# NikolaZubic/2dimageto3dmodel

Measured on NVIDIA H100. Metric: render+loss+GAN images/sec (cfg3: cfg2 render+loss at batch 32 + conv-GAN 256x256 G/D iteration, 1 G : 2 D, Adam), higher is better.
Workload: dtype tf32 (convs) / f32

## Files before the change

### 2dimageto3dmodel_b200/b3d/__init__.py

```python
import ctypes
import os

import torch

_HERE = os.path.dirname(os.path.abspath(__file__))
LIB_PATH = os.path.join(_HERE, "libb3d.so")

MODE_REFERENCE = 0
MODE_PAPER = 1
_MODES = {"R": MODE_REFERENCE, "reference": MODE_REFERENCE, "P": MODE_PAPER, "paper": MODE_PAPER,
          0: MODE_REFERENCE, 1: MODE_PAPER}


class B3DError(RuntimeError):
    pass


def _load():
    if not os.path.exists(LIB_PATH):
        raise B3DError(f"{LIB_PATH} is missing: build it with `make` (or __graft_entry__.build()). "
                       "There is no CPU fallback.")
    lib = ctypes.CDLL(LIB_PATH)
    lib.b3d_last_error.restype = ctypes.c_char_p
    lib.b3d_last_variant.restype = ctypes.c_char_p
    lib.b3d_launch_count.restype = ctypes.c_uint64
    lib.b3d_pc_silhouette_workspace_bytes.restype = ctypes.c_size_t
    return lib


lib = _load()

_vp = ctypes.c_void_p
_i = ctypes.c_int
_f = ctypes.c_float
_sz = ctypes.c_size_t
_ll = ctypes.c_longlong


_signed = []


def _sig(name, *argtypes):
    fn = getattr(lib, name)
    fn.argtypes = list(argtypes)
    fn.restype = ctypes.c_int
    _signed.append(name)
    return fn


_sig("b3d_pc_bin_count", _i)
_sig("b3d_inception_input", _vp, _i, _i, _i, _i, _i, _i, _i, _vp, _vp)
_sig("b3d_maxpool3x3s2_nhwc", _vp, _i, _i, _i, _i, _vp, _i, _vp)
_sig("b3d_mean_hw_nhwc", _vp, _i, _i, _i, _vp, _vp)
_sig("b3d_fid_accumulate", _vp, _i, _i, _vp, _vp, _vp)
_sig("b3d_pc_project", _vp, _vp, _i, _i, _i, _f, _f, _vp, _vp, _vp, _vp, _vp, _vp, _vp)
_sig("b3d_pc_silhouette_fwd_hosttaps", _vp, _vp, _vp, _i, _vp, _i, _i, _i, _i, _vp, _vp, _sz, _vp)
_sig("b3d_pc_silhouette_bwd_hosttaps", _vp, _vp, _vp, _i, _vp, _vp, _i, _i, _i, _i, _vp, _vp, _vp, _sz, _vp)
_sig("b3d_pc_project_bwd", _vp, _vp, _vp, _vp, _i, _i, _i, _f, _f, _vp, _vp, _vp)
_sig("b3d_pc_splat_grid", _vp, _i, _i, _i, _i, _vp, _vp)
_sig("b3d_mesh_face_setup", _vp, _vp, _vp, _i, _vp, _i, _i, _i, _i, _vp, _vp, _vp, _vp)
_sig("b3d_mesh_render_fwd", _vp, _vp, _vp, _vp, _i, _i, _i, _i, _i, _i, _vp, _vp, _vp, _vp, _vp)
_sig("b3d_conv2d_tf32", _vp, _vp, _vp, _vp, _i, _i, _i, _i, _i, _i, _i, _i, _vp, _vp, _i, _i, _i, _i, _i, _i, _i, _i, _i,
     _f, _vp, _i, _vp, _i, _i, _vp, _vp)
_sig("b3d_conv2d_wgrad_tf32", _vp, _vp, _vp, _i, _i, _i, _i, _i, _i, _i, _i, _i, _i, _i, _i, _i, _i, _i, _vp)
_sig("b3d_conv2d_thin_fwd", _vp, _vp, _vp, _vp, _i, _i, _i, _i, _i, _i, _i, _i, _i, _i, _i, _i, _i, _f, _vp)
_sig("b3d_conv2d_thin_wgrad", _vp, _vp, _vp, _i, _i, _i, _i, _i, _i, _i, _i, _i, _i, _i, _i, _vp)
_sig("b3d_vertex_pipeline_fwd", _vp, _ll, _ll, _ll, _ll, _i, _i, _vp, _vp, _i, _i, _vp, _vp, _vp, _vp, _vp, _vp, _vp)
_sig("b3d_vertex_pipeline_bwd", _vp, _vp, _vp, _vp, _vp, _i, _i, _i, _i, _vp, _vp, _vp, _vp, _vp, _vp, _vp, _vp, _vp)
_sig("b3d_bank_forward", _vp, _vp, _i, _vp, _i, _vp, _i, _vp, _sz, _vp, _i, _vp)
_sig("b3d_bank_backward", _vp, _vp, _i, _vp, _i, _vp, _vp, _vp, _vp)
_sig("b3d_pad_x_fwd", _vp, _vp, _ll, _i, _i, _i, _i, _vp)
_sig("b3d_pad_x_bwd", _vp, _vp, _ll, _i, _i, _i, _i, _vp)
_sig("b3d_stem_input_fwd", _vp, _vp, _vp, _i, _i, _i, _i, _i, _i, _i, _vp)
_sig("b3d_stem_input_bwd", _vp, _vp, _i, _i, _i, _i, _i, _i, _i, _vp)
_sig("b3d_leaky_bwd", _vp, _vp, _vp, _ll, _f, _vp)
_sig("b3d_fold_rows_fwd", _vp, _vp, _i, _i, _i, _i, _i, _i, _i, _vp)
_sig("b3d_fold_rows_bwd", _vp, _vp, _i, _i, _i, _i, _i, _i, _i, _vp)
_sig("b3d_wrap_x_inplace", _vp, _ll, _i, _i, _i, _i, _vp)
_sig("b3d_wrap_x_bwd_inplace", _vp, _ll, _i, _i, _i, _i, _vp)
_sig("b3d_pad_leaky_bias_bwd", _vp, _vp, _vp, _vp, _ll, _i, _i, _i, _i, _f, _vp)
_sig("b3d_vox_blur_axis", _vp, _vp, _vp, _i, _i, _i, _i, _i, _vp)
_sig("b3d_vox_scale_clamp", _vp, _vp, _vp, _i, _i, _vp)
_sig("b3d_vox_scale_clamp_bwd", _vp, _vp, _vp, _vp, _vp, _i, _i, _vp)
_sig("b3d_vox_termination", _vp, _i, _i, _i, _vp, _vp, _vp)
_sig("b3d_vox_termination_bwd", _vp, _vp, _i, _i, _i, _vp, _vp)
_sig("b3d_vox_splat_sorted", _vp, _vp, _i, _i, _i, _i, _vp, _vp)
_sig("b3d_vox_clamp01", _vp, ctypes.c_longlong, _vp)
_sig("b3d_vox_gather", _vp, _vp, _vp, _vp, _i, _i, _i, _i, _vp, _vp)
_sig("b3d_cbn_act_fwd", _vp, _vp, _vp, _vp, _i, _i, _vp, _i, _i, _i, _i, _i, _i, _i, _f, _i, _vp)
_sig("b3d_cbn_act_bwd1", _vp, _vp, _vp, _vp, _vp, _i, _i, _vp, _vp, _i, _vp, _vp, _i, _i, _vp, _vp, _i, _i, _i, _i, _i, _i, _i, _i,
     _f, _i, _vp)
_sig("b3d_cbn_act_bwd2", _vp, _vp, _vp, _vp, _vp, _i, _vp, _vp, _i, _f, _i, _i, _i, _i, _vp)
_sig("b3d_bn_sums", _vp, _ll, _i, _vp, _vp)
_sig("b3d_cbn_prepare", _vp, _i, _i, _i, _vp, ctypes.c_double, _f, _f, _i, _vp, _vp, _vp, _vp, _vp, _vp, _vp, _vp, _i, _i, _vp)
_sig("b3d_cbn_bwd_reduce", _vp, _vp, _i, _vp, _vp, _i, _i, _vp)
_sig("b3d_bn_sums_per_sample", _vp, _i, _ll, _i, _vp, _vp)
_sig("b3d_cbn_prepare_sync", _vp, _vp, _i, _i, _vp, _vp, _vp, _i, _i, _i, _vp, ctypes.c_double, _f, _f, _vp, _vp, _vp, _vp, _vp, _vp, _vp,
     _vp, _i, _i, _vp)
_sig("b3d_cbn_bwd_reduce_sync", _vp, _vp, _i, _i, _vp, _vp, _vp, _vp, _i, _vp, _vp, _i, _i, _vp)
_sig("b3d_chamfer_nn", _vp, _vp, _i, _i, _i, _vp, _vp, _vp)
_sig("b3d_chamfer_bwd", _vp, _vp, _vp, _vp, _i, _i, _i, _vp, _vp, _vp)
_sig("b3d_flat_loss_fwd", _vp, _vp, _i, _i, _i, _vp, _vp)
_sig("b3d_face_normals_fwd", _vp, _vp, _i, _i, _i, _vp, _vp)
_sig("b3d_face_normals_bwd", _vp, _vp, _vp, _i, _i, _i, _vp, _vp)
_sig("b3d_flat_loss_bwd", _vp, _vp, _i, _i, _i, _vp, _vp, _vp)
_sig("b3d_rgba_mse_iou_fwd", _vp, _vp, _vp, _i, _i, _i, _vp, _vp, _vp)
_sig("b3d_rgba_mse_bwd", _vp, _vp, _vp, _i, _i, _i, _vp, _vp, _vp, _vp)
_sig("b3d_rgba_l1_iou_fwd", _vp, _vp, _vp, _i, _i, _i, _vp, _vp, _vp)
_sig("b3d_rgba_l1_bwd", _vp, _vp, _vp, _i, _i, _i, _vp, _vp, _vp, _vp)
_sig("b3d_mesh_render_bwd", _vp, _vp, _vp, _i, _i, _i, _i, _i, _i, _i, _vp, _vp, _vp, _vp, _vp, _vp, _vp, _vp)
_sig("b3d_gather_fields", _vp, _i, _vp, _vp, _i, _vp)
_sig("b3d_image_batch", _vp, _vp, _vp, _vp, _i, _vp, _vp, _i, _i, _vp, _vp, _vp, _vp, _vp, _vp, _vp)
_sig("b3d_mesh_render_filtered_fwd", _vp, _vp, _vp, _vp, _i, _i, _i, _i, _i, _i, _i, _vp, _vp, _vp, _vp, _vp)
_sig("b3d_mesh_render_filtered_bwd", _vp, _vp, _vp, _i, _i, _i, _i, _i, _i, _i, _i, _vp, _vp, _vp, _vp, _vp, _vp, _vp, _vp)
_sig("b3d_mesh_face_pack", _vp, _vp, _vp, _f, _i, _i, _vp, _vp)
_sig("b3d_mesh_raster_attr_fwd", _vp, _vp, _i, _i, _i, _i, _i, _f, _i, _f, _f, _vp, _vp, _vp, _vp, _vp)
_sig("b3d_mesh_raster_attr_bwd", _vp, _vp, _i, _i, _i, _i, _i, _f, _i, _f, _f, _vp, _vp, _vp, _vp, _vp, _vp, _vp)
_sig("b3d_texel_visibility", _vp, _vp, _vp, _i, _i, _i, _i, _i, _i, _i, _vp, _vp, _vp)
_sig("b3d_pseudogt_pack", _vp, _i, _i, _vp, _vp, _i, _i, _i, _vp, _i, _i, _i, _vp, _vp, _vp, _vp)
_sig("b3d_sample_pack", _vp, _vp, _i, _i, _i, _vp, _i, _vp, _vp, _vp)


def mode_id(mode):
    try:
        return _MODES[mode]
    except KeyError:
        raise B3DError(f"unknown semantics mode {mode!r} (use 'R' or 'P')") from None


def check(rc):
    if rc != 0:
        raise B3DError(f"libb3d error {rc}: {lib.b3d_last_error().decode()}")


def last_variant():
    return lib.b3d_last_variant().decode()


def launch_count():
    return int(lib.b3d_launch_count())


def dev(t, name="tensor", dtype=torch.float32):
    if not isinstance(t, torch.Tensor):
        raise B3DError(f"{name}: expected a torch.Tensor")
    if not t.is_cuda:
        raise B3DError(f"{name}: libb3d runs on CUDA tensors only (got device {t.device}); "
                       "there is no CPU fallback")
    if t.dtype != dtype:
        raise B3DError(f"{name}: expected dtype {dtype}, got {t.dtype}")
    return t if t.is_contiguous() else t.contiguous()


# ... 60 lines not shown
```

### 2dimageto3dmodel_b200/b3d/bank.py

```python
import struct

import torch

from . import B3DError, check, lib, ptr, stream_ptr


def _r32(v):
    return (v + 31) // 32 * 32


def _r64(v):
    return (v + 63) // 64 * 64


class LayerWeights:
    __slots__ = ("wf", "wd", "df", "Cout", "Cin", "kh", "kw", "fold", "Cinp", "Coutp", "Tp", "bias")

    def __init__(self, spec):
        for k in ("Cout", "Cin", "kh", "kw", "fold", "Cinp", "Coutp", "Tp"):
            setattr(self, k, spec[k])
        self.wf = self.wd = self.df = self.bias = None


class WeightBank:
    def __init__(self, convs, fold=(), no_dgrad=(), round_tf32=True):
        self.names = list(convs)
        self.mods = [convs[n] for n in self.names]
        self.round_tf32 = bool(round_tf32)
        self.specs = []
        off_out = off_scr = off_w = 0
        for n, m in zip(self.names, self.mods):
            sn = hasattr(m, "weight_orig")
            w = m.weight_orig if sn else m.weight
            Cout, Cin, kh, kw = w.shape
            fd = n in fold
            Cinp = _r32(kh * Cin if fd else Cin)
            Tp = kw if fd else kh * kw
            sp = dict(name=n, sn=sn, Cout=Cout, Cin=Cin, kh=kh, kw=kw, fold=int(fd), Cinp=Cinp, Coutp=_r32(Cout), Tp=Tp,
                      K=Cin * kh * kw, need_d=n not in no_dgrad)
            sp["wf_off"] = off_out
            off_out += _r64(Tp * Cout * Cinp)
            self.specs.append(sp)
        self.f_total = off_out
        for sp in self.specs:
            sp["wd_off"] = -1
            if sp["need_d"]:
                sp["wd_off"] = off_out
                off_out += _r64(sp["Tp"] * sp["Cinp"] * sp["Coutp"])
        for sp in self.specs:
            sp["u_off"], sp["v_off"], sp["scal_off"] = off_out, off_out + _r64(sp["Cout"]), off_out + _r64(sp["Cout"]) + _r64(sp["K"])
            off_out = sp["scal_off"] + 64
            sp["t_off"], sp["s_off"] = off_scr, off_scr + _r64(2 * sp["K"])
            off_scr = sp["s_off"] + _r64(sp["Cout"])
            sp["dw_off"] = off_w
            off_w += _r64(sp["Cout"] * sp["K"])
        self.out_total, self.scr_total, self.w_total = off_out, off_scr, off_w
        self._ptrs = None
        self._dev = None

    def params(self):
        return [m.weight_orig if sp["sn"] else m.weight for m, sp in zip(self.mods, self.specs)]

    def _build(self, device):
        if lib.b3d_bank_layer_bytes() != 144:
            raise B3DError("bank: BankLayer record size mismatch between b3d/bank.py and csrc/sn_kernels.cu")
        rec, wtu, wv, emit, dot = [], [], [], [], []
        ptrs = []
        for i, (m, sp) in enumerate(zip(self.mods, self.specs)):
            w = m.weight_orig if sp["sn"] else m.weight
            u = m.weight_u if sp["sn"] else None
            v = m.weight_v if sp["sn"] else None
            for t in (w, u, v):
                if t is not None and (not t.is_cuda or t.dtype != torch.float32 or not t.is_contiguous()):
                    raise B3DError(f"bank: {sp['name']}: parameters must be contiguous CUDA fp32 tensors (no CPU fallback)")
            ptrs.append((w.data_ptr(), u.data_ptr() if u is not None else 0, v.data_ptr() if v is not None else 0))
            rec.append(struct.pack("<3Q9q12i", ptrs[-1][0], ptrs[-1][1], ptrs[-1][2], sp["t_off"], sp["s_off"], sp["wf_off"],
                                   sp["wd_off"], sp["u_off"], sp["v_off"], sp["scal_off"], sp["wf_off"], sp["dw_off"],
                                   sp["Cout"], sp["Cin"], sp["kh"], sp["kw"], sp["fold"], sp["Cinp"], sp["Coutp"], sp["Tp"],
                                   int(sp["sn"]), 0, 0, 0))
            if sp["sn"]:
                wtu += [(i, a, b, 0) for a in range(-(-sp["K"] // 256)) for b in range(-(-sp["Cout"] // 64))]
                wv += [(i, a, 0, 0) for a in range(-(-sp["Cout"] // 8))]
                dot += [(i, a, 0, 0) for a in range(-(-(sp["Tp"] * sp["Cout"] * sp["Cinp"]) // 4096))]
            emit += [(i, a, b, 0) for a in range(sp["Coutp"] // 32) for b in range(sp["Cinp"] // 32)]

        def dev_bytes(b):
            return torch.frombuffer(bytearray(b), dtype=torch.uint8).to(device)

        def items(lst):
            return torch.tensor(lst if lst else [(0, 0, 0, 0)], dtype=torch.int32).to(device), len(lst)

        self._table = dev_bytes(b"".join(rec))
        self._wtu, self._wv, self._emit, self._dot = items(wtu), items(wv), items(emit), items(dot)
        self._scratch = torch.zeros(max(self.scr_total, 64), device=device)
        self._ptrs, self._dev = ptrs, device

    def _check(self):
        ps = self.params()
        device = ps[0].device
        if self._ptrs is None or self._dev != device:
            self._build(device)
            return
        for (pw, pu, pv), m, sp in zip(self._ptrs, self.mods, self.specs):
            w = m.weight_orig if sp["sn"] else m.weight
            if w.data_ptr() != pw or (sp["sn"] and (m.weight_u.data_ptr() != pu or m.weight_v.data_ptr() != pv)):
                self._build(device)
                return

    def forward(self, training):
        self._check()
        ps = self.params()
        need_grad = torch.is_grad_enabled() and any(p.requires_grad for p in ps)
        outs = _BankFn.apply(self, bool(training), need_grad, *ps)
        n = len(self.specs)
        res = {}
        df_flat = outs[2 * n] if need_grad else None
        for i, sp in enumerate(self.specs):
            lw = LayerWeights(sp)
            lw.wf = outs[i]
            lw.wd = outs[n + i] if sp["need_d"] else None
            if need_grad:
                sz = sp["Tp"] * sp["Cout"] * sp["Cinp"]
                lw.df = df_flat[sp["wf_off"]: sp["wf_off"] + sz].view(sp["Tp"], sp["Cout"], sp["Cinp"])
            lw.bias = getattr(self.mods[i], "bias", None)
            res[sp["name"]] = lw
        return res


class _BankFn(torch.autograd.Function):
    @staticmethod
    def forward(ctx, bank, training, need_grad, *weights):
        device = weights[0].device
        out = torch.empty(bank.out_total, device=device, dtype=torch.float32)
        st = stream_ptr(weights[0])
        check(lib.b3d_bank_forward(ptr(bank._table), ptr(bank._wtu[0]), bank._wtu[1], ptr(bank._wv[0]), bank._wv[1],
                                   ptr(bank._emit[0]), bank._emit[1], ptr(bank._scratch), bank._scratch.numel() * 4,
                                   ptr(out), int(training) | (2 if bank.round_tf32 else 0), st))
        wfs, wds = [], []
        for sp in bank.specs:
            wfs.append(out[sp["wf_off"]: sp["wf_off"] + sp["Tp"] * sp["Cout"] * sp["Cinp"]].view(sp["Tp"], sp["Cout"], sp["Cinp"]))
            if sp["need_d"]:
                wds.append(out[sp["wd_off"]: sp["wd_off"] + sp["Tp"] * sp["Cinp"] * sp["Coutp"]].view(sp["Tp"], sp["Cinp"], sp["Coutp"]))
            else:
                wds.append(out.new_empty(0))
        df = torch.zeros(bank.f_total, device=device, dtype=torch.float32) if need_grad else out.new_empty(0)
        ctx.bank, ctx.out, ctx.df = bank, out, df
        ctx.mark_non_differentiable(*wds, df)
        return (*wfs, *wds, df)

    @staticmethod
    def backward(ctx, *grads):
        bank, out, df = ctx.bank, ctx.out, ctx.df
        n = len(bank.specs)
        if df.numel() == 0:
            return (None, None, None) + (None,) * n
        for sp, g in zip(bank.specs, grads[:n]):
            if g is None:
                continue
            sz = sp["Tp"] * sp["Cout"] * sp["Cinp"]
            if g.data_ptr() != df.data_ptr() + 4 * sp["wf_off"]:
                df[sp["wf_off"]: sp["wf_off"] + sz].copy_(g.reshape(-1))
        dw = torch.zeros(bank.w_total, device=df.device, dtype=torch.float32)
        bank.last_dw = dw
        check(lib.b3d_bank_backward(ptr(bank._table), ptr(bank._dot[0]), bank._dot[1], ptr(bank._emit[0]), bank._emit[1],
                                    ptr(out), ptr(df), ptr(dw), stream_ptr(df)))
        gws = []
        for sp, need in zip(bank.specs, ctx.needs_input_grad[3:]):
            gws.append(dw[sp["dw_off"]: sp["dw_off"] + sp["Cout"] * sp["K"]].view(sp["Cout"], sp["Cin"], sp["kh"], sp["kw"])
                       if need else None)
        return (None, None, None, *gws)
```

### 2dimageto3dmodel_b200/b3d/conv.py

```python
import ctypes

import torch

from . import B3DError, check, dev, last_variant, lib, ptr, stream_ptr
from .bank import LayerWeights

VARIANT_LOG = None


def _conv_call(fn, *args):
    rc = fn(*args)
    if VARIANT_LOG is not None and rc == 0:
        VARIANT_LOG.extend(v for v in last_variant().split(";") if v)
    return rc


def _ints(v):
    return (ctypes.c_int * len(v))(*v)


def _pad_last(t, mult):
    c = t.shape[-1]
    return t if c % mult == 0 else torch.nn.functional.pad(t, (0, mult - c % mult))

# ... 50 lines not shown
def stride2_classes(kh, kw, pad_y, H, W):
    out = []
    for cy in range(2):
        for cx in range(2):
            rs = [(r, s) for r in range(kh) for s in range(kw) if (cy + pad_y - r) % 2 == 0 and (cx - s) % 2 == 0]
            out.append((cy, cx, rs, [(cy + pad_y - r) // 2 for r, s in rs], [(cx - s) // 2 for r, s in rs],
                        (H - cy + 1) // 2, (W - cx + 1) // 2))
    return out


def _merge_parity_classes(classes):
    return len(classes) == 4 and all(c[2] for c in classes) and len({(len(c[2]), c[5], c[6]) for c in classes}) == 1


def _dgrad(gy, wd, in_hw, kh, kw, pad_y=0, stride=1, x_crop=0, g_pitch=0, mask=None, slope=1.0, sums=None):
    gy = _pad_last(gy, 32)
    N, Hout, Wout, Cop = gy.shape
    Cin = wd.shape[1]
    H, W = in_hw
    classes = stride2_classes(kh, kw, pad_y, H, W) if stride == 2 and not x_crop else []
    if stride != 1 and not classes:
        raise B3DError("conv2d_dgrad: stride must be 1 or 2 (x_crop: stride 1 only)")
    merged = _merge_parity_classes(classes)
    opts = None
    if g_pitch or mask is not None or merged:
        opts = _ConvOpts(None, 1.0, 0, g_pitch, 0)
        if mask is not None:
            opts.mask, opts.mask_slope, opts.stats_sum_only = mask.data_ptr(), slope, 1
        if merged:
            opts.nclass = 4
            for i, c in enumerate(classes):
                opts.class_ooy[i], opts.class_oox[i] = c[0], c[1]
    optr = ctypes.cast(ctypes.pointer(opts), ctypes.c_void_p) if opts is not None else None
    gx = torch.empty(N, H, W, Cin, device=gy.device, dtype=torch.float32)
    gptr, st = ctypes.c_void_p(gy.data_ptr()), stream_ptr(gy)

    def launch(Ha, Wa, dy, dx, osy, ooy, oox, taps):
        check(_conv_call(lib.b3d_conv2d_tf32, gptr, ptr(wd), None, ptr(gx), N, Hout, Wout, Cop, Ha, Wa, Cin, len(dy), _ints(dy),
                         _ints(dx), 1, 1, H, W, Cin, osy, osy, ooy, oox, 1.0, _ints(taps) if taps else None,
                         kh * kw if taps else 0, ptr(sums), 0, 0, optr, st))

    if stride == 1:
        launch(H, W, [pad_y - r for r in range(kh) for _ in range(kw)], [-s - x_crop for _ in range(kh) for s in range(kw)],
               1, 0, 0, None)
    elif merged:
        launch(classes[0][5], classes[0][6], [v for c in classes for v in c[3]], [v for c in classes for v in c[4]], 2, 0, 0,
               [r * kw + s for c in classes for r, s in c[2]])
    else:
        for cy, cx, rs, dy, dx, Ha, Wa in classes:
            if not rs:
                gx[:, cy::2, cx::2] = 0
                continue
            launch(Ha, Wa, dy, dx, 2, cy, cx, [r * kw + s for r, s in rs])
    return gx


def _wgrad(gy, x, kh, kw, pad_y=0, stride=1, x_crop=0, sink=None, g_pitch=0, fold_kh=0, fold_cin=0):
    N, Hout, Wout, Cout = gy.shape
    _, H, W, Cin = x.shape
    tap_major = int(sink is not None)
    st = stream_ptr(gy)
    if fold_kh:
        dw = sink if tap_major else torch.zeros(Cout, fold_cin, 1, kw, device=gy.device, dtype=torch.float32)
        check(_conv_call(lib.b3d_conv2d_wgrad_tf32, ctypes.c_void_p(gy.data_ptr()), ptr(x), ptr(dw), N, H, W, fold_cin, Hout,
                         Wout, Cout, 1, kw, pad_y, 1, 0, tap_major, fold_kh, g_pitch, st))
        return dw
    if _thin(Cout, Cin, kh, kw, stride):
        dw = sink if tap_major else torch.zeros(Cout, Cin, kh, kw, device=gy.device, dtype=torch.float32)
        check(_conv_call(lib.b3d_conv2d_thin_wgrad, ptr(gy), ptr(x), ptr(dw), N, H, W, Cin, Hout, Wout, Cout, kh, kw, pad_y,
                         x_crop, tap_major, st))
        return dw
    if tap_major:
        if Cout % 32:
            raise B3DError(f"conv2d: tap-major weight gradient needs Cout % 32 == 0 or a thin head (Cout={Cout})")
        dw = sink
    else:
        gy, x = _pad_last(gy, 32), _pad_last(x, 32)
        dw = torch.zeros(gy.shape[3], x.shape[3], kh, kw, device=gy.device, dtype=torch.float32)
    check(_conv_call(lib.b3d_conv2d_wgrad_tf32, ctypes.c_void_p(gy.data_ptr()), ptr(x), ptr(dw), N, H, W, x.shape[3], Hout, Wout,
                     gy.shape[3], kh, kw, pad_y, stride, x_crop, tap_major, 0, g_pitch, st))
    return dw if tap_major else dw[:Cout, :Cin]


def conv2d_nhwc(x, weight, bias=None, pad_y=0, stride=1, leaky=1.0, wt=None, pad_out=0, pad_mode=1, x_crop=0):
    x = dev(x, "x")
    Cout, Cin_w, kh, kw = weight.shape
    if Cin_w != x.shape[3]:
        raise B3DError(f"conv2d: input has {x.shape[3]} channels, weight expects {Cin_w}")
    wt = dev(wt if wt is not None else taps_layout(weight), "weight")
    return _fprop(x, wt, bias, kh, kw, pad_y, stride, leaky, pad_out, pad_mode, x_crop)


def conv2d_dgrad_nhwc(dy_, weight, in_hw, pad_y=0, stride=1, x_crop=0):
    Cout, Cin, kh, kw = weight.shape
    wd = _d_layout(weight.permute(2, 3, 0, 1).reshape(kh * kw, Cout, Cin))
    return _dgrad(dev(dy_, "grad_output"), wd, in_hw, kh, kw, pad_y, stride, x_crop)


def conv2d_wgrad_nhwc(dy_, x, kh, kw, pad_y=0, stride=1, x_crop=0):
    return _wgrad(dev(dy_, "grad_output"), dev(x, "input"), kh, kw, pad_y, stride, x_crop)


class ActLink:
    __slots__ = ("armed", "slope", "pad", "mode", "ptr", "shape", "want_gb", "gb", "done")

    def __init__(self):
        self.armed = self.done = False
        self.gb = None


class _Conv(torch.autograd.Function):
    @staticmethod
    def forward(ctx, x, w, bias, lw, pad_y, stride, leaky, pad_out, pad_mode, x_crop, stats=None, fold_raw=0, link_in=None,
                link_out=None, fold_fwd=False):
        x = dev(x.detach(), "x")
        Cx = x.shape[3]
        fold_pad = 0
        if fold_raw:
            if not lw.fold or Cx != 8 or lw.Cin != 8 or stride != 1 or x_crop:
                raise B3DError("conv2d: on-the-fly fold needs a folded 8-channel stride-1 stem")
            fold_pad = pad_y
        elif Cx != lw.Cinp:
            if lw.fold or Cx != lw.Cin:
                raise B3DError(f"conv2d: input has {Cx} channels, the layer expects {lw.Cinp if lw.fold else lw.Cin}")
            x = _pad_last(x, 32)
        kh, kw = (1, lw.kw) if lw.fold else (lw.kh, lw.kw)
        if lw.fold:
            pad_y = 0
        wf, b = dev(lw.wf.detach(), "weight"), bias.detach() if bias is not None else None
        if fold_raw and fold_fwd:
            from .ew import fold_rows
            out = _fprop(fold_rows(x, lw.kh, fold_pad, lw.Cinp), wf, b, kh, kw, 0, stride, leaky, pad_out, pad_mode, x_crop, stats)
        else:
            out = _fprop(x, wf, b, kh, kw, pad_y, stride, leaky, pad_out, pad_mode, x_crop, stats, fold_raw, fold_pad)
        ctx.save_for_backward(x, out if (leaky != 1.0 or pad_out) else None)
        ctx.lw = lw
        ctx.cfg = (pad_y, stride, Cx, bias is not None, leaky, pad_out, pad_mode, x_crop, kh, kw, fold_raw, fold_pad)
        thin = _thin(lw.Cout, lw.Cinp, kh, kw, stride)
        ctx.link_in = link_in if (link_in is not None and link_in.armed and link_in.ptr == x.data_ptr() and link_in.shape == tuple(x.shape)
                                  and Cx == lw.Cinp and lw.Cinp % 32 == 0 and not fold_raw and not thin) else None
        ctx.link_out = None
        if link_out is not None and pad_out and leaky != 1.0 and lw.Cout % 32 == 0 and not thin:
            link_out.armed, link_out.slope, link_out.pad, link_out.mode = True, float(leaky), int(pad_out), int(pad_mode)
            link_out.ptr, link_out.shape, link_out.done = out.data_ptr(), tuple(out.shape), False
            link_out.want_gb = bias is not None and bool(ctx.needs_input_grad[2])
            ctx.link_out = link_out
        return out

    @staticmethod
    def backward(ctx, gy):
        x, y = ctx.saved_tensors
        lw = ctx.lw
        pad_y, stride, Cx, has_bias, leaky, pad_out, pad_mode, x_crop, kh, kw, fold_raw, fold_pad = ctx.cfg
        Cout, Cin = lw.Cout, lw.Cinp
        N, H, W, _ = x.shape
        gy = dev(gy, "grad_output")
        st = stream_ptr(gy)
        gb = None
        want_gb = has_bias and ctx.needs_input_grad[2]
        g_pitch = 0
        link_out = ctx.link_out
        if link_out is not None and link_out.done:
            link_out.done = False
            if tuple(gy.shape) != tuple(y.shape):
                raise B3DError("conv2d: chained gradient has the wrong shape")
            g_pitch = y.shape[2]
            gb = link_out.gb if want_gb else None
            link_out.gb = None
            gy = gy[:, :, pad_out:y.shape[2] - pad_out]
        elif pad_out:
            _, Ho, OW, _ = y.shape
            masked = torch.empty(N, Ho, OW - 2 * pad_out, Cout, device=gy.device, dtype=torch.float32)
            gb = torch.zeros(Cout, device=gy.device, dtype=torch.float32) if want_gb else None
            check(lib.b3d_pad_leaky_bias_bwd(ptr(gy), ptr(y), ptr(masked), ptr(gb), N * Ho, OW - 2 * pad_out, Cout, pad_out,
                                             pad_mode, float(leaky), st))
            gy = masked
        elif leaky != 1.0:
            masked = torch.empty_like(gy)
            check(lib.b3d_leaky_bwd(ptr(gy), ptr(y), ptr(masked), gy.numel(), float(leaky), st))
            gy = masked
        if gb is None and want_gb:
            gb = gy.sum(dim=(0, 1, 2))
        gx = gw = None
        if ctx.needs_input_grad[0]:
            link_in = ctx.link_in
            sums = torch.zeros(2 * Cin, device=gy.device, dtype=torch.float64) if link_in is not None and link_in.want_gb else None
            gx = _dgrad(gy, lw.wd if lw.wd is not None else _d_layout(lw.wf.detach()), (gy.shape[1] if fold_raw else H, W), kh,
                        kw, pad_y, stride, x_crop, g_pitch, x if link_in is not None else None,
                        link_in.slope if link_in is not None else 1.0, sums)
            if link_in is not None:
                check(lib.b3d_wrap_x_bwd_inplace(ptr(gx), N * H, W - 2 * link_in.pad, Cin, link_in.pad, link_in.mode, st))
                link_in.gb = sums[:Cin].float() if sums is not None else None
                link_in.done = True
            if fold_raw:
                graw = torch.empty(N, H, W, Cx, device=gy.device, dtype=torch.float32)
                check(lib.b3d_fold_rows_bwd(ptr(gx), ptr(graw), N, H, W, Cx, lw.kh, fold_pad, Cin, st))
                gx = graw
            elif Cx != Cin:
# ... 50 lines not shown
```

### 2dimageto3dmodel_b200/b3d/ew.py

```python
import ctypes
import math
import struct

import torch

from . import B3DError, check, dev, lib, ptr, stream_ptr

REPLICATE, CIRCULAR = 0, 1


class _PadX(torch.autograd.Function):
    @staticmethod
    def forward(ctx, x_nhwc, amount, mode):
        x = dev(x_nhwc.detach(), "x")
        N, H, W, C = x.shape
        out = torch.empty(N, H, W + 2 * amount, C, device=x.device, dtype=torch.float32)
        check(lib.b3d_pad_x_fwd(ptr(x), ptr(out), N * H, W, C, amount, mode, stream_ptr(x)))
        ctx.cfg = (amount, mode, x.shape)
        return out

    @staticmethod
    def backward(ctx, g):
        amount, mode, shape = ctx.cfg
        N, H, W, C = shape
# ... 66 lines not shown


def identity_norm(x):
    return x


def norm_kind(norm):
    from torch.nn.modules.batchnorm import _BatchNorm
    if isinstance(norm, _BatchNorm):
        return 'batch'
    if isinstance(norm, torch.nn.InstanceNorm2d) and not norm.track_running_stats:
        return 'instance'
    if norm is identity_norm:
        return 'none'
    return None


def _check_glue(name, y, C_norm, up, pad, pad_mode):
    if y.dim() != 4:
        raise B3DError(f"{name}: expected a 4-D activation, got shape {tuple(y.shape)}")
    C, W = y.shape[1], y.shape[3]
    if C % 4 or 256 % (C // 4):
        raise B3DError(f"{name}: C={C} must be 4 * a divisor of 256")
    if C_norm is not None and C != C_norm:
        raise B3DError(f"{name}: {C} channels, but the norm layer has {C_norm}")
    if pad_mode not in (REPLICATE, CIRCULAR) or pad < 0 or (pad_mode == CIRCULAR and pad > up * W):
        raise B3DError(f"{name}: pad {pad} in mode {pad_mode} does not fit {up * W} columns")


def _f32(v):
    return struct.unpack("f", struct.pack("f", float(v)))[0]


def _dist_world():
    import torch.distributed as dist
    return dist.get_world_size() if dist.is_available() and dist.is_initialized() else 1


class CBNBatch:

    def __init__(self, cbns, z):
        self.offsets, off = {}, 0
        ws, bs = [], []
        for m in cbns:
            C = m.fc_gamma.out_features
            self.offsets[id(m)] = (off, off + C)
            off += 2 * C
            ws += [m.fc_gamma.weight, m.fc_beta.weight]
            bs += [m.fc_gamma.bias, m.fc_beta.bias]
        self.first = id(cbns[0])
        self.n_layers, self.done = len(cbns), 0
        self.gb = torch.nn.functional.linear(z, torch.cat(ws), torch.cat(bs))
        self.sink = None
        self.stats = torch.zeros(off, device=z.device, dtype=torch.float64) if z.is_cuda else None

    def stats_slot(self, cbn):
        if self.stats is None or norm_kind(cbn.norm) != 'batch' or not cbn.norm.training:
            return None
        goff, boff = self.offsets[id(cbn)]
        return self.stats[goff: goff + 2 * (boff - goff)]

    shared = False

    def grad_sink(self, N=None):
        if self.sink is None:
            self.sink = torch.empty_like(self.gb) if not self.shared else torch.empty(N, self.gb.shape[1], device=self.gb.device)
        return self.sink


class BNAffine(CBNBatch):
    shared = True

    def __init__(self, bn):
        C = bn.num_features
        self.offsets = {id(bn): (0, C)}
        self.first, self.n_layers, self.done = id(bn), 1, 0
        self.gb = torch.cat((bn.weight - 1, bn.bias)).view(1, 2 * C)
        self.sink, self.stats = None, None


class _CBNActPad(torch.autograd.Function):

    @staticmethod
    def forward(ctx, y, gb, cb, key, bn, skip, skip_off, up, pad, post_leaky, sums_in=None, slope=0.2, pad_mode=REPLICATE):
        y = dev(y.detach(), "y")
        N, H, W, C = y.shape
        gbd = dev(gb.detach(), "gamma/beta")
        P = gbd.shape[1]
        gp = 0 if cb.shared else P
        goff, boff = cb.offsets[key]
        st = stream_ptr(y)
        mode, sums, count, sync, peers = 0, None, 1.0, False, None
        kind = norm_kind(bn)
        if kind is None:
            raise B3DError(f"fused norm glue: unsupported norm layer {bn!r}")
        if kind == 'instance':
            sums = torch.empty(N, 2 * C, device=y.device, dtype=torch.float64)
            check(lib.b3d_bn_sums_per_sample(ptr(y), N, H * W, C, ptr(sums), st))
            mode, count = 3, float(H * W)
        elif kind == 'none':
            mode = 4
        elif bn.training or bn.running_mean is None:
            if sums_in is not None:
                sums = sums_in
            else:
                sums = torch.empty(2 * C, device=y.device, dtype=torch.float64)
                check(lib.b3d_bn_sums(ptr(y), N * H * W, C, ptr(sums), st))
            mode, count = 1, float(N * H * W)
            if bn.training and _dist_world() > 1 and bn.__class__.__name__.startswith("Synchronized"):
                import torch.distributed as dist
                from .sync import peer_sync
                mode, count, sync = 2, count * dist.get_world_size(), True
                peers = peer_sync(y.device) if C <= 512 else None
                if peers is None:
                    dist.all_reduce(sums)
        per_sample = mode >= 3
        mean = torch.empty((N, C) if per_sample else C, device=y.device, dtype=torch.float32)
        invstd = torch.empty_like(mean)
        scale = torch.empty(N, C, device=y.device, dtype=torch.float32)
        shift, gt = torch.empty_like(scale), torch.empty_like(scale)
        track = kind == 'batch' and bn.training and bn.track_running_stats
        momentum = -1.0 if kind != 'batch' or bn.momentum is None else float(bn.momentum)
        eps = float(bn.eps) if kind != 'none' else 0.0
        if peers is not None:
            check(lib.b3d_cbn_prepare_sync(peers.data, peers.flag, peers.rank, peers.world, ptr(peers.epoch), ptr(peers.err),
                                           ptr(gbd), gp, goff, boff, ptr(sums), count, float(bn.eps), momentum,
                                           ptr(bn.running_mean) if track else None, ptr(bn.running_var) if track else None,
                                           ptr(bn.num_batches_tracked) if track else None,
                                           ptr(mean), ptr(invstd), ptr(scale), ptr(shift), ptr(gt), N, C, st))
        else:
            check(lib.b3d_cbn_prepare(ptr(gbd), gp, goff, boff, ptr(sums), count, eps, momentum, mode,
                                      ptr(bn.running_mean) if (track or mode == 0) else None,
                                      ptr(bn.running_var) if (track or mode == 0) else None,
                                      ptr(bn.num_batches_tracked) if track else None,
                                      ptr(mean), ptr(invstd), ptr(scale), ptr(shift), ptr(gt), N, C, st))
        sk = dev(skip.detach(), "skip") if skip is not None else None
        pitch = sk.shape[2] if sk is not None else 0
        out = torch.empty(N, up * H, up * W + 2 * pad, C, device=y.device, dtype=torch.float32)
        check(lib.b3d_cbn_act_fwd(ptr(y), ptr(scale), ptr(shift), ptr(sk), pitch, skip_off, ptr(out), N, H, W, C, up, pad,
                                  int(pad_mode), float(slope), int(post_leaky), st))
        ctx.save_for_backward(y, gt, scale, shift, mean, invstd, sk if sk is not None else torch.empty(0))
        ctx.cb, ctx.key = cb, key
        ctx.cfg = (skip_off, up, pad, post_leaky, mode, sync, count, sk is not None, skip.shape if skip is not None else None,
                   P, goff, boff, float(slope), int(pad_mode))
        ctx.peers = peers
        ctx.clamp_lim = _f32(1.0 / math.sqrt(_f32(bn.eps))) if sync else None
        return out

    @staticmethod
    def backward(ctx, gout):
        y, gt, scale, shift, mean, invstd, sk = ctx.saved_tensors
        skip_off, up, pad, post_leaky, mode, sync, count, has_skip, skip_shape, P, goff, boff, slope, pad_mode = ctx.cfg
        cb = ctx.cb
        N, H, W, C = y.shape
        gout = dev(gout, "grad")
        st = stream_ptr(y)
        ga = torch.empty_like(y)
        gskip, gpitch = None, 0
        if has_skip and ctx.needs_input_grad[5]:
            gpitch = skip_shape[2]
            gskip = torch.zeros(skip_shape, device=y.device) if gpitch != W else torch.empty(skip_shape, device=y.device)
        want_gb = ctx.needs_input_grad[1]
        sink = cb.grad_sink(N) if want_gb else torch.empty(N, P, device=y.device)
        s1 = ctypes.c_void_p(sink.data_ptr() + 4 * boff)
        s2 = ctypes.c_void_p(sink.data_ptr() + 4 * goff)
        stat_pitch = C if mode >= 3 else 0
        check(lib.b3d_cbn_act_bwd1(ptr(gout), ptr(y), ptr(scale), ptr(shift), ptr(sk) if has_skip else None,
                                   sk.shape[2] if has_skip else 0, skip_off, ptr(mean), ptr(invstd), stat_pitch, ptr(ga), ptr(gskip),
                                   gpitch, skip_off, s1, s2, P, N, H, W, C, up, pad, pad_mode, slope, int(post_leaky), st))
        inv_m = 0.0
        if mode >= 3:
            inv_m = 1.0 / count if mode == 3 else 0.0
            check(lib.b3d_cbn_act_bwd2(ptr(ga), ptr(y), ptr(gt), ptr(mean), ptr(invstd), C, s1, s2, P, inv_m, N, H, W, C, st))
        elif mode != 0:
            red = torch.empty(2 * C, device=y.device, dtype=torch.float32)
            peers = ctx.peers
            if sync and peers is not None:
                check(lib.b3d_cbn_bwd_reduce_sync(peers.data, peers.flag, peers.rank, peers.world, ptr(peers.epoch), ptr(peers.err),
                                                  s1, s2, P, ptr(gt), ptr(red), N, C, st))
            else:
                check(lib.b3d_cbn_bwd_reduce(s1, s2, P, ptr(gt), ptr(red), N, C, st))
                if sync:
                    import torch.distributed as dist
                    dist.all_reduce(red)
            if sync:
                red[C:].mul_(invstd < ctx.clamp_lim)
            inv_m = 1.0 / count
        else:
            red = torch.zeros(2 * C, device=y.device, dtype=torch.float32)
        if mode < 3:
            check(lib.b3d_cbn_act_bwd2(ptr(ga), ptr(y), ptr(gt), ptr(mean), ptr(invstd), 0, ptr(red),
                                       ctypes.c_void_p(red.data_ptr() + 4 * C), 0, inv_m, N, H, W, C, st))
        ggb = None
        if want_gb:
            cb.done += 1
            if ctx.key == cb.first:
                if cb.done != cb.n_layers:
                    raise RuntimeError(f"CBNBatch: {cb.done} of {cb.n_layers} layers ran their backward before the first layer's")
                ggb = sink.sum(dim=0, keepdim=True) if cb.shared else sink
        return ga, ggb, None, None, None, gskip, None, None, None, None, None, None, None


def bn_act_pad(y_nchw, bn, skip_nchw=None, skip_off=0, up=1, pad=1, post_relu=False, slope=0.0):
    cb = BNAffine(bn)
    y = y_nchw.permute(0, 2, 3, 1)
    C = y.shape[3]
    if C % 4 or 256 % (C // 4):
        raise B3DError(f"bn_act_pad: C={C} must be 4 * a divisor of 256")
    skip = skip_nchw.permute(0, 2, 3, 1) if skip_nchw is not None else None
    out = _CBNActPad.apply(y, cb.gb, cb, id(bn), bn, skip, int(skip_off), int(up), int(pad), bool(post_relu), None, float(slope))
    return out.permute(0, 3, 1, 2)


def cbn_act_pad(y_nchw, cbn, z, skip_nchw=None, skip_off=0, up=1, pad=1, post_leaky=False, cb=None, sums=None,
                pad_mode=REPLICATE):
    if norm_kind(cbn.norm) is None:
        raise B3DError(f"cbn_act_pad: unsupported norm layer {cbn.norm!r}")
    _check_glue("cbn_act_pad", y_nchw, cbn.fc_gamma.out_features, int(up), int(pad), int(pad_mode))
    if cb is None:
        cb = CBNBatch([cbn], z)
    y = y_nchw.permute(0, 2, 3, 1)
    skip = skip_nchw.permute(0, 2, 3, 1) if skip_nchw is not None else None
    out = _CBNActPad.apply(y, cb.gb, cb, id(cbn), cbn.norm, skip, int(skip_off), int(up), int(pad), bool(post_leaky), sums, 0.2,
                           int(pad_mode))
    return out.permute(0, 3, 1, 2)


def in_act_pad(y_nchw, norm, pad=0, pad_mode=CIRCULAR, slope=0.2):
    if norm_kind(norm) != 'instance' or not norm.affine:
        raise B3DError(f"in_act_pad: expected an affine InstanceNorm2d without running buffers, got {norm!r}")
    _check_glue("in_act_pad", y_nchw, norm.num_features, 1, int(pad), int(pad_mode))
    cb = BNAffine(norm)
    out = _CBNActPad.apply(y_nchw.permute(0, 2, 3, 1), cb.gb, cb, id(norm), norm, None, 0, 1, int(pad), False, None,
                           float(slope), int(pad_mode))
    return out.permute(0, 3, 1, 2)
```

### 2dimageto3dmodel_b200/csrc/b3d_core.cu

```cuda
#include <atomic>
#include <stdarg.h>
#include <string.h>

#include "b3d_common.cuh"

namespace b3d {
static thread_local char g_err[512] = "";
static thread_local char g_variant[256] = "";
static std::atomic<uint64_t> g_launches{0};

void set_error(const char* fmt, ...) {
    va_list ap;
    va_start(ap, fmt);
    vsnprintf(g_err, sizeof(g_err), fmt, ap);
    va_end(ap);
}
void clear_variant() { g_variant[0] = 0; }
void add_variant(const char* fmt, ...) {
    size_t n = strlen(g_variant);
    if (n + 2 >= sizeof(g_variant)) return;
    if (n) g_variant[n++] = ';';
    va_list ap;
    va_start(ap, fmt);
    vsnprintf(g_variant + n, sizeof(g_variant) - n, fmt, ap);
    va_end(ap);
}
void count_launch(int n) { g_launches.fetch_add((uint64_t)n, std::memory_order_relaxed); }
}

extern "C" {
const char* b3d_last_error(void) { return b3d::g_err; }
const char* b3d_last_variant(void) { return b3d::g_variant; }
int b3d_version(void) { return 420; }
uint64_t b3d_launch_count(void) { return b3d::g_launches.load(std::memory_order_relaxed); }
}
```

### 2dimageto3dmodel_b200/csrc/ew_kernels.cu

```cuda
#include "b3d_common.cuh"

namespace {
constexpr int NT = 256;

__device__ __forceinline__ int src_col(int wo, int a, int W, int mode) {
    const int w = wo - a;
    if (mode == 0) return w < 0 ? 0 : (w >= W ? W - 1 : w);
    return w < 0 ? w + W : (w >= W ? w - W : w);
}

__global__ void __launch_bounds__(NT)
pad_x_fwd_kernel(const float4* __restrict__ x, float4* __restrict__ out, long long rows, int W, int C4, int a, int mode) {
    const int Wo = W + 2 * a;
    const long long total = rows * Wo * C4;
    for (long long i = (long long)blockIdx.x * NT + threadIdx.x; i < total; i += (long long)gridDim.x * NT) {
        const int c = (int)(i % C4);
        const long long t = i / C4;
        const int wo = (int)(t % Wo);
        const long long r = t / Wo;
        out[i] = __ldg(x + (r * W + src_col(wo, a, W, mode)) * C4 + c);
    }
}

__global__ void __launch_bounds__(NT)
// ... 542 lines not shown
        for (int r = 0; r < world; ++r) t += src[(size_t)r * SYNC_MAX + i];
        vec[i] = t;
    }
    __syncthreads();
}

__global__ void __launch_bounds__(512)
cbn_prepare_sync_kernel(SyncPeers P, int rank, int world, unsigned* epoch_ctr, int* err, const float* __restrict__ gb,
                        int gb_pitch, int gamma_off, int beta_off, const double* __restrict__ sums_local, double count, float eps,
                        float momentum, float* __restrict__ running_mean, float* __restrict__ running_var,
                        long long* __restrict__ nbt, float* __restrict__ mean_out, float* __restrict__ invstd_out,
                        float* __restrict__ scale, float* __restrict__ shift, float* __restrict__ gt, int N, int C) {
    __shared__ double tot[SYNC_MAX];
    __shared__ float mean_s[SYNC_MAX / 2], inv_s[SYNC_MAX / 2];
    const float f = cbn_momentum(momentum, nbt);
    for (int i = threadIdx.x; i < 2 * C; i += blockDim.x) tot[i] = sums_local[i];
    __syncthreads();
    peer_allreduce(P, rank, world, epoch_ctr, err, tot, 2 * C);
    for (int c = threadIdx.x; c < C; c += blockDim.x) {
        const double m = tot[c] / count;
        const double var_b = (tot[C + c] - tot[c] * m) / count;
        const float mean = (float)m, invstd = (float)(1.0 / sqrt(var_b > (double)eps ? var_b : (double)eps));
        mean_s[c] = mean;
        inv_s[c] = invstd;
        mean_out[c] = mean;
        invstd_out[c] = invstd;
        if (running_mean != nullptr) {
            running_mean[c] = (1.f - f) * running_mean[c] + f * mean;
            running_var[c] = (1.f - f) * running_var[c] + f * (float)(var_b * (count / (count > 1.0 ? count - 1.0 : 1.0)));
            if (c == 0 && nbt != nullptr) *nbt += 1;
        }
    }
    __syncthreads();
    for (int i = threadIdx.x; i < N * C; i += blockDim.x) {
        const int n = i / C, c = i - n * C;
        const float g1 = 1.f + gb[(long long)n * gb_pitch + gamma_off + c];
        const float sc = inv_s[c] * g1;
        scale[i] = sc;
        shift[i] = gb[(long long)n * gb_pitch + beta_off + c] - mean_s[c] * sc;
        gt[i] = g1;
    }
}

__global__ void __launch_bounds__(512)
cbn_bwd_reduce_sync_kernel(SyncPeers P, int rank, int world, unsigned* epoch_ctr, int* err, const float* __restrict__ S1,
                           const float* __restrict__ S2, int s_pitch, const float* __restrict__ gt, float* __restrict__ red, int N,
                           int C) {
    __shared__ double tot[SYNC_MAX];
    for (int c = threadIdx.x; c < C; c += blockDim.x) {
        float a = 0.f, b = 0.f;
        for (int n = 0; n < N; ++n) {
            const float g = gt[(long long)n * C + c];
            a = fmaf(g, S1[(long long)n * s_pitch + c], a);
            b = fmaf(g, S2[(long long)n * s_pitch + c], b);
        }
        tot[c] = (double)a;
        tot[C + c] = (double)b;
    }
    __syncthreads();
    peer_allreduce(P, rank, world, epoch_ctr, err, tot, 2 * C);
    for (int i = threadIdx.x; i < 2 * C; i += blockDim.x) red[i] = (float)tot[i];
}

__global__ void __launch_bounds__(NT)
cbn_bwd_reduce_kernel(const float* __restrict__ S1, const float* __restrict__ S2, int s_pitch, const float* __restrict__ gt,
                      float* __restrict__ red, int N, int C) {
    const int c = blockIdx.x * NT + threadIdx.x;
    if (c >= C) return;
    float a = 0.f, b = 0.f;
    for (int n = 0; n < N; ++n) {
        const float g = gt[(long long)n * C + c];
        a = fmaf(g, S1[(long long)n * s_pitch + c], a);
        b = fmaf(g, S2[(long long)n * s_pitch + c], b);
    }
    red[c] = a;
    red[C + c] = b;
}

namespace {
struct CbnGeom {
    int N, H, W, C4;
    int up, pad;
    int skip_pitch, skip_off;
    float slope;
    int post_leaky;
};

__device__ __forceinline__ float lk(float v, float s) { return v >= 0.f ? v : v * s; }

template <int PM>
__global__ void __launch_bounds__(NT)
cbn_act_fwd_kernel(const float4* __restrict__ y, const float4* __restrict__ scale, const float4* __restrict__ shift,
                   const float4* __restrict__ skip, float4* __restrict__ out, const CbnGeom g) {
    const int Wo = g.up * g.W + 2 * g.pad, Ho = g.up * g.H;
    const long long total = (long long)g.N * Ho * Wo * g.C4;
    for (long long i = (long long)blockIdx.x * NT + threadIdx.x; i < total; i += (long long)gridDim.x * NT) {
        const int c = (int)(i % g.C4);
        long long t = i / g.C4;
        const int xo = (int)(t % Wo);
        t /= Wo;
        const int yo = (int)(t % Ho);
        const int n = (int)(t / Ho);
        int xs = src_col(xo, g.pad, g.up * g.W, PM);
        const int ys = yo / g.up;
        xs /= g.up;
        const float4 v = __ldg(y + (((long long)n * g.H + ys) * g.W + xs) * g.C4 + c);
        const float4 sc = __ldg(scale + (long long)n * g.C4 + c), sh = __ldg(shift + (long long)n * g.C4 + c);
        float4 o = make_float4(lk(fmaf(v.x, sc.x, sh.x), g.slope), lk(fmaf(v.y, sc.y, sh.y), g.slope),
                               lk(fmaf(v.z, sc.z, sh.z), g.slope), lk(fmaf(v.w, sc.w, sh.w), g.slope));
        if (g.skip_pitch) {
            const float4 k = __ldg(skip + (((long long)n * g.H + ys) * g.skip_pitch + xs + g.skip_off) * g.C4 + c);
            o.x += k.x; o.y += k.y; o.z += k.z; o.w += k.w;
        }
        if (g.post_leaky) o = make_float4(lk(o.x, g.slope), lk(o.y, g.slope), lk(o.z, g.slope), lk(o.w, g.slope));
        out[i] = o;
    }
}

template <int PM>
__global__ void __launch_bounds__(NT)
cbn_act_fwd_rows_kernel(const float4* __restrict__ y, const float4* __restrict__ scale, const float4* __restrict__ shift,
                        const float4* __restrict__ skip, float4* __restrict__ out, const CbnGeom g) {
    const int Wo = g.up * g.W + 2 * g.pad, Ho = g.up * g.H, Wu = g.up * g.W;
    const int c = threadIdx.x % g.C4, px0 = threadIdx.x / g.C4, PPB = NT / g.C4;
    for (int row = blockIdx.x; row < g.N * Ho; row += gridDim.x) {
        const int n = row / Ho, yo = row - n * Ho;
        const int ys = yo / g.up;
        const float4 sc = __ldg(scale + (long long)n * g.C4 + c), sh = __ldg(shift + (long long)n * g.C4 + c);
        const float4* yrow = y + (((long long)n * g.H + ys) * g.W) * g.C4 + c;
        const float4* srow = g.skip_pitch ? skip + (((long long)n * g.H + ys) * g.skip_pitch + g.skip_off) * g.C4 + c : nullptr;
        float4* orow = out + (long long)row * Wo * g.C4 + c;
        constexpr int U = 4;
        for (int xb = px0; xb < Wo; xb += U * PPB) {
            float4 v[U], k[U];
#pragma unroll
            for (int u = 0; u < U; ++u) {
                const int xo = xb + u * PPB;
                if (xo >= Wo) continue;
                int xs = src_col(xo, g.pad, Wu, PM);
                xs = g.up == 2 ? xs >> 1 : xs;
                v[u] = __ldg(yrow + (long long)xs * g.C4);
                if (srow) k[u] = __ldg(srow + (long long)xs * g.C4);
            }
#pragma unroll
            for (int u = 0; u < U; ++u) {
                const int xo = xb + u * PPB;
                if (xo >= Wo) continue;
                float4 o = make_float4(lk(fmaf(v[u].x, sc.x, sh.x), g.slope), lk(fmaf(v[u].y, sc.y, sh.y), g.slope),
                                       lk(fmaf(v[u].z, sc.z, sh.z), g.slope), lk(fmaf(v[u].w, sc.w, sh.w), g.slope));
                if (srow) { o.x += k[u].x; o.y += k[u].y; o.z += k[u].z; o.w += k[u].w; }
                if (g.post_leaky) o = make_float4(lk(o.x, g.slope), lk(o.y, g.slope), lk(o.z, g.slope), lk(o.w, g.slope));
                orow[(long long)xo * g.C4] = o;
            }
        }
    }
}

template <int PM, bool PS>
__global__ void __launch_bounds__(NT)
cbn_act_bwd1_kernel(const float4* __restrict__ gout, const float4* __restrict__ y, const float4* __restrict__ scale,
                    const float4* __restrict__ shift, const float4* __restrict__ skip, const float4* __restrict__ mean,
                    const float4* __restrict__ invstd, float4* __restrict__ ga, float4* __restrict__ gskip, int gskip_pitch,
                    int gskip_off, float* __restrict__ S1, float* __restrict__ S2, int s_pitch, const CbnGeom g, int rows_per_cta) {
    const int n = blockIdx.y;
    const int y0 = blockIdx.x * rows_per_cta, y1 = min(y0 + rows_per_cta, g.H);
    const int Wu = g.up * g.W, Wo = Wu + 2 * g.pad;
    for (int c = threadIdx.x % g.C4, lane_px = threadIdx.x / g.C4, px_step = NT / g.C4; c < g.C4; c += g.C4) {
        const float4 sc = __ldg(scale + (long long)n * g.C4 + c), sh = __ldg(shift + (long long)n * g.C4 + c);
        const long long so = PS ? (long long)n * g.C4 + c : c;
        const float4 mu = __ldg(mean + so), is = __ldg(invstd + so);
        float4 a1 = make_float4(0.f, 0.f, 0.f, 0.f), a2 = a1;
        for (int p = y0 * g.W + lane_px; p < y1 * g.W; p += px_step) {
            const int ys = p / g.W, xs = p % g.W;
            float4 s = make_float4(0.f, 0.f, 0.f, 0.f);
            for (int i = 0; i < g.up; ++i) {
                const float4* row = gout + (((long long)n * g.up * g.H + g.up * ys + i) * Wo) * g.C4 + c;
                if (PM == 0) {
                    int lo = g.up * xs + g.pad, hi = lo + g.up;
                    if (xs == 0) lo = 0;
                    if (xs == g.W - 1) hi = Wo;
                    for (int xo = lo; xo < hi; ++xo) {
                        const float4 v = __ldg(row + (long long)xo * g.C4);
                        s.x += v.x; s.y += v.y; s.z += v.z; s.w += v.w;
                    }
                } else {
                    for (int u = g.up * xs; u < g.up * xs + g.up; ++u) {
                        float4 v = __ldg(row + (long long)(u + g.pad) * g.C4);
                        s.x += v.x; s.y += v.y; s.z += v.z; s.w += v.w;
                        if (u < g.pad) {
                            v = __ldg(row + (long long)(u + g.pad + Wu) * g.C4);
                            s.x += v.x; s.y += v.y; s.z += v.z; s.w += v.w;
                        }
                        if (u >= Wu - g.pad) {
                            v = __ldg(row + (long long)(u + g.pad - Wu) * g.C4);
                            s.x += v.x; s.y += v.y; s.z += v.z; s.w += v.w;
                        }
                    }
                }
            }
            const long long idx = (((long long)n * g.H + ys) * g.W + xs) * g.C4 + c;
            const float4 v = __ldg(y + idx);
            const float4 pre = make_float4(fmaf(v.x, sc.x, sh.x), fmaf(v.y, sc.y, sh.y), fmaf(v.z, sc.z, sh.z), fmaf(v.w, sc.w, sh.w));
            if (g.post_leaky) {
                float4 k = make_float4(0.f, 0.f, 0.f, 0.f);
                if (g.skip_pitch) k = __ldg(skip + (((long long)n * g.H + ys) * g.skip_pitch + xs + g.skip_off) * g.C4 + c);
                s.x = (lk(pre.x, g.slope) + k.x) >= 0.f ? s.x : s.x * g.slope;
                s.y = (lk(pre.y, g.slope) + k.y) >= 0.f ? s.y : s.y * g.slope;
                s.z = (lk(pre.z, g.slope) + k.z) >= 0.f ? s.z : s.z * g.slope;
                s.w = (lk(pre.w, g.slope) + k.w) >= 0.f ? s.w : s.w * g.slope;
            }
            if (gskip) gskip[(((long long)n * g.H + ys) * gskip_pitch + xs + gskip_off) * g.C4 + c] = s;
            const float4 a = make_float4(pre.x >= 0.f ? s.x : s.x * g.slope, pre.y >= 0.f ? s.y : s.y * g.slope,
                                         pre.z >= 0.f ? s.z : s.z * g.slope, pre.w >= 0.f ? s.w : s.w * g.slope);
            ga[idx] = a;
            a1.x += a.x; a1.y += a.y; a1.z += a.z; a1.w += a.w;
            a2.x = fmaf(a.x, (v.x - mu.x) * is.x, a2.x); a2.y = fmaf(a.y, (v.y - mu.y) * is.y, a2.y);
            a2.z = fmaf(a.z, (v.z - mu.z) * is.z, a2.z); a2.w = fmaf(a.w, (v.w - mu.w) * is.w, a2.w);
        }
        float* s1 = S1 + (long long)n * s_pitch + c * 4;
        float* s2 = S2 + (long long)n * s_pitch + c * 4;
        atomicAdd(s1 + 0, a1.x); atomicAdd(s1 + 1, a1.y); atomicAdd(s1 + 2, a1.z); atomicAdd(s1 + 3, a1.w);
        atomicAdd(s2 + 0, a2.x); atomicAdd(s2 + 1, a2.y); atomicAdd(s2 + 2, a2.z); atomicAdd(s2 + 3, a2.w);
    }
}

template <bool PS>
__global__ void __launch_bounds__(NT)
cbn_act_bwd2_kernel(float4* __restrict__ ga, const float4* __restrict__ y, const float4* __restrict__ gamma_t,
                    const float4* __restrict__ mean, const float4* __restrict__ invstd, const float4* __restrict__ m1,
                    const float4* __restrict__ m2, int m4, float inv_m, long long per_n, int C4, long long total) {
    for (long long i = (long long)blockIdx.x * NT + threadIdx.x; i < total; i += (long long)gridDim.x * NT) {
        const int c = (int)(i % C4);
        const long long n = i / per_n;
        const float4 a = ga[i], v = __ldg(y + i), gt = __ldg(gamma_t + n * C4 + c);
        const long long so = PS ? n * C4 + c : c;
        const float4 mu = __ldg(mean + so), is = __ldg(invstd + so);
        float4 q1 = __ldg(m1 + (PS ? n * m4 + c : c)), q2 = __ldg(m2 + (PS ? n * m4 + c : c));
        if (PS) {
            q1.x *= gt.x; q1.y *= gt.y; q1.z *= gt.z; q1.w *= gt.w;
            q2.x *= gt.x; q2.y *= gt.y; q2.z *= gt.z; q2.w *= gt.w;
        }
        q1.x *= inv_m; q1.y *= inv_m; q1.z *= inv_m; q1.w *= inv_m;
        q2.x *= inv_m; q2.y *= inv_m; q2.z *= inv_m; q2.w *= inv_m;
        ga[i] = make_float4(is.x * (a.x * gt.x - q1.x - (v.x - mu.x) * is.x * q2.x), is.y * (a.y * gt.y - q1.y - (v.y - mu.y) * is.y * q2.y),
                            is.z * (a.z * gt.z - q1.z - (v.z - mu.z) * is.z * q2.z), is.w * (a.w * gt.w - q1.w - (v.w - mu.w) * is.w * q2.w));
    }
}
}

extern "C" {
int b3d_cbn_act_fwd(const float* y, const float* scale, const float* shift, const float* skip, int skip_pitch, int skip_off,
                    float* out, int N, int H, int W, int C, int up, int pad, int pad_mode, float slope, int post_leaky,
                    void* stream) {
    B3D_REQUIRE(N >= 0 && H > 0 && W > 0 && C > 0 && C % 4 == 0 && (up == 1 || up == 2) && pad >= 0, B3D_EINVAL,
                "b3d_cbn_act_fwd: bad arguments");
    B3D_REQUIRE(pad_mode == 0 || (pad_mode == 1 && pad <= up * W), B3D_EINVAL, "b3d_cbn_act_fwd: pad mode %d with pad %d > %d columns",
                pad_mode, pad, up * W);
    if (N == 0) return B3D_OK;
    B3D_REQUIRE(y && scale && shift && out && (skip != nullptr) == (skip_pitch != 0), B3D_EINVAL, "b3d_cbn_act_fwd: null pointer");
    CbnGeom g{N, H, W, C / 4, up, pad, skip_pitch, skip_off, slope, post_leaky};
    const long long total = (long long)N * up * H * (up * W + 2 * pad) * (C / 4);
    cudaStream_t st = (cudaStream_t)stream;
    if (g.C4 <= NT && NT % g.C4 == 0 && (up == 1 || up == 2)) {
        const int rows = N * up * H, grid = rows < 132 * 16 ? rows : 132 * 16;
        if (pad_mode == 0)
            cbn_act_fwd_rows_kernel<0><<<grid, NT, 0, st>>>((const float4*)y, (const float4*)scale, (const float4*)shift,
                                                            (const float4*)skip, (float4*)out, g);
        else
            cbn_act_fwd_rows_kernel<1><<<grid, NT, 0, st>>>((const float4*)y, (const float4*)scale, (const float4*)shift,
                                                            (const float4*)skip, (float4*)out, g);
    } else if (pad_mode == 0) {
        cbn_act_fwd_kernel<0><<<grid_for(total), NT, 0, st>>>((const float4*)y, (const float4*)scale, (const float4*)shift,
                                                              (const float4*)skip, (float4*)out, g);
    } else {
        cbn_act_fwd_kernel<1><<<grid_for(total), NT, 0, st>>>((const float4*)y, (const float4*)scale, (const float4*)shift,
                                                              (const float4*)skip, (float4*)out, g);
    }
    B3D_LAUNCH_OK();
    return B3D_OK;
}

int b3d_cbn_act_bwd1(const float* gout, const float* y, const float* scale, const float* shift, const float* skip, int skip_pitch,
                     int skip_off, const float* mean, const float* invstd, int stat_pitch, float* ga, float* gskip, int gskip_pitch,
                     int gskip_off, float* S1, float* S2, int s_pitch, int N, int H, int W, int C, int up, int pad, int pad_mode,
                     float slope, int post_leaky, void* stream) {
    B3D_REQUIRE(N >= 0 && H > 0 && W > 0 && C > 0 && C % 4 == 0 && C / 4 <= NT && NT % (C / 4) == 0 && (up == 1 || up == 2), B3D_EINVAL,
                "b3d_cbn_act_bwd1: bad arguments (C/4 must divide %d)", NT);
    B3D_REQUIRE(stat_pitch == 0 || stat_pitch == C, B3D_EINVAL, "b3d_cbn_act_bwd1: statistics pitch %d must be 0 or C=%d", stat_pitch, C);
    B3D_REQUIRE(pad >= 0 && (pad_mode == 0 || (pad_mode == 1 && pad <= up * W)), B3D_EINVAL,
                "b3d_cbn_act_bwd1: pad mode %d with pad %d > %d columns", pad_mode, pad, up * W);
    if (N == 0) return B3D_OK;
    B3D_REQUIRE(gout && y && scale && shift && mean && invstd && ga && S1 && S2, B3D_EINVAL, "b3d_cbn_act_bwd1: null pointer");
    cudaStream_t st = (cudaStream_t)stream;
    B3D_REQUIRE(s_pitch >= C && s_pitch % 4 == 0, B3D_EINVAL, "b3d_cbn_act_bwd1: S pitch %d must be >= C and a multiple of 4", s_pitch);
    B3D_CUDA_OK(cudaMemset2DAsync(S1, sizeof(float) * (size_t)s_pitch, 0, sizeof(float) * (size_t)C, (size_t)N, st));
    B3D_CUDA_OK(cudaMemset2DAsync(S2, sizeof(float) * (size_t)s_pitch, 0, sizeof(float) * (size_t)C, (size_t)N, st));
    CbnGeom g{N, H, W, C / 4, up, pad, skip_pitch, skip_off, slope, post_leaky};
    int rows = (int)(((long long)N * H + 132 * 8 - 1) / (132 * 8));
    rows = rows < 1 ? 1 : rows;
    dim3 grid(b3d::ceil_div(H, rows), N);
    auto kernel = pad_mode == 0 ? (stat_pitch ? cbn_act_bwd1_kernel<0, true> : cbn_act_bwd1_kernel<0, false>)
                                : (stat_pitch ? cbn_act_bwd1_kernel<1, true> : cbn_act_bwd1_kernel<1, false>);
    kernel<<<grid, NT, 0, st>>>((const float4*)gout, (const float4*)y, (const float4*)scale, (const float4*)shift, (const float4*)skip,
                                (const float4*)mean, (const float4*)invstd, (float4*)ga, (float4*)gskip, gskip_pitch, gskip_off, S1, S2,
                                s_pitch, g, rows);
    B3D_LAUNCH_OK();
    return B3D_OK;
}

int b3d_cbn_act_bwd2(float* ga, const float* y, const float* gamma_t, const float* mean, const float* invstd, int stat_pitch,
                     const float* m1, const float* m2, int m_pitch, float inv_m, int N, int H, int W, int C, void* stream) {
    B3D_REQUIRE(N >= 0 && H > 0 && W > 0 && C > 0 && C % 4 == 0, B3D_EINVAL, "b3d_cbn_act_bwd2: bad arguments");
    B3D_REQUIRE(stat_pitch == 0 || (stat_pitch == C && m_pitch >= C && m_pitch % 4 == 0), B3D_EINVAL,
                "b3d_cbn_act_bwd2: statistics pitch %d must be 0 or C=%d (sums pitch %d >= C, a multiple of 4)", stat_pitch, C, m_pitch);
    if (N == 0) return B3D_OK;
    B3D_REQUIRE(ga && y && gamma_t && mean && invstd && m1 && m2, B3D_EINVAL, "b3d_cbn_act_bwd2: null pointer");
    const long long per_n = (long long)H * W * (C / 4), total = per_n * N;
    auto kernel = stat_pitch ? cbn_act_bwd2_kernel<true> : cbn_act_bwd2_kernel<false>;
    kernel<<<grid_for(total), NT, 0, (cudaStream_t)stream>>>((float4*)ga, (const float4*)y, (const float4*)gamma_t, (const float4*)mean,
                                                             (const float4*)invstd, (const float4*)m1, (const float4*)m2, m_pitch / 4,
                                                             inv_m, per_n, C / 4, total);
    B3D_LAUNCH_OK();
    return B3D_OK;
}

int b3d_bn_sums(const float* y, long long rows, int C, double* sums, void* stream) {
    B3D_REQUIRE(rows > 0 && C >= 4 && C % 4 == 0 && C / 4 <= NT && NT % (C / 4) == 0, B3D_EINVAL,
                "b3d_bn_sums: C=%d must be 4 * a divisor of %d", C, NT);
    B3D_REQUIRE(y && sums, B3D_EINVAL, "b3d_bn_sums: null pointer");
    B3D_CHECK_ALIGNED(y);
    cudaStream_t st = (cudaStream_t)stream;
    B3D_CUDA_OK(cudaMemsetAsync(sums, 0, sizeof(double) * 2 * (size_t)C, st));
    const int ppb = NT / (C / 4);
    long long blocks = (rows + ppb - 1) / ppb;
    if (blocks > 132 * 2) blocks = 132 * 2;
    bn_sums_kernel<false><<<(int)blocks, NT, 0, st>>>((const float4*)y, rows, C / 4, sums);
    B3D_LAUNCH_OK();
    return B3D_OK;
}

int b3d_bn_sums_per_sample(const float* y, int N, long long HW, int C, double* sums, void* stream) {
    B3D_REQUIRE(N > 0 && N <= 65535 && HW > 0 && C >= 4 && C % 4 == 0 && C / 4 <= NT && NT % (C / 4) == 0, B3D_EINVAL,
                "b3d_bn_sums_per_sample: N=%d (1..65535), C=%d must be 4 * a divisor of %d", N, C, NT);
    B3D_REQUIRE(y && sums, B3D_EINVAL, "b3d_bn_sums_per_sample: null pointer");
    B3D_CHECK_ALIGNED(y);
    cudaStream_t st = (cudaStream_t)stream;
    B3D_CUDA_OK(cudaMemsetAsync(sums, 0, sizeof(double) * 2 * (size_t)C * N, st));
    const int ppb = NT / (C / 4);
    long long blocks = (HW + ppb - 1) / ppb;
    const long long cap = (132 * 2 + N - 1) / N;
    if (blocks > cap) blocks = cap;
    bn_sums_kernel<true><<<dim3((unsigned)blocks, (unsigned)N), NT, 0, st>>>((const float4*)y, HW, C / 4, sums);
    B3D_LAUNCH_OK();
    return B3D_OK;
}

int b3d_cbn_prepare(const float* gb, int gb_pitch, int gamma_off, int beta_off, const double* sums, double count, float eps,
                    float momentum, int mode, float* running_mean, float* running_var, long long* num_batches_tracked,
                    float* mean, float* invstd, float* scale, float* shift, float* gt, int N, int C, void* stream) {
    B3D_REQUIRE(N > 0 && C > 0 && gb && mean && invstd && scale && shift && gt, B3D_EINVAL, "b3d_cbn_prepare: bad arguments");
    B3D_REQUIRE(mode >= 0 && mode <= 4, B3D_EINVAL, "b3d_cbn_prepare: unknown mode %d", mode);
    B3D_REQUIRE(mode == 0 ? (running_mean && running_var) : (mode == 4 || (sums != nullptr && count > 0)), B3D_EINVAL,
                "b3d_cbn_prepare: mode %d needs %s", mode, mode == 0 ? "running statistics" : "sums and a count");
    cbn_prepare_kernel<<<(N * C + NT - 1) / NT, NT, 0, (cudaStream_t)stream>>>(gb, gb_pitch, gamma_off, beta_off, sums, count, eps,
                                                                                momentum, mode, running_mean, running_var,
                                                                                num_batches_tracked, mean, invstd, scale, shift, gt, N, C);
    B3D_LAUNCH_OK();
    return B3D_OK;
}

int b3d_cbn_bwd_reduce(const float* S1, const float* S2, int s_pitch, const float* gt, float* red, int N, int C, void* stream) {
    B3D_REQUIRE(N > 0 && C > 0 && S1 && S2 && gt && red, B3D_EINVAL, "b3d_cbn_bwd_reduce: bad arguments");
    cbn_bwd_reduce_kernel<<<(C + NT - 1) / NT, NT, 0, (cudaStream_t)stream>>>(S1, S2, s_pitch, gt, red, N, C);
    B3D_LAUNCH_OK();
    return B3D_OK;
}

size_t b3d_sync_buffer_bytes(int world) { return (size_t)2 * world * SYNC_MAX * sizeof(double) + (size_t)2 * world * sizeof(unsigned) + 256; }
size_t b3d_sync_flag_offset(int world) { return (size_t)2 * world * SYNC_MAX * sizeof(double); }

static int fill_peers(SyncPeers& P, const void* const* peer_data, const void* const* peer_flag, int rank, int world, int C) {
    B3D_REQUIRE(world >= 2 && world <= SYNC_RANKS && rank >= 0 && rank < world, B3D_EINVAL, "sync: world=%d rank=%d (2..%d ranks)", world,
                rank, SYNC_RANKS);
    B3D_REQUIRE(C > 0 && 2 * C <= SYNC_MAX, B3D_EINVAL, "sync: C=%d exceeds %d", C, SYNC_MAX / 2);
    B3D_REQUIRE(peer_data && peer_flag, B3D_EINVAL, "sync: null peer tables");
// ... 34 lines not shown
```

### 2dimageto3dmodel_b200/csrc/sn_kernels.cu

```cuda
#include "b3d_common.cuh"

namespace {

constexpr int NT = 256;
constexpr float SN_EPS = 1e-12f;

struct alignas(16) BankLayer {
    const float* w;
    float* u;
    float* v;
    long long t_off;
    long long s_off;
    long long wf_off;
    long long wd_off;
    long long u_off;
    long long v_off;
    long long scal_off;
    long long df_off;
    long long dw_off;
    int Cout, Cin, kh, kw;
    int fold, Cinp, Coutp, Tp;
    int sn, pad0, pad1, pad2;
};

struct Item { int layer, a, b, c; };

constexpr double T_SCALE = 68719476736.0;
__device__ __forceinline__ float t_value(const float* scratch, long long t_off, int k) {
    return (float)((double)reinterpret_cast<const long long*>(scratch + t_off)[k] * (1.0 / T_SCALE));
}

__device__ __forceinline__ float block_reduce_sum(float v, float* red) {
    v = b3d::warp_sum(v);
    const int lane = threadIdx.x & 31, w = threadIdx.x >> 5;
    __syncthreads();
    if (lane == 0) red[w] = v;
    __syncthreads();
    float r = 0.f;
#pragma unroll
    for (int i = 0; i < NT / 32; ++i) r += red[i];
    return r;
}

__global__ void __launch_bounds__(NT)
bank_wtu_kernel(const BankLayer* __restrict__ layers, const Item* __restrict__ items, float* __restrict__ scratch) {
    const Item it = items[blockIdx.x];
    const BankLayer L = layers[it.layer];
    const int K = L.Cin * L.kh * L.kw;
    const int col = it.a * NT + threadIdx.x;
    const int r0 = it.b * 64, r1 = min(r0 + 64, L.Cout);
    if (col >= K) return;
    float acc = 0.f;
    const float* w = L.w + (size_t)r0 * K + col;
#pragma unroll 8
    for (int r = r0; r < r1; ++r, w += K) acc = fmaf(__ldg(w), __ldg(L.u + r), acc);
    atomicAdd(reinterpret_cast<unsigned long long*>(scratch + L.t_off) + col,
              (unsigned long long)__double2ll_rn((double)acc * T_SCALE));
}

__global__ void __launch_bounds__(NT)
bank_wv_kernel(const BankLayer* __restrict__ layers, const Item* __restrict__ items, float* __restrict__ scratch, int training) {
    __shared__ float red[NT / 32];
    const Item it = items[blockIdx.x];
    const BankLayer L = layers[it.layer];
    const int K = L.Cin * L.kh * L.kw;
    float inv = 1.f;
    if (training) {
        float p = 0.f;
        for (int k = threadIdx.x; k < K; k += NT) { const float x = t_value(scratch, L.t_off, k); p = fmaf(x, x, p); }
        inv = 1.f / fmaxf(sqrtf(block_reduce_sum(p, red)), SN_EPS);
    }
    const int warp = threadIdx.x >> 5, lane = threadIdx.x & 31;
    const int row = it.a * (NT / 32) + warp;
    if (row >= L.Cout) return;
    const float* w = L.w + (size_t)row * K;
    float acc = 0.f;
    for (int k = lane; k < K; k += 32) acc = fmaf(__ldg(w + k), training ? t_value(scratch, L.t_off, k) : L.v[k], acc);
    acc = b3d::warp_sum(acc);
    if (lane == 0) scratch[L.s_off + row] = acc * inv;
}

__device__ __forceinline__ float tf32_rna(float x, int on) {
    if (!on) return x;
    uint32_t r;
    asm("cvt.rna.tf32.f32 %0, %1;" : "=r"(r) : "f"(x));
    return __uint_as_float(r);
}

__device__ __forceinline__ float layer_sigma(const BankLayer& L, const float* sv, int training, float* red, float* inv_s) {
    float p = 0.f;
    for (int r = threadIdx.x; r < L.Cout; r += NT) {
        const float x = sv[r];
        p = fmaf(training ? x : L.u[r], x, p);
    }
    p = block_reduce_sum(p, red);
    if (!training) { *inv_s = 1.f; return p; }
    const float nrm = fmaxf(sqrtf(p), SN_EPS);
    *inv_s = 1.f / nrm;
    return p / nrm;
}

__global__ void __launch_bounds__(NT)
bank_emit_kernel(const BankLayer* __restrict__ layers, const Item* __restrict__ items, const float* __restrict__ scratch,
                 float* __restrict__ outb, int training, int round_tf32) {
    __shared__ float red[NT / 32];
    const Item it = items[blockIdx.x];
    const BankLayer L = layers[it.layer];
    const int K = L.Cin * L.kh * L.kw, taps = L.kh * L.kw;
    float sigma = 1.f, inv_s = 1.f;
    if (L.sn) {
        const float* sv = scratch + L.s_off;
        sigma = layer_sigma(L, sv, training, red, &inv_s);
        if (it.a == 0 && it.b == 0) {
            if (threadIdx.x == 0) { outb[L.scal_off] = sigma; outb[L.scal_off + 1] = 0.f; }
            float inv_t = 1.f;
            if (training) {
                float p = 0.f;
                for (int k = threadIdx.x; k < K; k += NT) { const float x = t_value(scratch, L.t_off, k); p = fmaf(x, x, p); }
                inv_t = 1.f / fmaxf(sqrtf(block_reduce_sum(p, red)), SN_EPS);
            }
            for (int k = threadIdx.x; k < K; k += NT) {
                const float x = training ? t_value(scratch, L.t_off, k) * inv_t : L.v[k];
                if (training) L.v[k] = x;
                outb[L.v_off + k] = x;
            }
            for (int r = threadIdx.x; r < L.Cout; r += NT) {
                const float x = training ? sv[r] * inv_s : L.u[r];
                if (training) L.u[r] = x;
                outb[L.u_off + r] = x;
            }
        }
    }
    const float rs = 1.f / sigma;
    const int co0 = it.a * 32, ci0 = it.b * 32;
    const int real_cin = L.fold ? L.kh * L.Cin : L.Cin;
    for (int e = threadIdx.x; e < 32 * 32; e += NT) {
        const int ci = ci0 + (e & 31), co = co0 + (e >> 5);
        if (co >= L.Cout || ci >= L.Cinp) continue;
        const bool real = ci < real_cin;
        int c = ci, r_fix = 0;
        if (L.fold) { c = ci % L.Cin; r_fix = ci / L.Cin; }
        for (int tp = 0; tp < L.Tp; ++tp) {
            float val = 0.f;
            if (real) {
                const int src = L.fold ? ((co * L.Cin + c) * L.kh + r_fix) * L.kw + tp : (co * L.Cin + c) * taps + tp;
                val = tf32_rna(__ldg(L.w + src) * rs, round_tf32);
            }
            outb[L.wf_off + ((size_t)tp * L.Cout + co) * L.Cinp + ci] = val;
        }
    }
    if (L.wd_off < 0) return;
    const int cop0 = it.a * 32;
    for (int e = threadIdx.x; e < 32 * 32; e += NT) {
        const int co = cop0 + (e & 31), ci = ci0 + (e >> 5);
        if (co >= L.Coutp || ci >= L.Cinp) continue;
        const bool real = ci < real_cin && co < L.Cout;
        int c = ci, r_fix = 0;
        if (L.fold) { c = ci % L.Cin; r_fix = ci / L.Cin; }
        for (int tp = 0; tp < L.Tp; ++tp) {
            float val = 0.f;
            if (real) {
                const int src = L.fold ? ((co * L.Cin + c) * L.kh + r_fix) * L.kw + tp : (co * L.Cin + c) * taps + tp;
                val = tf32_rna(__ldg(L.w + src) * rs, round_tf32);
            }
            outb[L.wd_off + ((size_t)tp * L.Cinp + ci) * L.Coutp + co] = val;
        }
    }
}

__global__ void __launch_bounds__(NT)
bank_bwd_dot_kernel(const BankLayer* __restrict__ layers, const Item* __restrict__ items, float* __restrict__ outb,
                    const float* __restrict__ dfb) {
    __shared__ float red[NT / 32];
    const Item it = items[blockIdx.x];
    const BankLayer L = layers[it.layer];
    if (!L.sn) return;
    const float* df = dfb + L.df_off;
    const float* wf = outb + L.wf_off;
    const size_t n = (size_t)L.Tp * L.Cout * L.Cinp;
    const size_t e0 = (size_t)it.a * 4096;
    float p = 0.f;
#pragma unroll 4
    for (int j = threadIdx.x; j < 4096; j += NT) {
        const size_t e = e0 + j;
        if (e < n) p = fmaf(__ldg(df + e), __ldg(wf + e), p);
    }
    p = block_reduce_sum(p, red);
    if (threadIdx.x == 0) atomicAdd(outb + L.scal_off + 1, p);
}

__global__ void __launch_bounds__(NT)
bank_bwd_emit_kernel(const BankLayer* __restrict__ layers, const Item* __restrict__ items, const float* __restrict__ outb,
                     const float* __restrict__ dfb, float* __restrict__ dwb) {
    const Item it = items[blockIdx.x];
    const BankLayer L = layers[it.layer];
    const int taps = L.kh * L.kw, K = L.Cin * taps;
    const float sigma = L.sn ? outb[L.scal_off] : 1.f, ip = L.sn ? outb[L.scal_off + 1] : 0.f;
    const float* df = dfb + L.df_off;
    float* dw = dwb + L.dw_off;
    const float* uu = outb + L.u_off;
    const float* vv = outb + L.v_off;
    const float rs = 1.f / sigma;
    const int co0 = it.a * 32, ci0 = it.b * 32;
    const int real_cin = L.fold ? L.kh * L.Cin : L.Cin;
    for (int e = threadIdx.x; e < 32 * 32; e += NT) {
        const int ci = ci0 + (e & 31), co = co0 + (e >> 5);
        if (co >= L.Cout || ci >= real_cin) continue;
        int c = ci, r_fix = 0;
        if (L.fold) { c = ci % L.Cin; r_fix = ci / L.Cin; }
        const float uc = L.sn ? uu[co] * ip : 0.f;
        for (int tp = 0; tp < L.Tp; ++tp) {
            const int src = L.fold ? ((co * L.Cin + c) * L.kh + r_fix) * L.kw + tp : (co * L.Cin + c) * taps + tp;
            const float g = __ldg(df + ((size_t)tp * L.Cout + co) * L.Cinp + ci);
            dw[src] = L.sn ? (g - uc * vv[src - co * K]) * rs : g;
        }
    }
}

}

extern "C" {

int b3d_bank_layer_bytes(void) { return (int)sizeof(BankLayer); }

int b3d_bank_forward(const void* layers, const void* items_wtu, int n_wtu, const void* items_wv, int n_wv,
                     const void* items_emit, int n_emit, float* scratch, size_t scratch_bytes, float* out, int training,
                     void* stream) {
    B3D_REQUIRE(layers && items_emit && scratch && out, B3D_EINVAL, "b3d_bank_forward: null pointer");
    B3D_REQUIRE(n_wv >= 0 && n_emit > 0 && n_wtu >= 0, B3D_EINVAL, "b3d_bank_forward: bad item counts");
    cudaStream_t st = (cudaStream_t)stream;
    B3D_CUDA_OK(cudaMemsetAsync(scratch, 0, scratch_bytes, st));
    const BankLayer* L = static_cast<const BankLayer*>(layers);
    const int flags = training;
    training &= 1;
    if (training && n_wtu > 0) {
        bank_wtu_kernel<<<n_wtu, NT, 0, st>>>(L, static_cast<const Item*>(items_wtu), scratch);
        B3D_LAUNCH_OK();
    }
    if (n_wv > 0) {
        bank_wv_kernel<<<n_wv, NT, 0, st>>>(L, static_cast<const Item*>(items_wv), scratch, training);
        B3D_LAUNCH_OK();
    }
    const int round_tf32 = (flags >> 1) & 1;
    bank_emit_kernel<<<n_emit, NT, 0, st>>>(L, static_cast<const Item*>(items_emit), scratch, out, training, round_tf32);
    B3D_LAUNCH_OK();
    return B3D_OK;
}

int b3d_bank_backward(const void* layers, const void* items_dot, int n_dot, const void* items_emit, int n_emit, float* out,
                      const float* df, float* dw, void* stream) {
    B3D_REQUIRE(layers && items_emit && n_emit > 0 && n_dot >= 0 && out && df && dw, B3D_EINVAL, "b3d_bank_backward: bad arguments");
    cudaStream_t st = (cudaStream_t)stream;
    const BankLayer* L = static_cast<const BankLayer*>(layers);
    if (n_dot > 0) {
        bank_bwd_dot_kernel<<<n_dot, NT, 0, st>>>(L, static_cast<const Item*>(items_dot), out, df);
        B3D_LAUNCH_OK();
    }
    bank_bwd_emit_kernel<<<n_emit, NT, 0, st>>>(L, static_cast<const Item*>(items_emit), out, df, dw);
    B3D_LAUNCH_OK();
    return B3D_OK;
}

}
```

### 2dimageto3dmodel_b200/csrc/tc_common.cuh

```cuda
#pragma once
#include <cuda.h>
#include <cuda_runtime.h>
#include <stdint.h>

#include "b3d_common.cuh"

namespace tc {

__device__ __forceinline__ uint32_t smem_u32(const void* p) { return (uint32_t)__cvta_generic_to_shared(p); }

__device__ __forceinline__ void mbar_init(uint64_t* bar, uint32_t count) {
    asm volatile("mbarrier.init.shared::cta.b64 [%0], %1;" ::"r"(smem_u32(bar)), "r"(count));
}
__device__ __forceinline__ void fence_barrier_init() { asm volatile("fence.mbarrier_init.release.cluster;" ::: "memory"); }
__device__ __forceinline__ void fence_proxy_async() { asm volatile("fence.proxy.async.shared::cta;" ::: "memory"); }

__device__ __forceinline__ void mbar_arrive_expect_tx(uint64_t* bar, uint32_t bytes) {
    asm volatile("mbarrier.arrive.expect_tx.shared::cta.b64 _, [%0], %1;" ::"r"(smem_u32(bar)), "r"(bytes) : "memory");
}
__device__ __forceinline__ void mbar_arrive(uint64_t* bar) {
    asm volatile("mbarrier.arrive.shared::cta.b64 _, [%0];" ::"r"(smem_u32(bar)) : "memory");
}
__device__ __forceinline__ void mbar_arrive(uint64_t* bar, uint32_t count) {
    asm volatile("mbarrier.arrive.shared::cta.b64 _, [%0], %1;" ::"r"(smem_u32(bar)), "r"(count) : "memory");
// ... 88 lines not shown
            "wgmma.mma_async.sync.aligned.m64n64k8.f32.tf32.tf32 "
            "{%0, %1, %2, %3, %4, %5, %6, %7, %8, %9, %10, %11, %12, %13, %14, %15, %16, %17, %18, %19, %20, %21, %22, %23, %24, %25, %26, %27, %28, %29, %30, %31}, "
            "{%32, %33, %34, %35}, %36, p, 1, 1;\n"
            "}\n"
            : "+f"(d[0]), "+f"(d[1]), "+f"(d[2]), "+f"(d[3]), "+f"(d[4]), "+f"(d[5]), "+f"(d[6]), "+f"(d[7]), "+f"(d[8]), "+f"(d[9]), "+f"(d[10]), "+f"(d[11]), "+f"(d[12]), "+f"(d[13]), "+f"(d[14]), "+f"(d[15]), "+f"(d[16]), "+f"(d[17]), "+f"(d[18]), "+f"(d[19]), "+f"(d[20]), "+f"(d[21]), "+f"(d[22]), "+f"(d[23]), "+f"(d[24]), "+f"(d[25]), "+f"(d[26]), "+f"(d[27]), "+f"(d[28]), "+f"(d[29]), "+f"(d[30]), "+f"(d[31])
            : "r"(a[0]), "r"(a[1]), "r"(a[2]), "r"(a[3]), "l"(db), "r"(accumulate));
    }
    __device__ __forceinline__ static void mma(float (&d)[32], uint64_t da, uint64_t db, uint32_t accumulate) {
        asm volatile(
            "{\n"
            ".reg .pred p;\n"
            "setp.ne.b32 p, %34, 0;\n"
            "wgmma.mma_async.sync.aligned.m64n64k8.f32.tf32.tf32 "
            "{%0, %1, %2, %3, %4, %5, %6, %7, %8, %9, %10, %11, %12, %13, %14, %15, %16, %17, %18, %19, %20, %21, %22, %23, %24, %25, %26, %27, %28, %29, %30, %31}, "
            "%32, %33, p, 1, 1;\n"
            "}\n"
            : "+f"(d[0]), "+f"(d[1]), "+f"(d[2]), "+f"(d[3]), "+f"(d[4]), "+f"(d[5]), "+f"(d[6]), "+f"(d[7]), "+f"(d[8]), "+f"(d[9]), "+f"(d[10]), "+f"(d[11]), "+f"(d[12]), "+f"(d[13]), "+f"(d[14]), "+f"(d[15]), "+f"(d[16]), "+f"(d[17]), "+f"(d[18]), "+f"(d[19]), "+f"(d[20]), "+f"(d[21]), "+f"(d[22]), "+f"(d[23]), "+f"(d[24]), "+f"(d[25]), "+f"(d[26]), "+f"(d[27]), "+f"(d[28]), "+f"(d[29]), "+f"(d[30]), "+f"(d[31])
            : "l"(da), "l"(db), "r"(accumulate));
    }
};
template <>
struct Wgmma<128> {
    __device__ __forceinline__ static void mma_rs(float (&d)[64], const uint32_t (&a)[4], uint64_t db, uint32_t accumulate) {
        asm volatile(
            "{\n"
            ".reg .pred p;\n"
            "setp.ne.b32 p, %69, 0;\n"
            "wgmma.mma_async.sync.aligned.m64n128k8.f32.tf32.tf32 "
            "{%0, %1, %2, %3, %4, %5, %6, %7, %8, %9, %10, %11, %12, %13, %14, %15, %16, %17, %18, %19, %20, %21, %22, %23, %24, %25, %26, %27, %28, %29, %30, %31, %32, %33, %34, %35, %36, %37, %38, %39, %40, %41, %42, %43, %44, %45, %46, %47, %48, %49, %50, %51, %52, %53, %54, %55, %56, %57, %58, %59, %60, %61, %62, %63}, "
            "{%64, %65, %66, %67}, %68, p, 1, 1;\n"
            "}\n"
            : "+f"(d[0]), "+f"(d[1]), "+f"(d[2]), "+f"(d[3]), "+f"(d[4]), "+f"(d[5]), "+f"(d[6]), "+f"(d[7]), "+f"(d[8]), "+f"(d[9]), "+f"(d[10]), "+f"(d[11]), "+f"(d[12]), "+f"(d[13]), "+f"(d[14]), "+f"(d[15]), "+f"(d[16]), "+f"(d[17]), "+f"(d[18]), "+f"(d[19]), "+f"(d[20]), "+f"(d[21]), "+f"(d[22]), "+f"(d[23]), "+f"(d[24]), "+f"(d[25]), "+f"(d[26]), "+f"(d[27]), "+f"(d[28]), "+f"(d[29]), "+f"(d[30]), "+f"(d[31]), "+f"(d[32]), "+f"(d[33]), "+f"(d[34]), "+f"(d[35]), "+f"(d[36]), "+f"(d[37]), "+f"(d[38]), "+f"(d[39]), "+f"(d[40]), "+f"(d[41]), "+f"(d[42]), "+f"(d[43]), "+f"(d[44]), "+f"(d[45]), "+f"(d[46]), "+f"(d[47]), "+f"(d[48]), "+f"(d[49]), "+f"(d[50]), "+f"(d[51]), "+f"(d[52]), "+f"(d[53]), "+f"(d[54]), "+f"(d[55]), "+f"(d[56]), "+f"(d[57]), "+f"(d[58]), "+f"(d[59]), "+f"(d[60]), "+f"(d[61]), "+f"(d[62]), "+f"(d[63])
            : "r"(a[0]), "r"(a[1]), "r"(a[2]), "r"(a[3]), "l"(db), "r"(accumulate));
    }
    __device__ __forceinline__ static void mma(float (&d)[64], uint64_t da, uint64_t db, uint32_t accumulate) {
        asm volatile(
            "{\n"
            ".reg .pred p;\n"
            "setp.ne.b32 p, %66, 0;\n"
            "wgmma.mma_async.sync.aligned.m64n128k8.f32.tf32.tf32 "
            "{%0, %1, %2, %3, %4, %5, %6, %7, %8, %9, %10, %11, %12, %13, %14, %15, %16, %17, %18, %19, %20, %21, %22, %23, %24, %25, %26, %27, %28, %29, %30, %31, %32, %33, %34, %35, %36, %37, %38, %39, %40, %41, %42, %43, %44, %45, %46, %47, %48, %49, %50, %51, %52, %53, %54, %55, %56, %57, %58, %59, %60, %61, %62, %63}, "
            "%64, %65, p, 1, 1;\n"
            "}\n"
            : "+f"(d[0]), "+f"(d[1]), "+f"(d[2]), "+f"(d[3]), "+f"(d[4]), "+f"(d[5]), "+f"(d[6]), "+f"(d[7]), "+f"(d[8]), "+f"(d[9]), "+f"(d[10]), "+f"(d[11]), "+f"(d[12]), "+f"(d[13]), "+f"(d[14]), "+f"(d[15]), "+f"(d[16]), "+f"(d[17]), "+f"(d[18]), "+f"(d[19]), "+f"(d[20]), "+f"(d[21]), "+f"(d[22]), "+f"(d[23]), "+f"(d[24]), "+f"(d[25]), "+f"(d[26]), "+f"(d[27]), "+f"(d[28]), "+f"(d[29]), "+f"(d[30]), "+f"(d[31]), "+f"(d[32]), "+f"(d[33]), "+f"(d[34]), "+f"(d[35]), "+f"(d[36]), "+f"(d[37]), "+f"(d[38]), "+f"(d[39]), "+f"(d[40]), "+f"(d[41]), "+f"(d[42]), "+f"(d[43]), "+f"(d[44]), "+f"(d[45]), "+f"(d[46]), "+f"(d[47]), "+f"(d[48]), "+f"(d[49]), "+f"(d[50]), "+f"(d[51]), "+f"(d[52]), "+f"(d[53]), "+f"(d[54]), "+f"(d[55]), "+f"(d[56]), "+f"(d[57]), "+f"(d[58]), "+f"(d[59]), "+f"(d[60]), "+f"(d[61]), "+f"(d[62]), "+f"(d[63])
            : "l"(da), "l"(db), "r"(accumulate));
    }
};
__device__ __forceinline__ uint64_t desc_k128(uint32_t smem_addr) {
    uint64_t d = 0;
    d |= (uint64_t)((smem_addr & 0x3FFFF) >> 4);
    d |= (uint64_t)1 << 16;
    d |= (uint64_t)(1024 >> 4) << 32;
    d |= (uint64_t)1 << 62;
    return d;
}
__device__ __forceinline__ uint64_t desc_k32(uint32_t smem_addr) {
    uint64_t d = 0;
    d |= (uint64_t)((smem_addr & 0x3FFFF) >> 4);
    d |= (uint64_t)1 << 16;
    d |= (uint64_t)(256 >> 4) << 32;
    d |= (uint64_t)3 << 62;
    return d;
}

typedef CUresult (*EncodeTiledFn)(CUtensorMap*, CUtensorMapDataType, cuuint32_t, void*, const cuuint64_t*,
                                  const cuuint64_t*, const cuuint32_t*, const cuuint32_t*, CUtensorMapInterleave,
                                  CUtensorMapSwizzle, CUtensorMapL2promotion, CUtensorMapFloatOOBfill);

inline EncodeTiledFn encode_fn() {
    static EncodeTiledFn fn = nullptr;
    if (!fn) {
        void* p = nullptr;
        cudaDriverEntryPointQueryResult q;
        if (cudaGetDriverEntryPoint("cuTensorMapEncodeTiled", &p, cudaEnableDefault, &q) == cudaSuccess &&
            q == cudaDriverEntryPointSuccess)
            fn = reinterpret_cast<EncodeTiledFn>(p);
    }
    return fn;
}

inline int make_tmap_f32(CUtensorMap* m, const void* base, int rank, const uint64_t* dims, const uint64_t* strides_b,
                         const uint32_t* box, const uint32_t* elem_strides = nullptr,
                         CUtensorMapSwizzle swz = CU_TENSOR_MAP_SWIZZLE_128B) {
    EncodeTiledFn fn = encode_fn();
    if (!fn) {
        b3d::set_error("cuTensorMapEncodeTiled is not available from the driver");
        return B3D_ECUDA;
    }
    cuuint64_t gd[5], gs[5];
    cuuint32_t bx[5], es[5];
    for (int i = 0; i < rank; ++i) {
        gd[i] = dims[i];
        bx[i] = box[i];
        es[i] = elem_strides ? elem_strides[i] : 1;
        if (i > 0) gs[i - 1] = strides_b[i - 1];
    }
    CUresult r = fn(m, CU_TENSOR_MAP_DATA_TYPE_FLOAT32, (cuuint32_t)rank, const_cast<void*>(base), gd, gs, bx, es,
                    CU_TENSOR_MAP_INTERLEAVE_NONE, swz, CU_TENSOR_MAP_L2_PROMOTION_L2_256B,
                    CU_TENSOR_MAP_FLOAT_OOB_FILL_NONE);
    if (r != CUDA_SUCCESS) {
        b3d::set_error("cuTensorMapEncodeTiled failed with CUresult %d (rank %d, inner box %u)", (int)r, rank, box[0]);
        return B3D_ECUDA;
    }
    return B3D_OK;
}

inline int num_sms() {
    int dev = 0, n = 0;
    if (cudaGetDevice(&dev) != cudaSuccess || cudaDeviceGetAttribute(&n, cudaDevAttrMultiProcessorCount, dev) != cudaSuccess || n < 1)
        return 132;
    return n;
}

}
```

### 2dimageto3dmodel_b200/csrc/tc_conv.cu

```cuda
#include "tc_common.cuh"

namespace {

constexpr int BM = 128;
constexpr int BK = 32;
constexpr int MMA_K = 8;
constexpr int MAX_TAPS = 25;
constexpr int NTHREADS = 384;

struct ConvParams {
    int N, Hout, Wout, Cout;
    int BW, BH, BI;
    int tiles_x, tiles_y;
    int xbase;
    int ntaps, kslices;
    int sy, sx;
    int dy[MAX_TAPS], dx[MAX_TAPS];
    int wtap[MAX_TAPS];
    int OH, OW, OC, osy, osx;
    float leaky;
    double* stats;
    int fold;
    int fold_y0;
    int mask;
// ... 640 lines not shown
}

int wgrad_splits(int base_ctas, long long ktotal) {
    constexpr long long FIXED = 16;
    const long long sms = tc::num_sms();
    long long smax = ktotal / 8;
    if (smax > 8 * sms) smax = 8 * sms;
    int best = 1;
    long long best_cost = -1;
    for (long long s = 1; s <= smax; ++s) {
        const long long cost = (base_ctas * s + sms - 1) / sms * ((ktotal + s - 1) / s + FIXED);
        if (best_cost < 0 || cost < best_cost) { best = (int)s; best_cost = cost; }
    }
    return best;
}

template <int BN, int STAGES, int KW = 1>
int launch_conv(const CUtensorMap& mx, const CUtensorMap& mw, const CUtensorMap& mm, const ConvParams& p, const float* bias, float* out,
                int tiles, cudaStream_t st) {
    using S = CSmem<BN, STAGES, KW>;
    static_assert(S::TOTAL <= 227 * 1024, "conv pipeline does not fit shared memory");
    B3D_CUDA_OK(cudaFuncSetAttribute(conv_wgmma_kernel<BN, STAGES, KW>, cudaFuncAttributeMaxDynamicSharedMemorySize, S::TOTAL));
    const int work = tiles * b3d::ceil_div(p.Cout, BN) * p.ncls;
    const int sms = tc::num_sms();
    conv_wgmma_kernel<BN, STAGES, KW><<<work < sms ? work : sms, NTHREADS, S::TOTAL, st>>>(mx, mw, mm, p, bias, out, tiles, work);
    B3D_LAUNCH_OK();
    if (KW > 1) b3d::add_variant("conv_wgmma_rowwin<%d,%d,%d>", BN, KW, STAGES);
    else b3d::add_variant("conv_wgmma<%d,%d>", BN, STAGES);
    return B3D_OK;
}

template <int BN>
int launch_rowwin(int kw, const CUtensorMap& mx, const CUtensorMap& mw, const CUtensorMap& mm, const ConvParams& p, const float* bias,
                  float* out, int tiles, cudaStream_t st) {
    if (kw == 2) return launch_conv<BN, BN == 64 ? 5 : 4, 2>(mx, mw, mm, p, bias, out, tiles, st);
    if (kw == 3) return launch_conv<BN, BN == 64 ? 4 : 3, 3>(mx, mw, mm, p, bias, out, tiles, st);
    return launch_conv<BN, BN == 64 ? 3 : 2, 5>(mx, mw, mm, p, bias, out, tiles, st);
}

int pow2_floor(int v) {
    int p = 1;
    while (p * 2 <= v) p *= 2;
    return p;
}

}

extern "C" {

int b3d_conv2d_tf32(const float* x, const float* wt, const float* bias, float* out, int N, int H, int W, int Cin,
                    int Hout, int Wout, int Cout, int ntaps, const int* dy, const int* dx, int sy, int sx, int OH,
                    int OW, int OC, int osy, int osx, int ooy, int oox, float leaky, const int* wtap,
                    int wtaps_total, double* stats, int fold_kh, int fold_pad, const b3d_conv_opts* opts, void* stream) {
    B3D_REQUIRE(N > 0 && H > 0 && W > 0 && Hout > 0 && Wout > 0 && Cout > 0, B3D_EINVAL, "b3d_conv2d_tf32: bad sizes");
    B3D_REQUIRE(Cin > 0 && Cin % BK == 0, B3D_EINVAL, "b3d_conv2d_tf32: Cin=%d must be a multiple of %d", Cin, BK);
    B3D_REQUIRE(ntaps >= 1 && ntaps <= MAX_TAPS && dy && dx, B3D_EINVAL, "b3d_conv2d_tf32: bad taps");
    B3D_REQUIRE(x && wt && out, B3D_EINVAL, "b3d_conv2d_tf32: null pointer");
    B3D_REQUIRE(sy >= 1 && sy <= 2 && sx >= 1 && sx <= 2, B3D_EINVAL, "b3d_conv2d_tf32: stride must be 1 or 2");
    if (!wtap) wtaps_total = ntaps;
    B3D_REQUIRE(wtaps_total >= ntaps || wtap, B3D_EINVAL, "b3d_conv2d_tf32: bad weight tap count");
    for (int t = 0; wtap && t < ntaps; ++t)
        B3D_REQUIRE(wtap[t] >= 0 && wtap[t] < wtaps_total, B3D_EINVAL, "b3d_conv2d_tf32: weight tap %d out of range", wtap[t]);
    B3D_CHECK_ALIGNED(x);
    B3D_CHECK_ALIGNED(wt);
    b3d::clear_variant();

    const float* mask = opts ? opts->mask : nullptr;
    const float mslope = opts ? opts->mask_slope : 1.f;
    B3D_REQUIRE(!mask || (reinterpret_cast<uintptr_t>(mask) % 16 == 0 && OC % 4 == 0), B3D_EINVAL,
                "b3d_conv2d_tf32: the mask needs a 16-byte aligned base and OC %% 4 == 0 (OC=%d)", OC);
    const int stats_sum = (opts && opts->stats_sum_only) ? 1 : 0;
    const int xpitch = (opts && opts->x_row_pitch) ? opts->x_row_pitch : W;
    const int ncls = (opts && opts->nclass > 1) ? opts->nclass : 1;
    B3D_REQUIRE(ncls <= 4 && ntaps % ncls == 0 && (ncls == 1 || (sy == 1 && sx == 1 && fold_kh == 0)), B3D_EINVAL,
                "b3d_conv2d_tf32: nclass=%d needs <= 4 equal tap groups of a stride-1 launch", ncls);
    const int tpc = ntaps / ncls;
    int cooy[4] = {ooy, ooy, ooy, ooy}, coox[4] = {oox, oox, oox, oox};
    for (int c = 0; c < ncls && ncls > 1; ++c) { cooy[c] = opts->class_ooy[c]; coox[c] = opts->class_oox[c]; }
    B3D_REQUIRE(xpitch >= W && (fold_kh == 0 || xpitch == W), B3D_EINVAL, "b3d_conv2d_tf32: x_row_pitch=%d must be >= W=%d (and absent with the on-the-fly fold)", xpitch, W);
    if (fold_kh > 0) {
        B3D_REQUIRE(fold_kh <= 8 && Cin == 32 * ((8 * fold_kh + 31) / 32) && sy == 1 && sx == 1 && !wtap && Wout % BM == 0,
                    B3D_EINVAL, "b3d_conv2d_tf32: on-the-fly fold needs 8 input channels, stride 1 and Wout %% 128 == 0 (Wout=%d)", Wout);
    }
    B3D_REQUIRE(!stats || mask || (osy == 1 && osx == 1), B3D_EINVAL, "b3d_conv2d_tf32: statistics need a dense output");
    const bool bn256 = Cout % 256 == 0 && (long long)N * Hout * Wout / BM * (Cout / 256) * ncls >= tc::num_sms();
    const int BN = bn256 ? 256 : Cout > 64 ? 128 : 64;
    cudaStream_t st = (cudaStream_t)stream;
    CUtensorMap mw;
    {
        const uint64_t dims[3] = {(uint64_t)Cin, (uint64_t)Cout, (uint64_t)wtaps_total};
        const uint64_t strides[2] = {(uint64_t)Cin * 4, (uint64_t)Cout * Cin * 4};
        const uint32_t box[3] = {(uint32_t)BK, (uint32_t)BN, 1};
        if (int rc = tc::make_tmap_f32(&mw, wt, 3, dims, strides, box)) return rc;
    }

    int g_kw = 0, g_step = 1, g_wstep = 1;
    if (sy == 1 && sx == 1 && fold_kh == 0) {
        int kw_ = 1;
        while (kw_ < tpc && dy[kw_] == dy[0]) ++kw_;
        const int step = kw_ > 1 ? dx[1] - dx[0] : 1;
        const int wstep = (wtap && kw_ > 1) ? wtap[1] - wtap[0] : 1;
        bool grid_ok = tpc % kw_ == 0 && (kw_ == 2 || kw_ == 3 || kw_ == 5) && (step == 1 || step == -1) && wstep >= 1 && wstep <= 2 &&
                       (ncls == 1 || wtap != nullptr);
        for (int t = 0; grid_ok && t < ntaps; ++t) {
            const int tc_ = t % tpc, t0 = t - tc_;
            grid_ok = dy[t] == dy[t0 + (tc_ / kw_) * kw_] && dx[t] == dx[0] + (tc_ % kw_) * step;
            if (wtap) grid_ok = grid_ok && wtap[t] == wtap[t0 + (tc_ / kw_) * kw_] + (tc_ % kw_) * wstep;
        }
        if (grid_ok && BN <= 128) { g_kw = kw_; g_step = step; g_wstep = wstep; }
    }

    auto run = [&](int xlo, int xhi) -> int {
        const int wspan = xhi - xlo;
        ConvParams p{};
        p.N = N; p.Hout = Hout; p.Wout = xhi; p.Cout = Cout; p.xbase = xlo;
        p.BW = pow2_floor(wspan < BM ? wspan : BM);
        p.BH = pow2_floor(Hout < BM / p.BW ? Hout : BM / p.BW);
        p.BI = BM / (p.BW * p.BH);
        p.tiles_x = b3d::ceil_div(wspan, p.BW);
        p.tiles_y = b3d::ceil_div(Hout, p.BH);
        const int tiles = p.tiles_x * p.tiles_y * b3d::ceil_div(N, p.BI);
        p.ntaps = tpc; p.kslices = Cin / BK; p.sy = sy; p.sx = sx; p.ncls = ncls;
        for (int t = 0; t < ntaps; ++t) { p.dy[t] = dy[t]; p.dx[t] = dx[t]; p.wtap[t] = wtap ? wtap[t] : t; }
        for (int c = 0; c < 4; ++c) { p.cooy[c] = cooy[c]; p.coox[c] = coox[c]; }
        p.OH = OH; p.OW = OW; p.OC = OC; p.osy = osy; p.osx = osx;
        p.leaky = leaky;
        p.stats = stats;
        p.mask = mask != nullptr; p.mslope = mslope; p.stats_sum = stats_sum;
        p.fold = fold_kh; p.fold_y0 = -fold_pad;
        {
            const unsigned long long esn = p.BI > 1 ? (unsigned long long)OH * OW * OC : 0, esy = p.BH > 1 ? (unsigned long long)osy * OW * OC : 0,
                                     esx = (unsigned long long)osx * OC;
            B3D_REQUIRE((p.BI - 1) * esn + (p.BH - 1) * esy + (p.BW - 1) * esx + OC < (1ull << 32), B3D_EINVAL,
                        "b3d_conv2d_tf32: a %d x %d x %d pixel tile spans more than 2^32 elements of the output", p.BI, p.BH, p.BW);
            p.esn = (uint32_t)esn; p.esy = (uint32_t)esy; p.esx = (uint32_t)esx;
        }
        CUtensorMap mm{};
        if (mask) {
            const uint64_t dims[4] = {(uint64_t)OC, (uint64_t)OW, (uint64_t)OH, (uint64_t)N};
            const uint64_t strides[3] = {(uint64_t)OC * 4, (uint64_t)OW * OC * 4, (uint64_t)OH * OW * OC * 4};
            const uint32_t box[4] = {(uint32_t)BK, (uint32_t)(osx * (p.BW - 1) + 1), (uint32_t)(osy * (p.BH - 1) + 1), (uint32_t)p.BI};
            const uint32_t es[4] = {1, (uint32_t)osx, (uint32_t)osy, 1};
            if (int rc = tc::make_tmap_f32(&mm, mask, 4, dims, strides, box, es)) return rc;
        }
        CUtensorMap mx;
        if (g_kw && wspan >= BM) {
            p.dx0 = g_step > 0 ? dx[0] : dx[g_kw - 1];
            for (int t = 0; t < g_kw; ++t) p.shift[t] = dx[t] - p.dx0;
            const uint64_t dims[4] = {(uint64_t)Cin, (uint64_t)W, (uint64_t)H, (uint64_t)N};
            const uint64_t strides[3] = {(uint64_t)Cin * 4, (uint64_t)xpitch * Cin * 4, (uint64_t)H * xpitch * Cin * 4};
            const uint32_t box[4] = {(uint32_t)BK, (uint32_t)(BM + g_kw - 1), 1, 1};
            if (int rc = tc::make_tmap_f32(&mx, x, 4, dims, strides, box)) return rc;
            CUtensorMap mwr;
            const uint64_t wdims[3] = {(uint64_t)Cin, (uint64_t)Cout, (uint64_t)wtaps_total};
            const uint64_t wstrides[2] = {(uint64_t)Cin * 4, (uint64_t)Cout * Cin * 4};
            const uint32_t wbox[3] = {(uint32_t)BK, (uint32_t)BN, (uint32_t)((g_kw - 1) * g_wstep + 1)};
            const uint32_t wes[3] = {1, 1, (uint32_t)g_wstep};
            if (int rc = tc::make_tmap_f32(&mwr, wt, 3, wdims, wstrides, wbox, wes)) return rc;
            return BN == 128 ? launch_rowwin<128>(g_kw, mx, mwr, mm, p, bias, out, tiles, st)
                             : launch_rowwin<64>(g_kw, mx, mwr, mm, p, bias, out, tiles, st);
        }
        if (fold_kh > 0) {
            B3D_REQUIRE(p.BH == 1 && p.BI == 1, B3D_EINVAL, "b3d_conv2d_tf32: on-the-fly fold needs one-row tiles");
            const uint64_t dims[4] = {8, (uint64_t)W, (uint64_t)H, (uint64_t)N};
            const uint64_t strides[3] = {32, (uint64_t)W * 32, (uint64_t)H * W * 32};
            const uint32_t box[4] = {8, (uint32_t)p.BW, 4, 1};
            if (int rc = tc::make_tmap_f32(&mx, x, 4, dims, strides, box, nullptr, CU_TENSOR_MAP_SWIZZLE_32B)) return rc;
        } else {
            const uint64_t dims[4] = {(uint64_t)Cin, (uint64_t)W, (uint64_t)H, (uint64_t)N};
            const uint64_t strides[3] = {(uint64_t)Cin * 4, (uint64_t)xpitch * Cin * 4, (uint64_t)H * xpitch * Cin * 4};
            const uint32_t box[4] = {(uint32_t)BK, (uint32_t)(sx * (p.BW - 1) + 1), (uint32_t)(sy * (p.BH - 1) + 1), (uint32_t)p.BI};
            const uint32_t es[4] = {1, (uint32_t)sx, (uint32_t)sy, 1};
            if (int rc = tc::make_tmap_f32(&mx, x, 4, dims, strides, box, es)) return rc;
        }
        if (BN == 256) return launch_conv<256, 4>(mx, mw, mm, p, bias, out, tiles, st);
        if (BN == 128) return launch_conv<128, 6>(mx, mw, mm, p, bias, out, tiles, st);
        return launch_conv<64, 8>(mx, mw, mm, p, bias, out, tiles, st);
    };
    const int bw_full = pow2_floor(Wout < BM ? Wout : BM);
    const int rem = Wout % bw_full;
    if (rem != 0 && rem * 8 <= bw_full && Wout > bw_full) {
        const int rc = run(0, Wout - rem);
        return rc ? rc : run(Wout - rem, Wout);
    }
    return run(0, Wout);
}

int b3d_conv2d_wgrad_tf32(const float* dy, const float* x, float* dw, int N, int H, int W, int Cin, int Hout, int Wout,
                          int Cout, int kh, int kw, int pad_y, int stride, int x_off, int tap_major, int fold_kh, int dy_row_pitch,
                          void* stream) {
    B3D_REQUIRE(N > 0 && Cin > 0 && Cout > 0 && H > 0 && W > 0 && Hout > 0 && Wout > 0, B3D_EINVAL,
                "b3d_conv2d_wgrad_tf32: bad sizes");
    B3D_REQUIRE(kh * kw <= MAX_TAPS && (stride == 1 || stride == 2) && x_off >= 0, B3D_EINVAL, "b3d_conv2d_wgrad_tf32: bad kernel/stride");
    B3D_REQUIRE(dy && x && dw, B3D_EINVAL, "b3d_conv2d_wgrad_tf32: null pointer");
    B3D_REQUIRE(Cin % 32 == 0 && Cout % 32 == 0, B3D_EINVAL,
                "b3d_conv2d_wgrad_tf32: Cin=%d and Cout=%d must be multiples of 32 (pad the channels with zeros)", Cin, Cout);
    B3D_CHECK_ALIGNED(dy);
    B3D_CHECK_ALIGNED(x);
    b3d::clear_variant();
    if (tap_major) B3D_CHECK_ALIGNED(dw);
    WgradParams p{};
    p.N = N; p.Hout = Hout; p.Wout = Wout; p.Cout = Cout; p.Cin = Cin;
    const uint64_t dpitch = dy_row_pitch > 0 ? dy_row_pitch : Wout;
    B3D_REQUIRE(dpitch >= (uint64_t)Wout, B3D_EINVAL, "b3d_conv2d_wgrad_tf32: dy_row_pitch=%d must be >= Wout=%d", dy_row_pitch, Wout);
    cudaStream_t st = (cudaStream_t)stream;
    if (fold_kh > 0) {
        B3D_REQUIRE(fold_kh > 4 && fold_kh <= 8 && Cin == 64 && kh == 1 && kw == STEM_KW && stride == 1 && x_off == 0 &&
                        Cout % 64 == 0 && W == Wout + STEM_KW - 1 && Hout == H + 2 * pad_y - fold_kh + 1,
                    B3D_EINVAL, "b3d_conv2d_wgrad_tf32: the raw-input stem weight gradient needs 4 < fold_kh <= 8 rows folded into "
                    "64 channels, a 1x5 stride-1 filter, Cout %% 64 == 0 and the x padding in the input");
        p.BWk = BK; p.BHk = 1;
        p.kx = b3d::ceil_div(Wout, BK);
        p.ky = Hout;
        p.kh = 1; p.kw = kw; p.pad_y = pad_y; p.st = 1; p.tapmajor = tap_major ? 1 : 0;
        p.splits = wgrad_splits(Cout / 64, (long long)N * p.kx * p.ky);
        CUtensorMap mdy, mx;
        {
            const uint64_t dims[5] = {32, (uint64_t)Wout, (uint64_t)Hout, (uint64_t)N, (uint64_t)Cout / 32};
            const uint64_t strides[4] = {(uint64_t)Cout * 4, dpitch * Cout * 4, (uint64_t)Hout * dpitch * Cout * 4, 128};
            const uint32_t box[5] = {32, (uint32_t)BK, 1, 1, 2};
            if (int rc = tc::make_tmap_f32(&mdy, dy, 5, dims, strides, box)) return rc;
        }
        {
            const uint64_t dims[4] = {8, (uint64_t)W, (uint64_t)H, (uint64_t)N};
            const uint64_t strides[3] = {32, (uint64_t)W * 32, (uint64_t)H * W * 32};
            const uint32_t box[4] = {8, (uint32_t)StemSmem::WPX, (uint32_t)fold_kh, 1};
            if (int rc = tc::make_tmap_f32(&mx, x, 4, dims, strides, box, nullptr, CU_TENSOR_MAP_SWIZZLE_NONE)) return rc;
        }
        B3D_CUDA_OK(cudaFuncSetAttribute(wgrad_stem_kernel, cudaFuncAttributeMaxDynamicSharedMemorySize, StemSmem::TOTAL));
        wgrad_stem_kernel<<<dim3(Cout / 64, p.splits), NTHREADS, StemSmem::TOTAL, st>>>(mdy, mx, p, fold_kh, dw);
        B3D_LAUNCH_OK();
        b3d::add_variant("wgrad_stem<%d,%d,%d>", STEM_KW, STEM_STAGES, STEM_NRAW);
        return B3D_OK;
    }
    p.BWk = pow2_floor(Wout < BK ? Wout : BK);
    p.BHk = BK / p.BWk;
    p.kx = b3d::ceil_div(Wout, p.BWk);
    p.ky = b3d::ceil_div(Hout, p.BHk);
    p.kh = kh; p.kw = kw; p.pad_y = pad_y; p.st = stride; p.xoff = x_off; p.tapmajor = tap_major ? 1 : 0;
    const int BN = Cin > 64 ? 128 : 64;
    int T = 1;
    p.tstep = 1;
    if (Wout >= BK) {
        if (stride == 1 && kw == 3 && BN == 64) T = 3;
        if (stride == 2 && kw == 4) { T = 2; p.tstep = 2; }
    }
    const int base_ctas = b3d::ceil_div(Cout, BM) * b3d::ceil_div(Cin, BN) * kh * (kw / T);
    const long long ktotal = (long long)N * p.kx * p.ky;
    const int splits = wgrad_splits(base_ctas, ktotal);
    p.splits = splits;

    CUtensorMap mdy, mx;
    {
        const uint64_t dims[5] = {32, (uint64_t)Wout, (uint64_t)Hout, (uint64_t)N, (uint64_t)Cout / 32};
        const uint64_t strides[4] = {(uint64_t)Cout * 4, dpitch * Cout * 4, (uint64_t)Hout * dpitch * Cout * 4, 128};
        const uint32_t box[5] = {32, (uint32_t)p.BWk, (uint32_t)p.BHk, 1, (uint32_t)(BM / 32)};
        if (int rc = tc::make_tmap_f32(&mdy, dy, 5, dims, strides, box)) return rc;
    }
    {
        const uint64_t dims[5] = {32, (uint64_t)W, (uint64_t)H, (uint64_t)N, (uint64_t)Cin / 32};
        const uint64_t strides[4] = {(uint64_t)Cin * 4, (uint64_t)W * Cin * 4, (uint64_t)H * W * Cin * 4, 128};
        const int wpx = T == 1 ? p.BWk : 36;
        const uint32_t box[5] = {32, (uint32_t)(stride * (wpx - 1) + 1), (uint32_t)(stride * (p.BHk - 1) + 1), 1, (uint32_t)(BN / 32)};
        const uint32_t es[5] = {1, (uint32_t)stride, (uint32_t)stride, 1, 1};
        if (int rc = tc::make_tmap_f32(&mx, x, 5, dims, strides, box, es, CU_TENSOR_MAP_SWIZZLE_NONE)) return rc;
    }
    dim3 grid(b3d::ceil_div(Cout, BM), b3d::ceil_div(Cin, BN), kh * (kw / T) * splits);
    if (T == 3) return launch_wgrad<64, 3, 3, 3>(mdy, mx, p, dw, grid, st);
    if (T == 2) return BN == 128 ? launch_wgrad<128, 2, 3, 2>(mdy, mx, p, dw, grid, st) : launch_wgrad<64, 3, 3, 2>(mdy, mx, p, dw, grid, st);
    if (BN == 128) return launch_wgrad<128, 3, 3, 1>(mdy, mx, p, dw, grid, st);
    return launch_wgrad<64, 4, 4, 1>(mdy, mx, p, dw, grid, st);
}

}
```

### 2dimageto3dmodel_b200/models/gan.py

```python
import math

import torch
import torch.nn as nn
import torch.nn.functional as F

from b3d import B3DError
from b3d.bank import WeightBank
from b3d.conv import conv2d as _tc_conv2d
from b3d.conv import ActLink, conv2d_banked
from b3d.ew import CIRCULAR, REPLICATE, CBNBatch, cbn_act_pad, identity_norm, in_act_pad, norm_kind, pad_x, stem_input
from rendering.utils import adjust_poles, symmetrize_texture


class TCConv2d(nn.Conv2d):

    def forward(self, x, leaky=1.0, pad_out=0, pad_mode=CIRCULAR, x_crop=0):
        if not x.is_cuda:
            raise B3DError("models.gan convolutions run on CUDA only (libb3d wgmma kernels); there is no CPU fallback")
        if self.stride[0] != self.stride[1] or self.dilation != (1, 1) or self.groups != 1 or self.padding_mode != 'zeros':
            raise B3DError("TCConv2d supports zero padding, square strides, no dilation / groups")
        if self.padding[1] != 0:
            x = F.pad(x, (self.padding[1], self.padding[1], 0, 0))
        return _tc_conv2d(x, self.weight, self.bias, pad_y=self.padding[0], stride=self.stride[0], leaky=leaky,
                          pad_out=pad_out, pad_mode=pad_mode, x_crop=x_crop)


def positional_encoding(Ny, Nx):
    half = (Nx == Ny // 2)
    lat = torch.arange(Ny, dtype=torch.float64) * (math.pi / Ny)
    lon = -math.pi + torch.arange(Ny, dtype=torch.float64) * (2 * math.pi / Ny)
    rows, cols = lat.view(Ny, 1).expand(Ny, Ny), lon.view(1, Ny).expand(Ny, Ny)
    enc = torch.stack((rows.cos(), rows.sin(), cols.cos(), cols.sin()))
    if half:
        enc = enc[:, :, Ny // 4: Ny - Ny // 4]
    return enc.numpy()


def _norm_and_bias(args):
    if args.norm_d == 'instance':
        return (lambda ch: nn.InstanceNorm2d(ch, affine=True)), False
    if args.norm_d == 'none':
        return (lambda ch: None), True
    raise ValueError(f"norm_d={args.norm_d!r}")


def _conv_norm_act(conv, norm, x, pad_next=0, lw=None, link_in=None, link_out=None):
    if lw is not None:
        run = lambda **kw: conv2d_banked(x, lw, pad_y=conv.padding[0], stride=conv.stride[0], link_in=link_in,
                                         link_out=link_out, **kw)
    else:
        run = lambda **kw: conv(x, **kw)
    if norm is None and conv.out_channels in (16, 32, 64, 128, 256, 512, 1024):
        return run(leaky=0.2, pad_out=pad_next, pad_mode=CIRCULAR)
    if norm_kind(norm) == 'instance' and norm.affine and conv.out_channels in (16, 32, 64, 128, 256, 512, 1024):
        return in_act_pad(run(), norm, pad_next, CIRCULAR, 0.2)
    y = run(leaky=0.2) if norm is None else F.leaky_relu(norm(run()), 0.2)
    return pad_x(y, pad_next, CIRCULAR) if pad_next else y


def _head(conv, x, lw):
    return conv(x) if lw is None else conv2d_banked(x, lw, pad_y=conv.padding[0], stride=conv.stride[0])


def _bankable(m):
    return isinstance(m, TCConv2d) and m.padding[1] == 0 and m.dilation == (1, 1) and m.groups == 1 and m.stride[0] == m.stride[1]


class _DiscriminatorBase(nn.Module):

    def _setup(self, args, circular, positional_embeddings):
        self.args = args
        self.circular = circular
        self.positional_embeddings = positional_embeddings
        if circular:
            self.pad = lambda x: pad_x(x, 2, CIRCULAR)
            self.pad2 = lambda x: pad_x(x, 1, CIRCULAR)
        else:
            self.pad = lambda x: x
        if positional_embeddings:
            self.pos_emb = None

    def _positions(self, x):
        if self.pos_emb is None:
            self.pos_emb = torch.FloatTensor(positional_encoding(x.shape[2], x.shape[3])).unsqueeze(0)
        dev_copy = getattr(self, '_pos_emb_dev', None)
        if dev_copy is None or dev_copy.device != x.device:
            dev_copy = self._pos_emb_dev = self.pos_emb.to(x.device)
        return dev_copy

    def _with_positions(self, x, extra=()):
        parts = [x, *extra]
        if self.positional_embeddings:
# ... 153 lines not shown
                        fold.append(f"{dn}.{cn}")
            bank = self.__dict__['_bank'] = WeightBank(convs, fold=fold)
        return bank.forward(self.training) if bank else None

    def forward(self, x, mesh_map=None, c=None, caption=None):
        W = self._weights() if x.is_cuda else None
        d1, m1 = self.d1(x, c, caption, W=W, prefix="d1.")
        if self.args.texture_only:
            d2, m2 = self.d2(x, c, caption, W=W, prefix="d2.")
        else:
            d2, m2 = self.d2(x, mesh_map, c, caption, W=W, prefix="d2.")
        if self.args.num_discriminators == 3:
            d3, m3 = self.d3(x, c, caption, W=W, prefix="d3.")
            return [d1, d2, d3], [m1, m2, m3]
        return [d1, d2], [m1, m2]


class ConditionalBatchNorm2d(nn.Module):
    def __init__(self, args, ch, emb_dim):
        super().__init__()
        kind = args.norm_g
        if kind == 'syncbatch':
            from sync_batchnorm import SynchronizedBatchNorm2d
            self.norm = SynchronizedBatchNorm2d(ch, affine=False)
        elif kind == 'batch':
            self.norm = nn.BatchNorm2d(ch, affine=False)
        elif kind == 'instance':
            self.norm = nn.InstanceNorm2d(ch, affine=False)
        elif kind == 'none':
            self.norm = identity_norm
        else:
            raise ValueError(f"norm_g={kind!r}")
        self.fc_gamma = nn.Linear(emb_dim, ch)
        self.fc_beta = nn.Linear(emb_dim, ch)

    def forward(self, x, z):
        g = self.fc_gamma(z)[:, :, None, None]
        b = self.fc_beta(z)[:, :, None, None]
        return self.norm(x) * (1 + g) + b


class ResBlockUp(nn.Module):
    def __init__(self, args, ch_in, ch_out, emb_dim, pad_fn):
        super().__init__()
        mid = min(ch_in, ch_out)
        self.ch_out = ch_out
        sn = nn.utils.spectral_norm
        self.conv1 = sn(TCConv2d(ch_in, mid, 3, padding=(1, 0), bias=False))
        self.conv2 = sn(TCConv2d(mid, ch_out, 3, padding=(1, 0), bias=False))
        self.norm1 = ConditionalBatchNorm2d(args, mid, emb_dim)
        self.norm2 = ConditionalBatchNorm2d(args, ch_out, emb_dim)
        self.relu = nn.LeakyReLU(0.2, inplace=True)
        self.pad = pad_fn
        self.shortcut = sn(TCConv2d(ch_in, ch_out, 1, bias=False)) if ch_in != ch_out else (lambda x: x)

    def forward(self, x, z):
        skip = self.shortcut(x)
        h = self.relu(self.norm1(self.conv1(self.pad(x, 1)), z))
        h = self.relu(self.norm2(self.conv2(self.pad(h, 1)), z))
        return h + skip

    def fusable(self):
        return norm_kind(self.norm1.norm) is not None and norm_kind(self.norm2.norm) is not None

    def forward_fused(self, xp, z, up, pad_next, post_leaky=False, W=None, prefix="", cb=None, pad_mode=REPLICATE):
        s1 = s2 = None
        if W is not None:
            if cb is not None:
                s1, s2 = cb.stats_slot(self.norm1), cb.stats_slot(self.norm2)
            c1 = lambda t: conv2d_banked(t, W[prefix + ".conv1"], pad_y=1, stats=s1)
            c2 = lambda t: conv2d_banked(t, W[prefix + ".conv2"], pad_y=1, stats=s2)
            sc = lambda t: conv2d_banked(t, W[prefix + ".shortcut"], x_crop=1)
        else:
            c1, c2, sc = self.conv1, self.conv2, (lambda t: self.shortcut(t, x_crop=1))
        y1 = c1(xp)
        a = cbn_act_pad(y1, self.norm1, z, up=1, pad=1, cb=cb, sums=s1, pad_mode=pad_mode)
        y2 = c2(a)
        if isinstance(self.shortcut, nn.Module):
            skip, off = sc(xp), 0
        else:
            skip, off = xp, 1
        return cbn_act_pad(y2, self.norm2, z, skip_nchw=skip, skip_off=off, up=up, pad=pad_next, post_leaky=post_leaky, cb=cb,
                           sums=s2, pad_mode=pad_mode)


class Generator(nn.Module):
    def __init__(self, args, emb_dim, symmetric=True, mesh_head=True):
        super().__init__()
        self.relu = nn.LeakyReLU(0.2, inplace=True)
        self.up = lambda x: F.interpolate(x, scale_factor=2, mode='nearest')
        self.args, self.symmetric, self.mesh_head = args, symmetric, mesh_head
        self.height, self.width = 8, (4 if symmetric else 8)
        if symmetric:
            self.pad = lambda x, amount: pad_x(x, amount, REPLICATE)
        else:
            self.pad = lambda x, amount: pad_x(x, amount, CIRCULAR)

        if args.conditional_class and args.conditional_color:
            self.emb_class = nn.Embedding(args.n_classes[0], emb_dim // 2)
            self.emb_color = nn.Embedding(args.n_classes[1], emb_dim // 2)
            emb_dim += emb_dim
        elif args.conditional_class:
            self.emb_class = nn.Embedding(args.n_classes[0], emb_dim)
            emb_dim += emb_dim

        self.fc = nn.Linear(emb_dim, self.height * self.width * 512)
        block = lambda cin, cout: ResBlockUp(args, cin, cout, emb_dim, self.pad)
        self.blk1 = block(512, 512)
        self.blk2 = block(512, 256)
        res = args.texture_resolution
        if res >= 256:
            self.blk3a = block(256, 256)
        if res >= 512:
            self.blk3b = block(256, 256)
        if res >= 1024:
            self.blk3c = block(256, 256)
        if args.conditional_text:
            self.att = SpatialAttention(256, args.text_embedding_dim)
        self.blk4 = block(256, 128)
        self.blk5 = block(128, 128)
        self.blk6 = block(128, 64)
        self.conv_final = TCConv2d(64, 3, 5, padding=(2, 0))
        if mesh_head:
            self.blk3_mesh = block(256, 64)
            self.conv_mesh = TCConv2d(64, 3, 5, padding=(2, 0))
            with torch.no_grad():
                self.conv_mesh.weight.zero_()
                self.conv_mesh.bias.zero_()

    def forward(self, z, c=None, caption=None, return_attention=False):
        a = self.args
        if a.conditional_class:
            if c is None:
                raise AssertionError("class-conditional generator needs c")
            cond = [z, self.emb_class(c[:, 0])]
            if a.conditional_color:
                cond.append(self.emb_color(c[:, 1]))
            z = torch.cat(cond, dim=1)

        x = self.fc(z).view(z.shape[0], -1, self.height, self.width)
        x = x.contiguous(memory_format=torch.channels_last)
        if not a.conditional_text and self.blk1.fusable() and not getattr(self, 'disable_fusion', False):
            return self._forward_fused(x, z, return_attention)
        x = self.up(self.blk1(x, z))
        x = self.blk2(x, z)
        attention_map = None
        if a.conditional_text:
            att, attention_map = self.att(x, *caption)
            x = x + att
        x = self.up(x)

        t = x
        for name in ('blk3a', 'blk3b', 'blk3c'):
            if hasattr(self, name):
                t = self.up(getattr(self, name)(t, z))
        t = self.up(self.blk4(t, z))
        t = self.up(self.blk5(t, z))
        t = self.relu(self.blk6(t, z))
        x_tex = torch.tanh(self.conv_final(self.pad(t, 2)))

        x_mesh = None
        if self.mesh_head:
            m = self.relu(self.blk3_mesh(x, z))
            x_mesh = adjust_poles(self.conv_mesh(self.pad(m, 2)))

        if self.symmetric:
            x_tex = symmetrize_texture(x_tex)
            if x_mesh is not None:
                x_mesh = symmetrize_texture(x_mesh)
            if attention_map is not None:
                attention_map = symmetrize_texture(attention_map)
        return (x_tex, x_mesh, attention_map) if return_attention else (x_tex, x_mesh)

    def _weights(self):
        if getattr(self, 'disable_bank', False):
            return None
        bank = self.__dict__.get('_bank')
        if bank is None:
            convs = {}
            for bn in ('blk1', 'blk2', 'blk3a', 'blk3b', 'blk3c', 'blk4', 'blk5', 'blk6', 'blk3_mesh'):
                blk = getattr(self, bn, None)
                if blk is None:
                    continue
                convs[bn + ".conv1"], convs[bn + ".conv2"] = blk.conv1, blk.conv2
                if isinstance(blk.shortcut, nn.Module):
                    convs[bn + ".shortcut"] = blk.shortcut
            convs["conv_final"] = self.conv_final
            if self.mesh_head:
                convs["conv_mesh"] = self.conv_mesh
            bank = self.__dict__['_bank'] = WeightBank(convs)
        return bank.forward(self.training)

    def _forward_fused(self, x, z, return_attention):
        W = self._weights()
        pm = REPLICATE if self.symmetric else CIRCULAR
        names = [n for n in ('blk1', 'blk2', 'blk3a', 'blk3b', 'blk3c', 'blk4', 'blk5', 'blk6') if hasattr(self, n)]
        if self.mesh_head:
            names.append('blk3_mesh')
        cb = CBNBatch([m for n in names for m in (getattr(self, n).norm1, getattr(self, n).norm2)], z)
        blk = lambda name, inp, **kw: getattr(self, name).forward_fused(inp, z, W=W, prefix=name, cb=cb, pad_mode=pm, **kw)
        head = (lambda conv, name, inp: conv(inp)) if W is None else (lambda conv, name, inp: conv2d_banked(inp, W[name], pad_y=2))
        sym = symmetrize_texture if self.symmetric else (lambda t: t)
        p = pad_x(x, 1, pm)
        p = blk('blk1', p, up=2, pad_next=1)
        p = blk('blk2', p, up=2, pad_next=1)
        t = p
        for name in ('blk3a', 'blk3b', 'blk3c'):
            if hasattr(self, name):
                t = blk(name, t, up=2, pad_next=1)
        t = blk('blk4', t, up=2, pad_next=1)
        t = blk('blk5', t, up=2, pad_next=1)
        t = blk('blk6', t, up=1, pad_next=2, post_leaky=True)
        x_tex = sym(torch.tanh(head(self.conv_final, "conv_final", t)))
        x_mesh = None
        if self.mesh_head:
            m = blk('blk3_mesh', p, up=1, pad_next=2, post_leaky=True)
            x_mesh = sym(adjust_poles(head(self.conv_mesh, "conv_mesh", m)))
        return (x_tex, x_mesh, None) if return_attention else (x_tex, x_mesh)


class SpatialAttention(nn.Module):

    def __init__(self, input_dim, context_dim):
        super().__init__()
        self.conv_context = nn.Conv2d(context_dim, input_dim, 1, stride=1, padding=0, bias=False)
        self.sm = nn.Softmax(dim=1)

    def forward(self, input, context, mask):
        B, _, ih, iw = input.shape
        L = context.size(2)
        q = input.reshape(B, -1, ih * iw).transpose(1, 2)
        src = self.conv_context(context.unsqueeze(3)).squeeze(3)
        att = torch.bmm(q, src).view(B * ih * iw, L)
        if mask is not None:
            att = att + mask.unsqueeze(1).expand(-1, ih * iw, -1).reshape(B * ih * iw, L).float() * -10000
        att = self.sm(att).view(B, ih * iw, L).transpose(1, 2)
        out = torch.bmm(src, att).view(B, -1, ih, iw)
        return out, att.reshape(B, -1, ih, iw)
```

### include/b3d.h

```cpp
#ifndef B3D_H_
#define B3D_H_

#include <stddef.h>
#include <stdint.h>

#ifdef __cplusplus
extern "C" {
#endif

#if defined(__GNUC__)
#define B3D_API __attribute__((visibility("default")))
#else
#define B3D_API
#endif

#define B3D_OK 0
#define B3D_EINVAL (-1)
#define B3D_EALIGN (-2)
#define B3D_ECUDA (-3)

#define B3D_MODE_REFERENCE 0
#define B3D_MODE_PAPER 1

B3D_API const char* b3d_last_error(void);
// ... 60 lines not shown
                                         int F, int H, int W, int Th, int Tw, int filter, int32_t* imidx, float* imwei,
                                         float* imout, float* improb, void* stream);
B3D_API int b3d_mesh_render_filtered_bwd(const float* fgeo, const float* fuv, const float* tex, int has_bg, int B, int F,
                                         int H, int W, int Th, int Tw, int filter, const int32_t* imidx,
                                         const float* imwei, const float* d_imout, const float* d_improb, float* dfp2d,
                                         float* dfuv, float* dtex, void* stream);

B3D_API int b3d_mesh_face_pack(const float* points3d, const float* points2d, const float* normalz, float multiplier,
                               int B, int F, float* fgeo, void* stream);
B3D_API int b3d_mesh_raster_attr_fwd(const float* fgeo, const float* attr, int d, int B, int F, int H, int W,
                                     float expand, int knum, float multiplier, float delta, int32_t* imidx,
                                     float* imwei, float* imfeat, float* improb, void* stream);
B3D_API int b3d_mesh_raster_attr_bwd(const float* fgeo, const float* attr, int d, int B, int F, int H, int W,
                                     float expand, int knum, float multiplier, float delta, const int32_t* imidx,
                                     const float* imwei, const float* d_imfeat, const float* d_improb, float* dp2d,
                                     float* dattr, void* stream);

B3D_API int b3d_texel_visibility(const int32_t* imidx, const float* imwei, const float* fuv, int B, int F, int H, int W,
                                 int Th, int Tw, int symmetric, uint32_t* words, uint8_t* vis, void* stream);

B3D_API int b3d_face_normals_fwd(const float* verts, const int32_t* faces, int B, int V, int F, float* normals, void* stream);
B3D_API int b3d_face_normals_bwd(const float* verts, const int32_t* faces, const float* gnormals, int B, int V, int F,
                                 float* dverts, void* stream);

B3D_API int b3d_flat_loss_fwd(const float* norms, const int32_t* ff, int B, int F, int K, float* loss,
                              void* stream);
B3D_API int b3d_flat_loss_bwd(const float* norms, const int32_t* ff, int B, int F, int K,
                              const float* gloss, float* dnorms, void* stream);

B3D_API int b3d_rgba_mse_iou_fwd(const float* image, const float* alpha, const float* target, int B, int H,
                                 int W, float* loss, int32_t* counts, void* stream);
B3D_API int b3d_rgba_mse_bwd(const float* image, const float* alpha, const float* target, int B, int H,
                             int W, const float* gloss, float* d_image, float* d_alpha, void* stream);

B3D_API int b3d_rgba_l1_iou_fwd(const float* image, const float* alpha, const float* target, int B, int H,
                                int W, float* loss, int32_t* counts, void* stream);
B3D_API int b3d_rgba_l1_bwd(const float* image, const float* alpha, const float* target, int B, int H,
                            int W, const float* gloss, float* d_image, float* d_alpha, void* stream);

B3D_API int b3d_chamfer_nn(const float* query, const float* cand, int B, int N, int M, float* dist,
                           int32_t* idx, void* stream);
B3D_API int b3d_chamfer_bwd(const float* query, const float* cand, const int32_t* idx, const float* gdist,
                            int B, int N, int M, float* dquery, float* dcand, void* stream);

typedef struct b3d_conv_opts {
    const float* mask;
    float mask_slope;
    int stats_sum_only;
    int x_row_pitch;
    int nclass;
    int class_ooy[4];
    int class_oox[4];
} b3d_conv_opts;
B3D_API int b3d_conv2d_tf32(const float* x, const float* wt, const float* bias, float* out, int N, int H, int W,
                            int Cin, int Hout, int Wout, int Cout, int ntaps, const int* dy, const int* dx,
                            int sy, int sx, int OH, int OW, int OC, int osy, int osx, int ooy, int oox,
                            float leaky, const int* wtap, int wtaps_total, double* stats, int fold_kh,
                            int fold_pad, const b3d_conv_opts* opts, void* stream);

B3D_API int b3d_conv2d_wgrad_tf32(const float* dy, const float* x, float* dw, int N, int H, int W, int Cin,
                                  int Hout, int Wout, int Cout, int kh, int kw, int pad_y, int stride,
                                  int x_off, int tap_major, int fold_kh, int dy_row_pitch, void* stream);

B3D_API int b3d_conv2d_thin_fwd(const float* x, const float* wt, const float* bias, float* out, int N, int H, int W, int Cin,
                                int Hout, int Wout, int Cout, int kh, int kw, int pad_y, int x_off, int OW, int OC,
                                float leaky, void* stream);
B3D_API int b3d_conv2d_thin_wgrad(const float* dy, const float* x, float* dw, int N, int H, int W, int Cin, int Hout,
                                  int Wout, int Cout, int kh, int kw, int pad_y, int x_off, int tap_major, void* stream);

B3D_API int b3d_vertex_record_bytes(void);
B3D_API int b3d_vertex_pipeline_fwd(const float* dmap, long long sn, long long sc, long long sy, long long sx, int h, int w,
                                    const void* rec, const void* sgn, int B, int V, const float* scale, const float* trans,
                                    const float* rot, const float* z0, float* raw, float* vtx, void* stream);
B3D_API int b3d_vertex_pipeline_bwd(const float* g_raw, const float* g_vtx, const float* raw, const void* rec, const void* sgn,
                                    int B, int V, int h, int w, const float* scale, const float* trans, const float* rot,
                                    const float* z0, float* d_dmap, float* d_scale, float* d_trans, float* d_z0, void* stream);

B3D_API int b3d_bank_layer_bytes(void);
B3D_API int b3d_bank_forward(const void* layers, const void* items_wtu, int n_wtu, const void* items_wv, int n_wv,
                             const void* items_emit, int n_emit, float* scratch, size_t scratch_bytes, float* out,
                             int training, void* stream);
B3D_API int b3d_bank_backward(const void* layers, const void* items_dot, int n_dot, const void* items_emit, int n_emit,
                              float* out, const float* df, float* dw, void* stream);

B3D_API int b3d_pad_x_fwd(const float* x, float* out, long long rows, int W, int C, int amount, int mode, void* stream);
B3D_API int b3d_pad_x_bwd(const float* gout, float* gx, long long rows, int W, int C, int amount, int mode, void* stream);
B3D_API int b3d_stem_input_fwd(const float* x, const float* pos, float* out, int N, int C1, int C2, int H, int W, int amount,
                               int mode, void* stream);
B3D_API int b3d_stem_input_bwd(const float* gout, float* gx, int N, int C1, int C2, int H, int W, int amount, int mode,
                               void* stream);
B3D_API int b3d_fold_rows_fwd(const float* x, float* out, int N, int H, int W, int C, int kh, int pad_y, int Cp, void* stream);
B3D_API int b3d_fold_rows_bwd(const float* gout, float* gx, int N, int H, int W, int C, int kh, int pad_y, int Cp, void* stream);
B3D_API int b3d_wrap_x_inplace(float* buf, long long rows, int W, int C, int amount, int mode, void* stream);
B3D_API int b3d_wrap_x_bwd_inplace(float* g, long long rows, int W, int C, int amount, int mode, void* stream);
B3D_API int b3d_pad_leaky_bias_bwd(const float* gout_pad, const float* y_pad, float* gy, float* gbias, long long rows, int W,
                                   int C, int amount, int mode, float slope, void* stream);
B3D_API int b3d_leaky_bwd(const float* gy, const float* y, float* out, long long n, float slope, void* stream);

B3D_API int b3d_cbn_act_fwd(const float* y, const float* scale, const float* shift, const float* skip, int skip_pitch,
                            int skip_off, float* out, int N, int H, int W, int C, int up, int pad, int pad_mode, float slope,
                            int post_leaky, void* stream);
B3D_API int b3d_cbn_act_bwd1(const float* gout, const float* y, const float* scale, const float* shift, const float* skip,
                             int skip_pitch, int skip_off, const float* mean, const float* invstd, int stat_pitch, float* ga,
                             float* gskip, int gskip_pitch, int gskip_off, float* S1, float* S2, int s_pitch, int N, int H,
                             int W, int C, int up, int pad, int pad_mode, float slope, int post_leaky, void* stream);
B3D_API int b3d_cbn_act_bwd2(float* ga, const float* y, const float* gamma_t, const float* mean, const float* invstd,
                             int stat_pitch, const float* m1, const float* m2, int m_pitch, float inv_m, int N, int H, int W,
                             int C, void* stream);
B3D_API int b3d_bn_sums(const float* y, long long rows, int C, double* sums, void* stream);
B3D_API int b3d_cbn_prepare(const float* gb, int gb_pitch, int gamma_off, int beta_off, const double* sums, double count,
                            float eps, float momentum, int mode, float* running_mean, float* running_var,
                            long long* num_batches_tracked, float* mean, float* invstd, float* scale, float* shift, float* gt,
                            int N, int C, void* stream);
B3D_API int b3d_cbn_bwd_reduce(const float* S1, const float* S2, int s_pitch, const float* gt, float* red, int N, int C,
                               void* stream);
B3D_API int b3d_bn_sums_per_sample(const float* y, int N, long long HW, int C, double* sums, void* stream);
B3D_API size_t b3d_sync_buffer_bytes(int world);
B3D_API size_t b3d_sync_flag_offset(int world);
B3D_API int b3d_cbn_prepare_sync(const void* const* peer_data, const void* const* peer_flag, int rank, int world,
                                 unsigned* epoch, int* err, const float* gb, int gb_pitch, int gamma_off, int beta_off,
                                 const double* sums_local, double count, float eps, float momentum, float* running_mean,
                                 float* running_var, long long* num_batches_tracked, float* mean, float* invstd, float* scale,
                                 float* shift, float* gt, int N, int C, void* stream);
B3D_API int b3d_cbn_bwd_reduce_sync(const void* const* peer_data, const void* const* peer_flag, int rank, int world,
                                    unsigned* epoch, int* err, const float* S1, const float* S2, int s_pitch, const float* gt,
                                    float* red, int N, int C, void* stream);

B3D_API int b3d_inception_input(const float* img, int B, int H, int W, int OH, int OW, int OC, int normalize, float* out,
                                void* stream);
B3D_API int b3d_maxpool3x3s2_nhwc(const float* x, int N, int H, int W, int C, float* out, int OC, void* stream);
B3D_API int b3d_mean_hw_nhwc(const float* x, int N, int HW, int C, float* out, void* stream);
B3D_API int b3d_fid_accumulate(const float* feat, int n, int D, double* sum, double* outer, void* stream);

#define B3D_GATHER_F32 0
#define B3D_GATHER_F16 1
#define B3D_GATHER_I64 2
#define B3D_GATHER_MAX_FIELDS 8
typedef struct {
    const void* src;
    int src_type;
    int n;
    int C_src, C, H, W;
    int mirror;
    float scale, bias;
    void* dst;
} b3d_gather_field;
B3D_API int b3d_gather_fields(const b3d_gather_field* fields, int nfields, const int32_t* idx, const uint8_t* flip, int B,
                              void* stream);

#define B3D_IMAGE_MAX_RES 4
#define B3D_IMAGE_MAX_SIDE 2048
B3D_API int b3d_image_batch(const uint32_t* pixels, const int64_t* offsets, const int32_t* geometry, const float* poses,
                            int n, const int32_t* idx, const uint8_t* flip, int B, int nres, const int32_t* res,
                            float* const* images, float* scale, float* translation, float* rot, int64_t* ind,
                            void* stream);

B3D_API int b3d_pseudogt_pack(const uint8_t* vis, int Th, int Tw, const float* tex, const float* alpha, int B, int R, int C,
                              const float* image, int Ci, int h, int w, uint16_t* tex_out, uint16_t* alpha_out,
                              uint16_t* image_out, void* stream);

B3D_API int b3d_sample_pack(const float* image, const int32_t* imidx, int B, int H, int W, const float* tex, int T,
                            uint8_t* tiles, uint8_t* tex8, void* stream);

#ifdef __cplusplus
}
#endif
// ... 2 lines not shown
```

Before: 1441.

## Fold nearest-upsample into 3x3 conv via sub-pixel 2x2 parity-class weights

Generator up-blocks previously upsampled the activation 2x in the norm/activation kernel and then ran a 3x3 conv on the large map. Now the conv runs directly on the low-resolution input. The 3x3 weights are pre-combined into four 2x2 parity-class kernels (16 taps), and dgrad and wgrad use matching 4x4 transposed kernels plus a fold kernel. This removes the upsampled intermediate and cuts conv FLOPs by about 9/4 relative to 16/4 tap work. The skip path is also read at half resolution. In exchange it adds new kernels, extra weight-bank storage and a zeroed per-step wgrad scratch buffer.

```diff
diff --git a/2dimageto3dmodel_b200/b3d/__init__.py b/2dimageto3dmodel_b200/b3d/__init__.py
--- a/2dimageto3dmodel_b200/b3d/__init__.py
+++ b/2dimageto3dmodel_b200/b3d/__init__.py
@@ -69,6 +69,7 @@
 _sig("b3d_vertex_pipeline_bwd", _vp, _vp, _vp, _vp, _vp, _i, _i, _i, _i, _vp, _vp, _vp, _vp, _vp, _vp, _vp, _vp, _vp)
 _sig("b3d_bank_forward", _vp, _vp, _i, _vp, _i, _vp, _i, _vp, _sz, _vp, _i, _vp)
 _sig("b3d_bank_backward", _vp, _vp, _i, _vp, _i, _vp, _vp, _vp, _vp)
+_sig("b3d_up2_fold", _vp, _vp, _i, _i, _vp)
 _sig("b3d_pad_x_fwd", _vp, _vp, _ll, _i, _i, _i, _i, _vp)
 _sig("b3d_pad_x_bwd", _vp, _vp, _ll, _i, _i, _i, _i, _vp)
 _sig("b3d_stem_input_fwd", _vp, _vp, _vp, _i, _i, _i, _i, _i, _i, _i, _vp)
diff --git a/2dimageto3dmodel_b200/b3d/bank.py b/2dimageto3dmodel_b200/b3d/bank.py
--- a/2dimageto3dmodel_b200/b3d/bank.py
+++ b/2dimageto3dmodel_b200/b3d/bank.py
@@ -14,16 +14,16 @@
 
 
 class LayerWeights:
-    __slots__ = ("wf", "wd", "df", "Cout", "Cin", "kh", "kw", "fold", "Cinp", "Coutp", "Tp", "bias")
+    __slots__ = ("wf", "wd", "wp", "df", "Cout", "Cin", "kh", "kw", "fold", "Cinp", "Coutp", "Tp", "bias")
 
     def __init__(self, spec):
         for k in ("Cout", "Cin", "kh", "kw", "fold", "Cinp", "Coutp", "Tp"):
             setattr(self, k, spec[k])
-        self.wf = self.wd = self.df = self.bias = None
+        self.wf = self.wd = self.wp = self.df = self.bias = None
 
 
 class WeightBank:
-    def __init__(self, convs, fold=(), no_dgrad=(), round_tf32=True):
+    def __init__(self, convs, fold=(), no_dgrad=(), round_tf32=True, up2=()):
         self.names = list(convs)
         self.mods = [convs[n] for n in self.names]
         self.round_tf32 = bool(round_tf32)
@@ -36,8 +36,11 @@
             fd = n in fold
             Cinp = _r32(kh * Cin if fd else Cin)
             Tp = kw if fd else kh * kw
+            u2 = n in up2
+            if u2 and (fd or (kh, kw) != (3, 3) or Cin % 32 or Cout % 32):
+                raise B3DError(f"bank: {n}: up2 needs an unfolded 3x3 layer with Cin, Cout multiples of 32")
             sp = dict(name=n, sn=sn, Cout=Cout, Cin=Cin, kh=kh, kw=kw, fold=int(fd), Cinp=Cinp, Coutp=_r32(Cout), Tp=Tp,
-                      K=Cin * kh * kw, need_d=n not in no_dgrad)
+                      K=Cin * kh * kw, need_d=n not in no_dgrad or u2, up2=int(u2))
             sp["wf_off"] = off_out
             off_out += _r64(Tp * Cout * Cinp)
             self.specs.append(sp)
@@ -46,7 +49,7 @@
             sp["wd_off"] = -1
             if sp["need_d"]:
                 sp["wd_off"] = off_out
-                off_out += _r64(sp["Tp"] * sp["Cinp"] * sp["Coutp"])
+                off_out += _r64((32 if sp["up2"] else sp["Tp"]) * sp["Cinp"] * sp["Coutp"])
         for sp in self.specs:
             sp["u_off"], sp["v_off"], sp["scal_off"] = off_out, off_out + _r64(sp["Cout"]), off_out + _r64(sp["Cout"]) + _r64(sp["K"])
             off_out = sp["scal_off"] + 64
@@ -77,7 +80,7 @@
             rec.append(struct.pack("<3Q9q12i", ptrs[-1][0], ptrs[-1][1], ptrs[-1][2], sp["t_off"], sp["s_off"], sp["wf_off"],
                                    sp["wd_off"], sp["u_off"], sp["v_off"], sp["scal_off"], sp["wf_off"], sp["dw_off"],
                                    sp["Cout"], sp["Cin"], sp["kh"], sp["kw"], sp["fold"], sp["Cinp"], sp["Coutp"], sp["Tp"],
-                                   int(sp["sn"]), 0, 0, 0))
+                                   int(sp["sn"]), sp["up2"], 0, 0))
             if sp["sn"]:
                 wtu += [(i, a, b, 0) for a in range(-(-sp["K"] // 256)) for b in range(-(-sp["Cout"] // 64))]
                 wv += [(i, a, 0, 0) for a in range(-(-sp["Cout"] // 8))]
@@ -119,6 +122,8 @@
             lw = LayerWeights(sp)
             lw.wf = outs[i]
             lw.wd = outs[n + i] if sp["need_d"] else None
+            if sp["up2"]:
+                lw.wp, lw.wd = lw.wd[:16], lw.wd[16:].reshape(16, sp["Cin"], sp["Cout"])
             if need_grad:
                 sz = sp["Tp"] * sp["Cout"] * sp["Cinp"]
                 lw.df = df_flat[sp["wf_off"]: sp["wf_off"] + sz].view(sp["Tp"], sp["Cout"], sp["Cinp"])
@@ -139,7 +144,9 @@
         wfs, wds = [], []
         for sp in bank.specs:
             wfs.append(out[sp["wf_off"]: sp["wf_off"] + sp["Tp"] * sp["Cout"] * sp["Cinp"]].view(sp["Tp"], sp["Cout"], sp["Cinp"]))
-            if sp["need_d"]:
+            if sp["up2"]:
+                wds.append(out[sp["wd_off"]: sp["wd_off"] + 32 * sp["Cin"] * sp["Cout"]].view(32, sp["Cout"], sp["Cin"]))
+            elif sp["need_d"]:
                 wds.append(out[sp["wd_off"]: sp["wd_off"] + sp["Tp"] * sp["Cinp"] * sp["Coutp"]].view(sp["Tp"], sp["Cinp"], sp["Coutp"]))
             else:
                 wds.append(out.new_empty(0))
diff --git a/2dimageto3dmodel_b200/b3d/conv.py b/2dimageto3dmodel_b200/b3d/conv.py
--- a/2dimageto3dmodel_b200/b3d/conv.py
+++ b/2dimageto3dmodel_b200/b3d/conv.py
@@ -156,6 +156,105 @@
     return dw if tap_major else dw[:Cout, :Cin]
 
 
+def up2_fprop_taps():
+    cls = [(py, px) for py in range(2) for px in range(2)]
+    q = [(py, px, a, b) for py, px in cls for a in range(2) for b in range(2)]
+    return ([py + a - 1 for py, px, a, b in q], [px + b for py, px, a, b in q], [((py * 2 + px) * 2 + a) * 2 + b for py, px, a, b in q],
+            cls)
+
+
+def up2_dgrad_taps():
+    return [r - 1 for r in range(4) for _ in range(4)], [s - 3 for _ in range(4) for s in range(4)]
+
+
+def up2_wgrad_columns(W):
+    return [(1, W, -1), (0, 1, -3), (W + 1, 1, 2 * W - 1)]
+
+
+def _up_fprop(xp, wp, wsc=None, stats=None):
+    N, H, Wp, Cin = xp.shape
+    W, Cout = Wp - 2, wp.shape[1]
+    st = stream_ptr(xp)
+    y = torch.empty(N, 2 * H, 2 * W, Cout, device=xp.device, dtype=torch.float32)
+    dy, dx, wtap, cls = up2_fprop_taps()
+    opts = _ConvOpts(None, 1.0, 0, 0, 4)
+    for i, (py, px) in enumerate(cls):
+        opts.class_ooy[i], opts.class_oox[i] = py, px
+    check(_conv_call(lib.b3d_conv2d_tf32, ptr(xp), ptr(wp), None, ptr(y), N, H, Wp, Cin, H, W, Cout, 16, _ints(dy), _ints(dx), 1, 1,
+                     2 * H, 2 * W, Cout, 2, 2, 0, 0, 1.0, _ints(wtap), 16, ptr(stats), 0, 0,
+                     ctypes.cast(ctypes.pointer(opts), ctypes.c_void_p), st))
+    sc = None
+    if wsc is not None:
+        Csc = wsc.shape[1]
+        sc = torch.empty(N, H, W, Csc, device=xp.device, dtype=torch.float32)
+        check(_conv_call(lib.b3d_conv2d_tf32, ptr(xp), ptr(wsc), None, ptr(sc), N, H, Wp, Cin, H, W, Csc, 1, _ints([0]), _ints([1]), 1,
+                         1, H, W, Csc, 1, 1, 0, 0, 1.0, None, 0, None, 0, 0, None, st))
+    return y, sc
+
+
+def _up_dgrad(gy, wd4, gsc=None, wdsc=None):
+    N, H2, W2, Cout = gy.shape
+    H, Wp, Cin = H2 // 2, W2 // 2 + 2, wd4.shape[1]
+    st = stream_ptr(gy)
+    gx = torch.empty(N, H, Wp, Cin, device=gy.device, dtype=torch.float32)
+    dy, dx = up2_dgrad_taps()
+    check(_conv_call(lib.b3d_conv2d_tf32, ptr(gy), ptr(wd4), None, ptr(gx), N, H2, W2, Cout, H, Wp, Cin, 16, _ints(dy), _ints(dx), 2, 2,
+                     H, Wp, Cin, 1, 1, 0, 0, 1.0, None, 0, None, 0, 0, None, st))
+    if gsc is not None:
+        gs = torch.empty_like(gx)
+        check(_conv_call(lib.b3d_conv2d_tf32, ptr(gsc), ptr(wdsc), None, ptr(gs), N, H, Wp - 2, gsc.shape[3], H, Wp, Cin, 1, _ints([0]),
+                         _ints([-1]), 1, 1, H, Wp, Cin, 1, 1, 0, 0, 1.0, None, 0, None, 0, 0, None, st))
+        gx += gs
+    return gx
+
+
+def _up_wgrad(gy, xp, df, gsc=None, dfsc=None):
+    N, H, Wp, Cin = xp.shape
+    _, H2, W2, Cout = gy.shape
+    st = stream_ptr(gy)
+    dpt = torch.zeros(16, Cin, Cout, device=gy.device, dtype=torch.float32)
+    for j0, w, x_off in up2_wgrad_columns(Wp - 2):
+        check(_conv_call(lib.b3d_conv2d_wgrad_tf32, ctypes.c_void_p(xp.data_ptr() + 4 * Cin * j0), ptr(gy), ptr(dpt), N, H2, W2, Cout,
+                         H, w, Cin, 4, 4, 1, 2, x_off, 1, 0, Wp, st))
+    check(lib.b3d_up2_fold(ptr(dpt), ptr(df), Cout, Cin, st))
+    if gsc is not None:
+        check(_conv_call(lib.b3d_conv2d_wgrad_tf32, ptr(gsc), ptr(xp), ptr(dfsc), N, H, Wp, Cin, H, Wp - 2, gsc.shape[3], 1, 1, 0, 1,
+                         1, 1, 0, 0, st))
+
+
+class _UpConv(torch.autograd.Function):
+
+    @staticmethod
+    def forward(ctx, xp, wf, wfsc, lw, lwsc, stats):
+        xp = dev(xp.detach(), "x")
+        if xp.shape[3] != lw.Cin or lw.wp is None:
+            raise B3DError(f"conv2d_up2: input has {xp.shape[3]} channels (layer: {lw.Cin}), or the layer is not an up2 layer")
+        y, sc = _up_fprop(xp, dev(lw.wp.detach(), "weight"), dev(lwsc.wf.detach(), "weight") if lwsc is not None else None, stats)
+        ctx.save_for_backward(xp)
+        ctx.lw, ctx.lwsc = lw, lwsc
+        return (y, sc) if sc is not None else y
+
+    @staticmethod
+    def backward(ctx, gy, gsc=None):
+        xp, = ctx.saved_tensors
+        lw, lwsc = ctx.lw, ctx.lwsc
+        gy = dev(gy, "grad_output")
+        gsc = dev(gsc, "grad_output") if gsc is not None else None
+        gx = _up_dgrad(gy, lw.wd, gsc, lwsc.wd if gsc is not None else None) if ctx.needs_input_grad[0] else None
+        if ctx.needs_input_grad[1] or ctx.needs_input_grad[2]:
+            if lw.df is None or (gsc is not None and lwsc.df is None):
+                raise B3DError("conv2d_up2: weight gradients need the bank's gradient sinks")
+            _up_wgrad(gy, xp, lw.df, gsc, lwsc.df if gsc is not None else None)
+        return (gx, lw.df if ctx.needs_input_grad[1] else None, lwsc.df if ctx.needs_input_grad[2] else None, None, None, None)
+
+
+def conv2d_up2_banked(xp_nchw, lw, lw_sc=None, stats=None):
+    x = xp_nchw.permute(0, 2, 3, 1)
+    out = _UpConv.apply(x, lw.wf, lw_sc.wf if lw_sc is not None else None, lw, lw_sc, stats)
+    y, sc = out if lw_sc is not None else (out, None)
+    return y.permute(0, 3, 1, 2), sc.permute(0, 3, 1, 2) if sc is not None else None
+
+
 def conv2d_nhwc(x, weight, bias=None, pad_y=0, stride=1, leaky=1.0, wt=None, pad_out=0, pad_mode=1, x_crop=0):
     x = dev(x, "x")
     Cout, Cin_w, kh, kw = weight.shape
@@ -188,6 +287,8 @@
     def forward(ctx, x, w, bias, lw, pad_y, stride, leaky, pad_out, pad_mode, x_crop, stats=None, fold_raw=0, link_in=None,
                 link_out=None, fold_fwd=False):
         x = dev(x.detach(), "x")
+        if lw.wp is not None:
+            raise B3DError("conv2d: a layer registered with up2 runs through conv2d_up2_banked")
         Cx = x.shape[3]
         fold_pad = 0
         if fold_raw:
diff --git a/2dimageto3dmodel_b200/b3d/ew.py b/2dimageto3dmodel_b200/b3d/ew.py
--- a/2dimageto3dmodel_b200/b3d/ew.py
+++ b/2dimageto3dmodel_b200/b3d/ew.py
@@ -172,7 +172,8 @@
 class _CBNActPad(torch.autograd.Function):
 
     @staticmethod
-    def forward(ctx, y, gb, cb, key, bn, skip, skip_off, up, pad, post_leaky, sums_in=None, slope=0.2, pad_mode=REPLICATE):
+    def forward(ctx, y, gb, cb, key, bn, skip, skip_off, up, pad, post_leaky, sums_in=None, slope=0.2, pad_mode=REPLICATE,
+                skip_half=False):
         y = dev(y.detach(), "y")
         N, H, W, C = y.shape
         gbd = dev(gb.detach(), "gamma/beta")
@@ -225,14 +226,14 @@
                                       ptr(bn.num_batches_tracked) if track else None,
                                       ptr(mean), ptr(invstd), ptr(scale), ptr(shift), ptr(gt), N, C, st))
         sk = dev(skip.detach(), "skip") if skip is not None else None
-        pitch = sk.shape[2] if sk is not None else 0
+        pitch = (-sk.shape[2] if skip_half else sk.shape[2]) if sk is not None else 0
         out = torch.empty(N, up * H, up * W + 2 * pad, C, device=y.device, dtype=torch.float32)
         check(lib.b3d_cbn_act_fwd(ptr(y), ptr(scale), ptr(shift), ptr(sk), pitch, skip_off, ptr(out), N, H, W, C, up, pad,
                                   int(pad_mode), float(slope), int(post_leaky), st))
         ctx.save_for_backward(y, gt, scale, shift, mean, invstd, sk if sk is not None else torch.empty(0))
         ctx.cb, ctx.key = cb, key
         ctx.cfg = (skip_off, up, pad, post_leaky, mode, sync, count, sk is not None, skip.shape if skip is not None else None,
-                   P, goff, boff, float(slope), int(pad_mode))
+                   P, goff, boff, float(slope), int(pad_mode), pitch)
         ctx.peers = peers
         ctx.clamp_lim = _f32(1.0 / math.sqrt(_f32(bn.eps))) if sync else None
         return out
@@ -240,7 +241,7 @@
     @staticmethod
     def backward(ctx, gout):
         y, gt, scale, shift, mean, invstd, sk = ctx.saved_tensors
-        skip_off, up, pad, post_leaky, mode, sync, count, has_skip, skip_shape, P, goff, boff, slope, pad_mode = ctx.cfg
+        skip_off, up, pad, post_leaky, mode, sync, count, has_skip, skip_shape, P, goff, boff, slope, pad_mode, pitch = ctx.cfg
         cb = ctx.cb
         N, H, W, C = y.shape
         gout = dev(gout, "grad")
@@ -248,16 +249,17 @@
         ga = torch.empty_like(y)
         gskip, gpitch = None, 0
         if has_skip and ctx.needs_input_grad[5]:
-            gpitch = skip_shape[2]
-            gskip = torch.zeros(skip_shape, device=y.device) if gpitch != W else torch.empty(skip_shape, device=y.device)
+            gpitch = pitch
+            covered = abs(gpitch) == (W // 2 if gpitch < 0 else W)
+            gskip = torch.empty(skip_shape, device=y.device) if covered else torch.zeros(skip_shape, device=y.device)
         want_gb = ctx.needs_input_grad[1]
         sink = cb.grad_sink(N) if want_gb else torch.empty(N, P, device=y.device)
         s1 = ctypes.c_void_p(sink.data_ptr() + 4 * boff)
         s2 = ctypes.c_void_p(sink.data_ptr() + 4 * goff)
         stat_pitch = C if mode >= 3 else 0
-        check(lib.b3d_cbn_act_bwd1(ptr(gout), ptr(y), ptr(scale), ptr(shift), ptr(sk) if has_skip else None,
-                                   sk.shape[2] if has_skip else 0, skip_off, ptr(mean), ptr(invstd), stat_pitch, ptr(ga), ptr(gskip),
-                                   gpitch, skip_off, s1, s2, P, N, H, W, C, up, pad, pad_mode, slope, int(post_leaky), st))
+        check(lib.b3d_cbn_act_bwd1(ptr(gout), ptr(y), ptr(scale), ptr(shift), ptr(sk) if has_skip else None, pitch, skip_off,
+                                   ptr(mean), ptr(invstd), stat_pitch, ptr(ga), ptr(gskip), gpitch, skip_off, s1, s2, P, N, H, W, C,
+                                   up, pad, pad_mode, slope, int(post_leaky), st))
         inv_m = 0.0
         if mode >= 3:
             inv_m = 1.0 / count if mode == 3 else 0.0
@@ -288,7 +290,7 @@
                 if cb.done != cb.n_layers:
                     raise RuntimeError(f"CBNBatch: {cb.done} of {cb.n_layers} layers ran their backward before the first layer's")
                 ggb = sink.sum(dim=0, keepdim=True) if cb.shared else sink
-        return ga, ggb, None, None, None, gskip, None, None, None, None, None, None, None
+        return ga, ggb, None, None, None, gskip, None, None, None, None, None, None, None, None
 
 
 def bn_act_pad(y_nchw, bn, skip_nchw=None, skip_off=0, up=1, pad=1, post_relu=False, slope=0.0):
@@ -303,7 +305,7 @@
 
 
 def cbn_act_pad(y_nchw, cbn, z, skip_nchw=None, skip_off=0, up=1, pad=1, post_leaky=False, cb=None, sums=None,
-                pad_mode=REPLICATE):
+                pad_mode=REPLICATE, skip_half=False):
     if norm_kind(cbn.norm) is None:
         raise B3DError(f"cbn_act_pad: unsupported norm layer {cbn.norm!r}")
     _check_glue("cbn_act_pad", y_nchw, cbn.fc_gamma.out_features, int(up), int(pad), int(pad_mode))
@@ -312,7 +314,7 @@
     y = y_nchw.permute(0, 2, 3, 1)
     skip = skip_nchw.permute(0, 2, 3, 1) if skip_nchw is not None else None
     out = _CBNActPad.apply(y, cb.gb, cb, id(cbn), cbn.norm, skip, int(skip_off), int(up), int(pad), bool(post_leaky), sums, 0.2,
-                           int(pad_mode))
+                           int(pad_mode), bool(skip_half))
     return out.permute(0, 3, 1, 2)
 
 
diff --git a/2dimageto3dmodel_b200/csrc/b3d_core.cu b/2dimageto3dmodel_b200/csrc/b3d_core.cu
--- a/2dimageto3dmodel_b200/csrc/b3d_core.cu
+++ b/2dimageto3dmodel_b200/csrc/b3d_core.cu
@@ -31,6 +31,6 @@
 extern "C" {
 const char* b3d_last_error(void) { return b3d::g_err; }
 const char* b3d_last_variant(void) { return b3d::g_variant; }
-int b3d_version(void) { return 420; }
+int b3d_version(void) { return 430; }
 uint64_t b3d_launch_count(void) { return b3d::g_launches.load(std::memory_order_relaxed); }
 }
diff --git a/2dimageto3dmodel_b200/csrc/ew_kernels.cu b/2dimageto3dmodel_b200/csrc/ew_kernels.cu
--- a/2dimageto3dmodel_b200/csrc/ew_kernels.cu
+++ b/2dimageto3dmodel_b200/csrc/ew_kernels.cu
@@ -648,6 +648,7 @@
     int N, H, W, C4;
     int up, pad;
     int skip_pitch, skip_off;
+    int skip_sh;
     float slope;
     int post_leaky;
 };
@@ -675,7 +676,8 @@
         float4 o = make_float4(lk(fmaf(v.x, sc.x, sh.x), g.slope), lk(fmaf(v.y, sc.y, sh.y), g.slope),
                                lk(fmaf(v.z, sc.z, sh.z), g.slope), lk(fmaf(v.w, sc.w, sh.w), g.slope));
         if (g.skip_pitch) {
-            const float4 k = __ldg(skip + (((long long)n * g.H + ys) * g.skip_pitch + xs + g.skip_off) * g.C4 + c);
+            const float4 k = __ldg(skip + (((long long)n * (g.H >> g.skip_sh) + (ys >> g.skip_sh)) * g.skip_pitch + (xs >> g.skip_sh) +
+                                           g.skip_off) * g.C4 + c);
             o.x += k.x; o.y += k.y; o.z += k.z; o.w += k.w;
         }
         if (g.post_leaky) o = make_float4(lk(o.x, g.slope), lk(o.y, g.slope), lk(o.z, g.slope), lk(o.w, g.slope));
@@ -694,7 +696,8 @@
         const int ys = yo / g.up;
         const float4 sc = __ldg(scale + (long long)n * g.C4 + c), sh = __ldg(shift + (long long)n * g.C4 + c);
         const float4* yrow = y + (((long long)n * g.H + ys) * g.W) * g.C4 + c;
-        const float4* srow = g.skip_pitch ? skip + (((long long)n * g.H + ys) * g.skip_pitch + g.skip_off) * g.C4 + c : nullptr;
+        const float4* srow = g.skip_pitch ? skip + (((long long)n * (g.H >> g.skip_sh) + (ys >> g.skip_sh)) * g.skip_pitch + g.skip_off) * g.C4 + c
+                                          : nullptr;
         float4* orow = out + (long long)row * Wo * g.C4 + c;
         constexpr int U = 4;
         for (int xb = px0; xb < Wo; xb += U * PPB) {
@@ -706,7 +709,7 @@
                 int xs = src_col(xo, g.pad, Wu, PM);
                 xs = g.up == 2 ? xs >> 1 : xs;
                 v[u] = __ldg(yrow + (long long)xs * g.C4);
-                if (srow) k[u] = __ldg(srow + (long long)xs * g.C4);
+                if (srow) k[u] = __ldg(srow + (long long)(xs >> g.skip_sh) * g.C4);
             }
 #pragma unroll
             for (int u = 0; u < U; ++u) {
@@ -722,7 +725,7 @@
     }
 }
 
-template <int PM, bool PS>
+template <int PM, bool PS, int HS>
 __global__ void __launch_bounds__(NT)
 cbn_act_bwd1_kernel(const float4* __restrict__ gout, const float4* __restrict__ y, const float4* __restrict__ scale,
                     const float4* __restrict__ shift, const float4* __restrict__ skip, const float4* __restrict__ mean,
@@ -736,52 +739,59 @@
         const long long so = PS ? (long long)n * g.C4 + c : c;
         const float4 mu = __ldg(mean + so), is = __ldg(invstd + so);
         float4 a1 = make_float4(0.f, 0.f, 0.f, 0.f), a2 = a1;
-        for (int p = y0 * g.W + lane_px; p < y1 * g.W; p += px_step) {
-            const int ys = p / g.W, xs = p % g.W;
-            float4 s = make_float4(0.f, 0.f, 0.f, 0.f);
-            for (int i = 0; i < g.up; ++i) {
-                const float4* row = gout + (((long long)n * g.up * g.H + g.up * ys + i) * Wo) * g.C4 + c;
-                if (PM == 0) {
-                    int lo = g.up * xs + g.pad, hi = lo + g.up;
-                    if (xs == 0) lo = 0;
-                    if (xs == g.W - 1) hi = Wo;
-                    for (int xo = lo; xo < hi; ++xo) {
-                        const float4 v = __ldg(row + (long long)xo * g.C4);
-                        s.x += v.x; s.y += v.y; s.z += v.z; s.w += v.w;
-                    }
-                } else {
-                    for (int u = g.up * xs; u < g.up * xs + g.up; ++u) {
-                        float4 v = __ldg(row + (long long)(u + g.pad) * g.C4);
-                        s.x += v.x; s.y += v.y; s.z += v.z; s.w += v.w;
-                        if (u < g.pad) {
-                            v = __ldg(row + (long long)(u + g.pad + Wu) * g.C4);
+        const int Wq = g.W >> HS;
+        for (int p = (y0 >> HS) * Wq + lane_px; p < (y1 >> HS) * Wq; p += px_step) {
+            float4 t = make_float4(0.f, 0.f, 0.f, 0.f);
+#pragma unroll
+            for (int e = 0; e < (1 << (2 * HS)); ++e) {
+                const int ys = ((p / Wq) << HS) + (e >> 1), xs = ((p % Wq) << HS) + (e & 1);
+                float4 s = make_float4(0.f, 0.f, 0.f, 0.f);
+                for (int i = 0; i < g.up; ++i) {
+                    const float4* row = gout + (((long long)n * g.up * g.H + g.up * ys + i) * Wo) * g.C4 + c;
+                    if (PM == 0) {
+                        int lo = g.up * xs + g.pad, hi = lo + g.up;
+                        if (xs == 0) lo = 0;
+                        if (xs == g.W - 1) hi = Wo;
+                        for (int xo = lo; xo < hi; ++xo) {
+                            const float4 v = __ldg(row + (long long)xo * g.C4);
                             s.x += v.x; s.y += v.y; s.z += v.z; s.w += v.w;
                         }
-                        if (u >= Wu - g.pad) {
-                            v = __ldg(row + (long long)(u + g.pad - Wu) * g.C4);
+                    } else {
+                        for (int u = g.up * xs; u < g.up * xs + g.up; ++u) {
+                            float4 v = __ldg(row + (long long)(u + g.pad) * g.C4);
                             s.x += v.x; s.y += v.y; s.z += v.z; s.w += v.w;
+                            if (u < g.pad) {
+                                v = __ldg(row + (long long)(u + g.pad + Wu) * g.C4);
+                                s.x += v.x; s.y += v.y; s.z += v.z; s.w += v.w;
+                            }
+                            if (u >= Wu - g.pad) {
+                                v = __ldg(row + (long long)(u + g.pad - Wu) * g.C4);
+                                s.x += v.x; s.y += v.y; s.z += v.z; s.w += v.w;
+                            }
                         }
                     }
                 }
+                const long long idx = (((long long)n * g.H + ys) * g.W + xs) * g.C4 + c;
+                const float4 v = __ldg(y + idx);
+                const float4 pre = make_float4(fmaf(v.x, sc.x, sh.x), fmaf(v.y, sc.y, sh.y), fmaf(v.z, sc.z, sh.z), fmaf(v.w, sc.w, sh.w));
+                if (g.post_leaky) {
+                    float4 k = make_float4(0.f, 0.f, 0.f, 0.f);
+                    if (g.skip_pitch)
+                        k = __ldg(skip + (((long long)n * (g.H >> HS) + (ys >> HS)) * g.skip_pitch + (xs >> HS) + g.skip_off) * g.C4 + c);
+                    s.x = (lk(pre.x, g.slope) + k.x) >= 0.f ? s.x : s.x * g.slope;
+                    s.y = (lk(pre.y, g.slope) + k.y) >= 0.f ? s.y : s.y * g.slope;
+                    s.z = (lk(pre.z, g.slope) + k.z) >= 0.f ? s.z : s.z * g.slope;
+                    s.w = (lk(pre.w, g.slope) + k.w) >= 0.f ? s.w : s.w * g.slope;
+                }
+                t.x += s.x; t.y += s.y; t.z += s.z; t.w += s.w;
+                const float4 a = make_float4(pre.x >= 0.f ? s.x : s.x * g.slope, pre.y >= 0.f ? s.y : s.y * g.slope,
+                                             pre.z >= 0.f ? s.z : s.z * g.slope, pre.w >= 0.f ? s.w : s.w * g.slope);
+                ga[idx] = a;
+                a1.x += a.x; a1.y += a.y; a1.z += a.z; a1.w += a.w;
+                a2.x = fmaf(a.x, (v.x - mu.x) * is.x, a2.x); a2.y = fmaf(a.y, (v.y - mu.y) * is.y, a2.y);
+                a2.z = fmaf(a.z, (v.z - mu.z) * is.z, a2.z); a2.w = fmaf(a.w, (v.w - mu.w) * is.w, a2.w);
             }
-            const long long idx = (((long long)n * g.H + ys) * g.W + xs) * g.C4 + c;
-            const float4 v = __ldg(y + idx);
-            const float4 pre = make_float4(fmaf(v.x, sc.x, sh.x), fmaf(v.y, sc.y, sh.y), fmaf(v.z, sc.z, sh.z), fmaf(v.w, sc.w, sh.w));
-            if (g.post_leaky) {
-                float4 k = make_float4(0.f, 0.f, 0.f, 0.f);
-                if (g.skip_pitch) k = __ldg(skip + (((long long)n * g.H + ys) * g.skip_pitch + xs + g.skip_off) * g.C4 + c);
-                s.x = (lk(pre.x, g.slope) + k.x) >= 0.f ? s.x : s.x * g.slope;
-                s.y = (lk(pre.y, g.slope) + k.y) >= 0.f ? s.y : s.y * g.slope;
-                s.z = (lk(pre.z, g.slope) + k.z) >= 0.f ? s.z : s.z * g.slope;
-                s.w = (lk(pre.w, g.slope) + k.w) >= 0.f ? s.w : s.w * g.slope;
-            }
-            if (gskip) gskip[(((long long)n * g.H + ys) * gskip_pitch + xs + gskip_off) * g.C4 + c] = s;
-            const float4 a = make_float4(pre.x >= 0.f ? s.x : s.x * g.slope, pre.y >= 0.f ? s.y : s.y * g.slope,
-                                         pre.z >= 0.f ? s.z : s.z * g.slope, pre.w >= 0.f ? s.w : s.w * g.slope);
-            ga[idx] = a;
-            a1.x += a.x; a1.y += a.y; a1.z += a.z; a1.w += a.w;
-            a2.x = fmaf(a.x, (v.x - mu.x) * is.x, a2.x); a2.y = fmaf(a.y, (v.y - mu.y) * is.y, a2.y);
-            a2.z = fmaf(a.z, (v.z - mu.z) * is.z, a2.z); a2.w = fmaf(a.w, (v.w - mu.w) * is.w, a2.w);
+            if (gskip) gskip[(((long long)n * (g.H >> HS) + p / Wq) * gskip_pitch + p % Wq + gskip_off) * g.C4 + c] = t;
         }
         float* s1 = S1 + (long long)n * s_pitch + c * 4;
         float* s2 = S2 + (long long)n * s_pitch + c * 4;
@@ -822,9 +832,12 @@
                 "b3d_cbn_act_fwd: bad arguments");
     B3D_REQUIRE(pad_mode == 0 || (pad_mode == 1 && pad <= up * W), B3D_EINVAL, "b3d_cbn_act_fwd: pad mode %d with pad %d > %d columns",
                 pad_mode, pad, up * W);
+    const int skip_sh = skip_pitch < 0;
+    skip_pitch = skip_sh ? -skip_pitch : skip_pitch;
+    B3D_REQUIRE(!skip_sh || (H % 2 == 0 && W % 2 == 0), B3D_EINVAL, "b3d_cbn_act_fwd: a half-resolution skip needs even H, W");
     if (N == 0) return B3D_OK;
     B3D_REQUIRE(y && scale && shift && out && (skip != nullptr) == (skip_pitch != 0), B3D_EINVAL, "b3d_cbn_act_fwd: null pointer");
-    CbnGeom g{N, H, W, C / 4, up, pad, skip_pitch, skip_off, slope, post_leaky};
+    CbnGeom g{N, H, W, C / 4, up, pad, skip_pitch, skip_off, skip_sh, slope, post_leaky};
     const long long total = (long long)N * up * H * (up * W + 2 * pad) * (C / 4);
     cudaStream_t st = (cudaStream_t)stream;
     if (g.C4 <= NT && NT % g.C4 == 0 && (up == 1 || up == 2)) {
@@ -855,18 +868,26 @@
     B3D_REQUIRE(stat_pitch == 0 || stat_pitch == C, B3D_EINVAL, "b3d_cbn_act_bwd1: statistics pitch %d must be 0 or C=%d", stat_pitch, C);
     B3D_REQUIRE(pad >= 0 && (pad_mode == 0 || (pad_mode == 1 && pad <= up * W)), B3D_EINVAL,
                 "b3d_cbn_act_bwd1: pad mode %d with pad %d > %d columns", pad_mode, pad, up * W);
+    const int skip_sh = skip_pitch < 0;
+    skip_pitch = skip_sh ? -skip_pitch : skip_pitch;
+    B3D_REQUIRE(skip_sh == (gskip_pitch < 0) || !gskip, B3D_EINVAL, "b3d_cbn_act_bwd1: skip and its gradient differ in resolution");
+    gskip_pitch = gskip_pitch < 0 ? -gskip_pitch : gskip_pitch;
+    B3D_REQUIRE(!skip_sh || (H % 2 == 0 && W % 2 == 0), B3D_EINVAL, "b3d_cbn_act_bwd1: a half-resolution skip needs even H, W");
     if (N == 0) return B3D_OK;
     B3D_REQUIRE(gout && y && scale && shift && mean && invstd && ga && S1 && S2, B3D_EINVAL, "b3d_cbn_act_bwd1: null pointer");
     cudaStream_t st = (cudaStream_t)stream;
     B3D_REQUIRE(s_pitch >= C && s_pitch % 4 == 0, B3D_EINVAL, "b3d_cbn_act_bwd1: S pitch %d must be >= C and a multiple of 4", s_pitch);
     B3D_CUDA_OK(cudaMemset2DAsync(S1, sizeof(float) * (size_t)s_pitch, 0, sizeof(float) * (size_t)C, (size_t)N, st));
     B3D_CUDA_OK(cudaMemset2DAsync(S2, sizeof(float) * (size_t)s_pitch, 0, sizeof(float) * (size_t)C, (size_t)N, st));
-    CbnGeom g{N, H, W, C / 4, up, pad, skip_pitch, skip_off, slope, post_leaky};
+    CbnGeom g{N, H, W, C / 4, up, pad, skip_pitch, skip_off, skip_sh, slope, post_leaky};
     int rows = (int)(((long long)N * H + 132 * 8 - 1) / (132 * 8));
     rows = rows < 1 ? 1 : rows;
+    rows += skip_sh && rows % 2;
     dim3 grid(b3d::ceil_div(H, rows), N);
-    auto kernel = pad_mode == 0 ? (stat_pitch ? cbn_act_bwd1_kernel<0, true> : cbn_act_bwd1_kernel<0, false>)
-                                : (stat_pitch ? cbn_act_bwd1_kernel<1, true> : cbn_act_bwd1_kernel<1, false>);
+    auto kernel = skip_sh ? (pad_mode == 0 ? (stat_pitch ? cbn_act_bwd1_kernel<0, true, 1> : cbn_act_bwd1_kernel<0, false, 1>)
+                                           : (stat_pitch ? cbn_act_bwd1_kernel<1, true, 1> : cbn_act_bwd1_kernel<1, false, 1>))
+                          : (pad_mode == 0 ? (stat_pitch ? cbn_act_bwd1_kernel<0, true, 0> : cbn_act_bwd1_kernel<0, false, 0>)
+                                           : (stat_pitch ? cbn_act_bwd1_kernel<1, true, 0> : cbn_act_bwd1_kernel<1, false, 0>));
     kernel<<<grid, NT, 0, st>>>((const float4*)gout, (const float4*)y, (const float4*)scale, (const float4*)shift, (const float4*)skip,
                                 (const float4*)mean, (const float4*)invstd, (float4*)ga, (float4*)gskip, gskip_pitch, gskip_off, S1, S2,
                                 s_pitch, g, rows);
diff --git a/2dimageto3dmodel_b200/csrc/sn_kernels.cu b/2dimageto3dmodel_b200/csrc/sn_kernels.cu
--- a/2dimageto3dmodel_b200/csrc/sn_kernels.cu
+++ b/2dimageto3dmodel_b200/csrc/sn_kernels.cu
@@ -20,7 +20,7 @@
     long long dw_off;
     int Cout, Cin, kh, kw;
     int fold, Cinp, Coutp, Tp;
-    int sn, pad0, pad1, pad2;
+    int sn, up2, pad1, pad2;
 };
 
 struct Item { int layer, a, b, c; };
@@ -98,6 +98,17 @@
     const float nrm = fmaxf(sqrtf(p), SN_EPS);
     *inv_s = 1.f / nrm;
     return p / nrm;
+}
+
+__device__ __forceinline__ int up2_lo(int p, int a) { return p ? 2 * a : a; }
+__device__ __forceinline__ int up2_hi(int p, int a) { return p ? 1 + a : 2 * a; }
+
+__device__ __forceinline__ float up2_phase(const float (&w)[9], int q) {
+    const int py = q >> 3, px = (q >> 2) & 1, a = (q >> 1) & 1, b = q & 1;
+    float v = 0.f;
+    for (int k = up2_lo(py, a); k <= up2_hi(py, a); ++k)
+        for (int l = up2_lo(px, b); l <= up2_hi(px, b); ++l) v += w[k * 3 + l];
+    return v;
 }
 
 __global__ void __launch_bounds__(NT)
@@ -150,6 +161,26 @@
         }
     }
     if (L.wd_off < 0) return;
+    if (L.up2) {
+        float* P = outb + L.wd_off;
+        float* D4 = P + (size_t)16 * L.Cout * L.Cin;
+        for (int pass = 0; pass < 2; ++pass)
+            for (int e = threadIdx.x; e < 32 * 32; e += NT) {
+                const int ci = ci0 + (pass ? e >> 5 : e & 31), co = co0 + (pass ? e & 31 : e >> 5);
+                if (co >= L.Cout || ci >= L.Cin) continue;
+                float w[9];
+#pragma unroll
+                for (int t = 0; t < 9; ++t) w[t] = __ldg(L.w + (co * L.Cin + ci) * 9 + t) * rs;
+                for (int q = 0; q < 16; ++q) {
+                    const float val = tf32_rna(up2_phase(w, q), round_tf32);
+                    const int py = q >> 3, px = (q >> 2) & 1, a = (q >> 1) & 1, b = q & 1;
+                    const int t4 = (3 - py - 2 * a) * 4 + 3 - px - 2 * b;
+                    if (pass) D4[((size_t)t4 * L.Cin + ci) * L.Cout + co] = val;
+                    else P[((size_t)q * L.Cout + co) * L.Cin + ci] = val;
+                }
+            }
+        return;
+    }
     const int cop0 = it.a * 32;
     for (int e = threadIdx.x; e < 32 * 32; e += NT) {
         const int co = cop0 + (e & 31), ci = ci0 + (e >> 5);
@@ -217,9 +248,42 @@
     }
 }
 
+__global__ void __launch_bounds__(NT)
+up2_fold_kernel(const float* __restrict__ dpt, float* __restrict__ df, int Cout, int Cin) {
+    __shared__ float tile[9][32][33];
+    const int co0 = blockIdx.x * 32, ci0 = blockIdx.y * 32;
+    for (int e = threadIdx.x; e < 32 * 32; e += NT) {
+        const int co = e & 31, ci = e >> 5;
+        float acc[9] = {};
+        for (int q = 0; q < 16; ++q) {
+            const int py = q >> 3, px = (q >> 2) & 1, a = (q >> 1) & 1, b = q & 1;
+            const int t4 = (3 - py - 2 * a) * 4 + 3 - px - 2 * b;
+            const float g = __ldg(dpt + ((size_t)t4 * Cin + ci0 + ci) * Cout + co0 + co);
+            for (int k = up2_lo(py, a); k <= up2_hi(py, a); ++k)
+                for (int l = up2_lo(px, b); l <= up2_hi(px, b); ++l) acc[k * 3 + l] += g;
+        }
+#pragma unroll
+        for (int t = 0; t < 9; ++t) tile[t][co][ci] = acc[t];
+    }
+    __syncthreads();
+    for (int e = threadIdx.x; e < 32 * 32; e += NT) {
+        const int ci = e & 31, co = e >> 5;
+#pragma unroll
+        for (int t = 0; t < 9; ++t) df[((size_t)t * Cout + co0 + co) * Cin + ci0 + ci] += tile[t][co][ci];
+    }
+}
+
 }
 
 extern "C" {
+
+int b3d_up2_fold(const float* dpt, float* df, int Cout, int Cin, void* stream) {
+    B3D_REQUIRE(dpt && df && Cout > 0 && Cin > 0 && Cout % 32 == 0 && Cin % 32 == 0, B3D_EINVAL,
+                "b3d_up2_fold: bad arguments (Cout=%d, Cin=%d must be multiples of 32)", Cout, Cin);
+    up2_fold_kernel<<<dim3(Cout / 32, Cin / 32), NT, 0, (cudaStream_t)stream>>>(dpt, df, Cout, Cin);
+    B3D_LAUNCH_OK();
+    return B3D_OK;
+}
 
 int b3d_bank_layer_bytes(void) { return (int)sizeof(BankLayer); }
 
diff --git a/2dimageto3dmodel_b200/csrc/tc_common.cuh b/2dimageto3dmodel_b200/csrc/tc_common.cuh
--- a/2dimageto3dmodel_b200/csrc/tc_common.cuh
+++ b/2dimageto3dmodel_b200/csrc/tc_common.cuh
@@ -194,6 +194,11 @@
 inline int make_tmap_f32(CUtensorMap* m, const void* base, int rank, const uint64_t* dims, const uint64_t* strides_b,
                          const uint32_t* box, const uint32_t* elem_strides = nullptr,
                          CUtensorMapSwizzle swz = CU_TENSOR_MAP_SWIZZLE_128B) {
+    thread_local bool ctx_bound = false;
+    if (!ctx_bound) {
+        int dev = 0;
+        if (cudaGetDevice(&dev) == cudaSuccess && cudaSetDevice(dev) == cudaSuccess) ctx_bound = true;
+    }
     EncodeTiledFn fn = encode_fn();
     if (!fn) {
         b3d::set_error("cuTensorMapEncodeTiled is not available from the driver");
diff --git a/2dimageto3dmodel_b200/csrc/tc_conv.cu b/2dimageto3dmodel_b200/csrc/tc_conv.cu
--- a/2dimageto3dmodel_b200/csrc/tc_conv.cu
+++ b/2dimageto3dmodel_b200/csrc/tc_conv.cu
@@ -746,7 +746,14 @@
         B3D_REQUIRE(fold_kh <= 8 && Cin == 32 * ((8 * fold_kh + 31) / 32) && sy == 1 && sx == 1 && !wtap && Wout % BM == 0,
                     B3D_EINVAL, "b3d_conv2d_tf32: on-the-fly fold needs 8 input channels, stride 1 and Wout %% 128 == 0 (Wout=%d)", Wout);
     }
-    B3D_REQUIRE(!stats || mask || (osy == 1 && osx == 1), B3D_EINVAL, "b3d_conv2d_tf32: statistics need a dense output");
+    bool tiles = ncls == 4 && osy == 2 && osx == 2 && OH == 2 * Hout && OW == 2 * Wout;
+    for (int c = 0, seen = 0; tiles && c < 4; ++c) {
+        const int bit = 1 << (2 * cooy[c] + coox[c]);
+        tiles = cooy[c] >= 0 && cooy[c] <= 1 && coox[c] >= 0 && coox[c] <= 1 && !(seen & bit);
+        seen |= bit;
+    }
+    B3D_REQUIRE(!stats || mask || (osy == 1 && osx == 1) || tiles, B3D_EINVAL,
+                "b3d_conv2d_tf32: statistics need a dense output, or four parity classes that tile it");
     const bool bn256 = Cout % 256 == 0 && (long long)N * Hout * Wout / BM * (Cout / 256) * ncls >= tc::num_sms();
     const int BN = bn256 ? 256 : Cout > 64 ? 128 : 64;
     cudaStream_t st = (cudaStream_t)stream;
@@ -855,7 +862,7 @@
                           void* stream) {
     B3D_REQUIRE(N > 0 && Cin > 0 && Cout > 0 && H > 0 && W > 0 && Hout > 0 && Wout > 0, B3D_EINVAL,
                 "b3d_conv2d_wgrad_tf32: bad sizes");
-    B3D_REQUIRE(kh * kw <= MAX_TAPS && (stride == 1 || stride == 2) && x_off >= 0, B3D_EINVAL, "b3d_conv2d_wgrad_tf32: bad kernel/stride");
+    B3D_REQUIRE(kh * kw <= MAX_TAPS && (stride == 1 || stride == 2) && x_off > -kw, B3D_EINVAL, "b3d_conv2d_wgrad_tf32: bad kernel/stride");
     B3D_REQUIRE(dy && x && dw, B3D_EINVAL, "b3d_conv2d_wgrad_tf32: null pointer");
     B3D_REQUIRE(Cin % 32 == 0 && Cout % 32 == 0, B3D_EINVAL,
                 "b3d_conv2d_wgrad_tf32: Cin=%d and Cout=%d must be multiples of 32 (pad the channels with zeros)", Cin, Cout);
diff --git a/2dimageto3dmodel_b200/models/gan.py b/2dimageto3dmodel_b200/models/gan.py
--- a/2dimageto3dmodel_b200/models/gan.py
+++ b/2dimageto3dmodel_b200/models/gan.py
@@ -7,7 +7,7 @@
 from b3d import B3DError
 from b3d.bank import WeightBank
 from b3d.conv import conv2d as _tc_conv2d
-from b3d.conv import ActLink, conv2d_banked
+from b3d.conv import ActLink, conv2d_banked, conv2d_up2_banked
 from b3d.ew import CIRCULAR, REPLICATE, CBNBatch, cbn_act_pad, identity_norm, in_act_pad, norm_kind, pad_x, stem_input
 from rendering.utils import adjust_poles, symmetrize_texture
 
@@ -327,6 +327,16 @@
             skip, off = xp, 1
         return cbn_act_pad(y2, self.norm2, z, skip_nchw=skip, skip_off=off, up=up, pad=pad_next, post_leaky=post_leaky, cb=cb,
                            sums=s2, pad_mode=pad_mode)
+
+    def forward_fused_up(self, xp, z, pad_next, W, prefix, cb, post_leaky=False, pad_mode=REPLICATE):
+        s1, s2 = cb.stats_slot(self.norm1), cb.stats_slot(self.norm2)
+        has_sc = isinstance(self.shortcut, nn.Module)
+        y1, skip = conv2d_up2_banked(xp, W[prefix + ".conv1"], W[prefix + ".shortcut"] if has_sc else None, stats=s1)
+        a = cbn_act_pad(y1, self.norm1, z, up=1, pad=1, cb=cb, sums=s1, pad_mode=pad_mode)
+        y2 = conv2d_banked(a, W[prefix + ".conv2"], pad_y=1, stats=s2)
+        skip, off = (skip, 0) if has_sc else (xp, 1)
+        return cbn_act_pad(y2, self.norm2, z, skip_nchw=skip, skip_off=off, skip_half=True, up=1, pad=pad_next,
+                           post_leaky=post_leaky, cb=cb, sums=s2, pad_mode=pad_mode)
 
 
 class Generator(nn.Module):
@@ -417,6 +427,8 @@
                 attention_map = symmetrize_texture(attention_map)
         return (x_tex, x_mesh, attention_map) if return_attention else (x_tex, x_mesh)
 
+    UP_BLOCKS = ('blk2', 'blk3a', 'blk3b', 'blk3c', 'blk4', 'blk5', 'blk6', 'blk3_mesh')
+
     def _weights(self):
         if getattr(self, 'disable_bank', False):
             return None
@@ -433,7 +445,7 @@
             convs["conv_final"] = self.conv_final
             if self.mesh_head:
                 convs["conv_mesh"] = self.conv_mesh
-            bank = self.__dict__['_bank'] = WeightBank(convs)
+            bank = self.__dict__['_bank'] = WeightBank(convs, up2=[n + ".conv1" for n in self.UP_BLOCKS])
         return bank.forward(self.training)
 
     def _forward_fused(self, x, z, return_attention):
@@ -443,7 +455,13 @@
         if self.mesh_head:
             names.append('blk3_mesh')
         cb = CBNBatch([m for n in names for m in (getattr(self, n).norm1, getattr(self, n).norm2)], z)
-        blk = lambda name, inp, **kw: getattr(self, name).forward_fused(inp, z, W=W, prefix=name, cb=cb, pad_mode=pm, **kw)
+
+        def blk(name, inp, up=2, pad_next=1, post_leaky=False):
+            b = getattr(self, name)
+            if W is not None and name in self.UP_BLOCKS:
+                return b.forward_fused_up(inp, z, pad_next, W, name, cb, post_leaky=post_leaky, pad_mode=pm)
+            return b.forward_fused(inp, z, up=1 if W is not None else up, pad_next=pad_next, post_leaky=post_leaky, W=W, prefix=name,
+                                   cb=cb, pad_mode=pm)
         head = (lambda conv, name, inp: conv(inp)) if W is None else (lambda conv, name, inp: conv2d_banked(inp, W[name], pad_y=2))
         sym = symmetrize_texture if self.symmetric else (lambda t: t)
         p = pad_x(x, 1, pm)
diff --git a/include/b3d.h b/include/b3d.h
--- a/include/b3d.h
+++ b/include/b3d.h
@@ -166,6 +166,7 @@
                              int training, void* stream);
 B3D_API int b3d_bank_backward(const void* layers, const void* items_dot, int n_dot, const void* items_emit, int n_emit,
                               float* out, const float* df, float* dw, void* stream);
+B3D_API int b3d_up2_fold(const float* dpt, float* df, int Cout, int Cin, void* stream);
 
 B3D_API int b3d_pad_x_fwd(const float* x, float* out, long long rows, int W, int C, int amount, int mode, void* stream);
 B3D_API int b3d_pad_x_bwd(const float* gout, float* gx, long long rows, int W, int C, int amount, int mode, void* stream);
```

Result: faster. 1591, median of 6 (+10.4%).
